# QData/LaMP

Hardware: AMD Instinct MI355X
Metric: forward samples/sec, reuters d512 2+2L 4h (higher is better)
Workload: dtype f32

## Files before the change

### include/lamp_hip.h

```cpp
#ifndef LAMP_HIP_H
#define LAMP_HIP_H

#include <stddef.h>
#include <stdint.h>

#ifdef __cplusplus
extern "C" {
#endif
#if defined(__GNUC__)
#pragma GCC visibility push(default)
#endif

#define LAMP_HIP_ABI_VERSION 5

typedef void* lamp_stream_t;

enum lamp_status {
    LAMP_OK = 0,
    LAMP_E_DIMS = -1,
    LAMP_E_ALIGN = -2,
    LAMP_E_WORKSPACE = -3,
    LAMP_E_UNSUPPORTED = -4,
    LAMP_E_NULL = -5
};
// ... 36 lines not shown
    const float* ln_g;
    const float* ln_b;
    int32_t n_head;
    int32_t present;
} lamp_mha_weights;

typedef struct lamp_ffn_weights {
    const float* w1;
    const float* b1;
    const float* w2;
    const float* b2;
    const float* ln_g;
    const float* ln_b;
} lamp_ffn_weights;

typedef struct lamp_enc_layer {
    lamp_mha_weights slf_attn;
    lamp_ffn_weights pos_ffn;
} lamp_enc_layer;

typedef struct lamp_dec_layer {
    lamp_mha_weights enc_attn;
    lamp_ffn_weights pos_ffn1;
    lamp_mha_weights slf_attn;
    lamp_ffn_weights pos_ffn2;
} lamp_dec_layer;

typedef struct lamp_chain_pack {
    const float* fc;
    const float* w1;
    const float* w2;
    const float* fc4;
    const float* w14;
    const float* w24;
} lamp_chain_pack;

typedef struct lamp_model {
    int32_t n_src_vocab, n_position, n_labels;
    int32_t d_model, d_inner, d_k, d_v;
    int32_t n_layers_enc, n_layers_dec;
    int32_t label_mask_flags;
    const float* src_word_emb;
    const float* position_enc;
    const float* tgt_word_emb;
    const float* w_out;
    const uint8_t* label_mask;
    const uint32_t* label_mask_bits;
    const int32_t* label_tiles;
    const lamp_enc_layer* enc_layers;
    const lamp_dec_layer* dec_layers;
    const float* dec0_query;
    const lamp_chain_pack* chain_packs;
    const float* enc0_emb_w1;
    const float* enc0_pos_w1;
    int64_t label_mask_allowed;
} lamp_model;

typedef struct lamp_aux {
    float* const* enc_self_attn;
    float* const* dec_self_attn;
    float* const* dec_enc_attn;
    float* const* int_preds;
    int32_t n_int_preds;
    int32_t reserved;
} lamp_aux;

int lamp_version(void);
const char* lamp_strerror(int status);


int lamp_linear_fwd(const float* A, int64_t M, int32_t K, int64_t lda,
                    const float* W, int32_t N, int64_t ldw, const float* bias,
                    const float* residual, int64_t ldr, int32_t relu,
                    float* C, int64_t ldc, lamp_stream_t stream);

#define LAMP_PREC_FP32 0
#define LAMP_PREC_BF16X3 1
#define LAMP_PREC_BF16X6 2
int lamp_linear_prec_fwd(const float* A, int64_t M, int32_t K, int64_t lda,
                         const float* W, int32_t N, int64_t ldw, const float* bias,
                         const float* residual, int64_t ldr, int32_t relu,
                         float* C, int64_t ldc, int32_t precision, lamp_stream_t stream);

int lamp_layernorm_fwd(const float* x, int64_t M, int32_t d, const float* gamma, const float* beta,
                       float eps, float* y, lamp_stream_t stream);

int lamp_sdpa_fwd(const float* q, const float* k, const float* v, float* out, float* attn,
                  int32_t B, int32_t H, int32_t lq, int32_t lk, int32_t d_k, int32_t d_v,
                  float inv_temperature, const lamp_mask* mask, const lamp_attn_layout* layout,
                  lamp_stream_t stream);

int lamp_sdpa_fwd_fast_maps(const float* q, const float* k, const float* v, float* out, float* attn, float* lse,
                            int32_t B, int32_t H, int32_t lq, int32_t lk, int32_t d_k, int32_t d_v,
                            float inv_temperature, const lamp_mask* mask, const lamp_attn_layout* layout,
                            lamp_stream_t stream);

#define LAMP_ATTN_SOFTMAX 0
#define LAMP_ATTN_SIGMOID 1

int lamp_sdpa_act_fwd(const float* q, const float* k, const float* v, float* out, float* attn,
                      int32_t B, int32_t H, int32_t lq, int32_t lk, int32_t d_k, int32_t d_v,
                      float inv_temperature, int32_t act, const lamp_mask* mask, const lamp_attn_layout* layout,
                      lamp_stream_t stream);

int lamp_mha_act_fwd(const float* xq, const float* xkv, int32_t B, int32_t lq, int32_t lk,
                     int32_t d_model, int32_t d_k, int32_t d_v, const lamp_mha_weights* w, int32_t act,
                     const lamp_mask* mask, float* out, float* attn,
                     void* workspace, size_t workspace_bytes, lamp_stream_t stream);

size_t lamp_mha_workspace_bytes(int32_t B, int32_t lq, int32_t lk, int32_t d_model, int32_t n_head,
                                int32_t d_k, int32_t d_v);
int lamp_mha_fwd(const float* xq, const float* xkv, int32_t B, int32_t lq, int32_t lk,
                 int32_t d_model, int32_t d_k, int32_t d_v, const lamp_mha_weights* w,
                 const lamp_mask* mask, float* out, float* attn,
                 void* workspace, size_t workspace_bytes, lamp_stream_t stream);

size_t lamp_ffn_workspace_bytes(int64_t M, int32_t d_model, int32_t d_inner);
int lamp_ffn_fwd(const float* x, int64_t M, int32_t d_model, int32_t d_inner,
                 const lamp_ffn_weights* w, float* out,
                 void* workspace, size_t workspace_bytes, lamp_stream_t stream);

int lamp_embed_fwd(const int64_t* src_seq, const int64_t* src_pos, int64_t n_tokens,
                   const float* emb, int32_t n_vocab, const float* pos_table, int32_t n_position,
                   int32_t d_model, float* out, lamp_stream_t stream);

int lamp_diag_logits_fwd(const float* y, const float* w_out, int32_t B, int32_t L, int32_t d_model,
                         float* logits, lamp_stream_t stream);

int lamp_sigmoid_bce_fwd(const float* logits, const float* targets, int64_t n_rows, int32_t L,
                         float* probs, float* row_loss, lamp_stream_t stream);

int lamp_prior_graph_build(const int64_t* label_ids, const int64_t* offsets, int64_t n_samples, int32_t L,
                           float* adj, uint8_t* blocked, lamp_stream_t stream);

int lamp_pack_weight(const float* W, int32_t N, int32_t K, int64_t ldw, int32_t format, float* packed, lamp_stream_t stream);


typedef struct lamp_gemm_desc {
    const float* A;
    const float* B;
    float* C;
    int32_t M, N, K;
    int32_t batch0, batch1;
    int32_t accumulate;
    int64_t a_row_stride, a_col_stride, a_batch0, a_batch1;
    int64_t b_row_stride, b_col_stride, b_batch0, b_batch1;
    int64_t ldc, c_batch0, c_batch1;
    const float* relu_mask;
    int64_t ld_mask;
    float alpha;
    int32_t reserved;
} lamp_gemm_desc;
size_t lamp_gemm_workspace_bytes(int32_t M, int32_t N, int32_t K, int32_t batch);
int lamp_gemm(const lamp_gemm_desc* d, void* workspace, size_t workspace_bytes, lamp_stream_t stream);

int lamp_gemm_grouped(const lamp_gemm_desc* descs, int32_t n, lamp_stream_t stream);


typedef struct lamp_reduce_job {
    const float* partial;
    int64_t n_total, n_seg;
    float* out[3];
    int32_t n_partials;
    int32_t reserved;
} lamp_reduce_job;
int lamp_reduce_partials_grouped(const lamp_reduce_job* jobs, int32_t n, lamp_stream_t stream);
// ... 13 lines not shown
    float p_attn, p_out;
    uint32_t seed_attn, seed_out;
} lamp_mha_train_desc;
int lamp_mha_train_fwd(const lamp_mha_train_desc* c, const lamp_mha_weights* w, const float* xq, const float* xk,
                       const float* xv, const lamp_mask* mask, float* q, float* k, float* v, float* a, float* P, float* Pd,
                       float* lse, float* o, float* y, lamp_stream_t stream);
size_t lamp_mha_bwd_workspace_bytes(const lamp_mha_train_desc* c);
size_t lamp_mha_bwd_partials_bytes(const lamp_mha_train_desc* c);
int lamp_mha_bwd(const lamp_mha_train_desc* c, const lamp_mha_weights* w, const float* xq, const float* xk, const float* xv,
                 const float* q, const float* k, const float* v, const float* a, const float* P, const float* Pd,
                 const float* o, const float* dy, float* dxq, float* d_o, float* da, float* dP, float* dq, float* dk, float* dv,
                 float* dxk, float* dxv, float* dgamma, float* dbeta, float* dwq, float* dwk, float* dwv, float* dfc,
                 void* workspace, size_t workspace_bytes, void* partials, size_t partials_bytes, lamp_reduce_job* job,
                 lamp_stream_t stream);

int lamp_mha_train_act_fwd(const lamp_mha_train_desc* c, const lamp_mha_weights* w, int32_t act, const float* xq,
                           const float* xk, const float* xv, const lamp_mask* mask, float* q, float* k, float* v, float* a,
                           float* P, float* Pd, float* lse, float* o, float* y, lamp_stream_t stream);
int lamp_mha_act_bwd(const lamp_mha_train_desc* c, const lamp_mha_weights* w, int32_t act, const float* xq, const float* xk,
                     const float* xv, const float* q, const float* k, const float* v, const float* a, const float* P,
                     const float* Pd, const float* o, const float* dy, float* dxq, float* d_o, float* da, float* dP, float* dq,
                     float* dk, float* dv, float* dxk, float* dxv, float* dgamma, float* dbeta, float* dwq, float* dwk,
                     float* dwv, float* dfc, void* workspace, size_t workspace_bytes, void* partials, size_t partials_bytes,
                     lamp_reduce_job* job, lamp_stream_t stream);

int lamp_layernorm_residual_fwd(const float* x, const float* residual, int64_t residual_rows, int64_t M, int32_t d,
                                const float* gamma, const float* beta, float eps, float dropout_p, uint32_t seed,
                                float* y, lamp_stream_t stream);

size_t lamp_layernorm_bwd_workspace_bytes(int64_t M, int32_t d);
int lamp_layernorm_bwd(const float* x, const float* residual, int64_t residual_rows, int64_t M, int32_t d,
                       const float* gamma, float eps, float dropout_p, uint32_t seed, const float* dy, float* dz,
                       float* dx, float* dgamma, float* dbeta, float* dbias, void* workspace, size_t workspace_bytes,
                       lamp_stream_t stream);

size_t lamp_colsum_workspace_bytes(int64_t M, int64_t N);
int lamp_colsum(const float* x, int64_t M, int64_t N, int64_t ldx, float* out, void* workspace,
                size_t workspace_bytes, lamp_stream_t stream);

int lamp_dropout(const float* x, int64_t n, float p, uint32_t seed, float* y, lamp_stream_t stream);

int lamp_softmax_bwd(const float* P, const float* dP, int64_t rows, int32_t lk, float scale, float* dS,
                     lamp_stream_t stream);

int lamp_sigmoid_attn_bwd(const float* P, const float* dP, int64_t rows, int32_t lk, float scale, float dropout_p,
                          uint32_t seed, float* dS, lamp_stream_t stream);

int lamp_diag_logits_bwd(const float* y, const float* w_out, const float* dlogits, int32_t B, int32_t L,
                         int32_t d_model, float* dy, float* dw, lamp_stream_t stream);

int lamp_embed_bwd(const int64_t* src_seq, int64_t n_tokens, const float* dout, int32_t d_model, int32_t n_vocab,
                   int64_t pad_idx, float* d_emb, lamp_stream_t stream);


size_t lamp_forward_workspace_bytes(const lamp_model* m, int32_t micro_batch, int32_t T,
                                    int32_t want_attn);

int lamp_forward(const lamp_model* m, const int64_t* src_seq, const int64_t* src_pos,
                 int32_t B, int32_t T, float* logits, float* enc_output, const lamp_aux* aux,
                 void* workspace, size_t workspace_bytes, lamp_stream_t stream);

#define LAMP_FWD_PACKED_ENCODER 1

#define LAMP_FWD_DEC_SIGMOID 2

#define LAMP_FWD_MATMUL_BF16X3 4
#define LAMP_FWD_MATMUL_BF16X6 8

#define LAMP_FWD_LABEL_BIAS 16

typedef struct lamp_fwd_options {
    int32_t enc_self_attn;
    int32_t flags;
    const lamp_mask* enc_mask;
    const lamp_chain_pack* enc_chain_packs;
} lamp_fwd_options;

size_t lamp_forward_opts_workspace_bytes(const lamp_model* m, const lamp_fwd_options* opts, int32_t micro_batch, int32_t T,
                                         int32_t want_attn);
int lamp_forward_opts(const lamp_model* m, const lamp_fwd_options* opts, const int64_t* src_seq, const int64_t* src_pos,
                      int32_t B, int32_t T, float* logits, float* enc_output, const lamp_aux* aux, void* workspace,
                      size_t workspace_bytes, lamp_stream_t stream);

typedef struct lamp_onehot_frontend {
    const float* t1;
    const float* conv1_b;
    const float* conv2_w;
    const float* conv2_b;
    const float* conv2_pack;
    int32_t n_vocab;
    int32_t taps;
} lamp_onehot_frontend;

size_t lamp_onehot_forward_workspace_bytes(const lamp_model* m, const lamp_onehot_frontend* fe, int32_t micro_batch, int32_t T,
                                           int32_t want_attn);
int lamp_onehot_forward(const lamp_model* m, const lamp_onehot_frontend* fe, const int64_t* src_seq, const int64_t* src_pos,
                        int32_t B, int32_t T, float* logits, float* enc_output, const lamp_aux* aux, void* workspace,
                        size_t workspace_bytes, lamp_stream_t stream);

size_t lamp_onehot_forward_opts_workspace_bytes(const lamp_model* m, const lamp_onehot_frontend* fe, const lamp_fwd_options* opts,
                                                int32_t micro_batch, int32_t T, int32_t want_attn);
int lamp_onehot_forward_opts(const lamp_model* m, const lamp_onehot_frontend* fe, const lamp_fwd_options* opts,
                             const int64_t* src_seq, const int64_t* src_pos, int32_t B, int32_t T, float* logits,
                             float* enc_output, const lamp_aux* aux, void* workspace, size_t workspace_bytes,
                             lamp_stream_t stream);

int lamp_conv_pack(const float* w, int32_t c_out, int32_t c_in, int32_t taps, int32_t flip, float* packed, lamp_stream_t stream);
int lamp_onehot_front_fwd(const int64_t* src_seq, int32_t B, int32_t T, const lamp_onehot_frontend* fe, int32_t d_model,
                          float dropout_p, uint32_t seed, float* xpad, lamp_stream_t stream);
int lamp_conv_window_fwd(const float* xpad, int32_t B, int32_t rows_out, int32_t rows_in, int32_t c_in, const float* w_pack,
                         int32_t c_out, const float* bias, int32_t relu, const float* pos_table, int32_t n_position,
                         const int64_t* src_pos, int64_t pos_ld, float* out, float* relu_out, lamp_stream_t stream);
int lamp_conv_relu_bwd_pad(const float* dy, const float* relu_out, int32_t B, int32_t rows, int32_t d, float* dz,
                           lamp_stream_t stream);
size_t lamp_onehot_front_bwd_partials_bytes(int32_t B, int32_t T, int32_t n_vocab, int32_t d_model);
int lamp_onehot_front_bwd(const int64_t* src_seq, int32_t B, int32_t T, const lamp_onehot_frontend* fe, int32_t d_model,
                          float dropout_p, uint32_t seed, const float* dP, float* dz, float* partials, size_t partials_bytes,
                          lamp_stream_t stream);

size_t lamp_ranking_metrics_workspace_bytes(int64_t n_rows, int32_t L);
int lamp_ranking_metrics(const float* probs, int64_t ld_probs, const float* targets, int64_t ld_targets, int64_t n_rows,
                         int32_t L, double fdr_cutoff, double* auc, double* aupr, double* fdr_recall, int64_t* n_pos,
                         int64_t* n_neg, void* workspace, size_t workspace_bytes, lamp_stream_t stream);

int lamp_threshold_counts(const float* probs, int64_t ld_probs, const float* targets, int64_t ld_targets, int64_t n_rows,
                          int32_t L, float threshold, int32_t* label_tp, int32_t* label_fp, int32_t* label_fn,
                          int32_t* sample_tp, int32_t* sample_pred, int32_t* sample_gold, int32_t* sample_mismatch,
                          lamp_stream_t stream);


int lamp_bce_logits_train(const float* const* logits, const float* weights, float* const* dlogits, int32_t n_mats,
                          const float* targets, int64_t n_rows, int32_t L, float* probs, int64_t ld_probs, float* row_loss,
                          int64_t ld_row_loss, lamp_stream_t stream);

int lamp_embed_bwd_ordered(const int64_t* src_seq, int64_t n_tokens, const float* dout, int32_t d_model, int32_t n_vocab,
                           int64_t pad_idx, float* d_emb, lamp_stream_t stream);

enum lamp_optim_kind { LAMP_OPTIM_ADAM = 0, LAMP_OPTIM_SGD = 1 };
typedef struct lamp_optim_entry {
    float* param;
    const float* grad;
    float* exp_avg;
    float* exp_avg_sq;
    int64_t numel;
} lamp_optim_entry;
int lamp_optim_step(const lamp_optim_entry* entries, int32_t n, int32_t kind, int64_t step, double lr, double beta1,
                    double beta2, double eps, lamp_stream_t stream);

enum lamp_kernel_class {
    LAMP_K_EMBED = 0, LAMP_K_GEMM = 1, LAMP_K_ATTN = 2, LAMP_K_LAYERNORM = 3, LAMP_K_DIAG = 4,
    LAMP_K_COUNT = 5
};
int lamp_prof_enable(int32_t on);
int lamp_prof_reset(void);
int lamp_prof_read(int32_t kernel_class, int64_t* launches, double* total_ms, double* flops,
                   double* bytes);

#if defined(__GNUC__)
#pragma GCC visibility pop
#endif
#ifdef __cplusplus
}
#endif
#endif
```

### lamp_amd/Models.py

```python
import ctypes as C

import collections

import torch
import torch.nn as nn

from . import _native as N
from .Decoders import GraphDecoder, MLPDecoder, RNNDecoder
from .Encoders import GraphEncoder, MLPEncoder, RNNEncoder
from .SubLayers import XavierLinear


def _chain_pack(fc, w1, w2, keep):
    ptrs = []
    for fmt in (0, 1):
        trio = [N.weight_pack(w, fmt) for w in (fc, w1, w2)]
        if any(t is None for t in trio):
            trio = [None] * 3
        keep.append(trio)
        ptrs += [N.ptr(t) for t in trio]
    return N.ChainPack(*ptrs)


class _MatmulPrecision:
# ... 88 lines not shown

    def get_trainable_parameters(self):
        frozen = set()
        if hasattr(self.encoder, 'position_enc'):
            frozen |= {id(p) for p in self.encoder.position_enc.parameters()}
        if self.onehot:
            frozen |= {id(p) for p in self.encoder.src_word_emb.parameters()}
        return (p for p in self.parameters() if id(p) not in frozen)

    def invalidate_native_cache(self):
        self._native_cache = None
        self._param_list = None

    def load_state_dict(self, state_dict, *args, **kwargs):
        if state_dict and all(k.startswith('module.') for k in state_dict):
            stripped = collections.OrderedDict((k[len('module.'):], v) for k, v in state_dict.items())
            meta = getattr(state_dict, '_metadata', None)
            if meta is not None:
                stripped._metadata = collections.OrderedDict(
                    (k[len('module.'):] if k.startswith('module.') else ('' if k == 'module' else k), v) for k, v in meta.items())
            state_dict = stripped
        self.invalidate_native_cache()
        return super().load_state_dict(state_dict, *args, **kwargs)

    def train(self, mode=True):
        self.invalidate_native_cache()
        return super().train(mode)

    def _apply(self, fn, *args, **kwargs):
        self.invalidate_native_cache()
        return super()._apply(fn, *args, **kwargs)

    def _weight_tensors(self):
        if not self._fused:
            raise NotImplementedError('the lamp_model descriptor exists for the graph encoder + graph decoder only')
        enc, dec = self.encoder, self.decoder
        out = [enc.src_word_emb.weight, dec.tgt_word_emb.weight, self.tgt_word_proj.linear.weight]
        if hasattr(enc, 'position_enc'):
            out.append(enc.position_enc.weight)

        def mha(m):
            out.extend((m.w_qs.weight, m.w_ks.weight, m.w_vs.weight, m.layer_norm.weight, m.layer_norm.bias))
            if getattr(m, 'fc', None) is not None:
                out.append(m.fc.weight)

        def ffn(m):
            out.extend((m.w_1.weight, m.w_1.bias, m.w_2.weight, m.w_2.bias, m.layer_norm.weight, m.layer_norm.bias))
        for l in enc.layer_stack:
            mha(l.slf_attn)
            ffn(l.pos_ffn)
        for l in dec.layer_stack:
            mha(l.enc_attn)
            ffn(l.pos_ffn1)
            if hasattr(l, 'slf_attn'):
                mha(l.slf_attn)
            ffn(l.pos_ffn2)
        return out

    def _fold_weights(self):
        enc = self.encoder
        ff = enc.layer_stack[0].pos_ffn
        return (enc.src_word_emb.weight, enc.position_enc.weight if hasattr(enc, 'position_enc') else None,
                ff.w_1.weight, ff.w_1.bias)

    def _onehot_weights(self):
        enc = self.encoder
        return (enc.src_word_emb.weight, enc.conv1.weight, enc.conv1.bias, enc.conv2.weight, enc.conv2.bias)

    def _chain_weights(self):
        out = []
        for l in self.decoder.layer_stack:
            for att, ff in ((l.enc_attn, l.pos_ffn1), (getattr(l, 'slf_attn', None), l.pos_ffn2)):
                if att is not None and getattr(att, 'fc', None) is not None:
                    out += [att.fc.weight, ff.w_1.weight, ff.w_2.weight]
        return out

    def _enc_chain_weights(self):
        out = []
        for l in self.encoder.layer_stack:
            if getattr(l.slf_attn, 'fc', None) is not None:
                out += [l.slf_attn.fc.weight, l.pos_ffn.w_1.weight, l.pos_ffn.w_2.weight]
        return out

    def _native_model(self):
        replica = getattr(self, '_is_replica', False)
        params = None if replica else self._param_list
        if params is None:
            params = self._weight_tensors()
            if not replica:
                self._param_list = params
        mask = self.decoder.label_mask_u8
        tiles = self.decoder.label_tiles
        bits = self.decoder.label_mask_bits
        bias = getattr(self.decoder, 'label_bias_f32', None)
        if bias is not None:
            mask, tiles, bits = bias, None, None
        hoist = self.cache_layer0_query and not replica
        packs = self.use_chain_packs and not replica
        onehot = bool(getattr(self.encoder, 'onehot', False))
        live = self.enc_self_attn
        fold = self.fold_embedding and not replica and len(self.encoder.layer_stack) > 0 and not onehot and not live
        sparse = bool(self.use_sparse_label_attention and self.use_mask_bits and self.decoder.label_rows_sparse and bias is None)
        key = tuple(p.data_ptr() for p in params) + (N.ptr(mask), N.ptr(bits), N.ptr(tiles), self.use_label_tiles,
                                                      hoist, self.use_mask_bits, packs, fold, sparse, live, bias is not None)
        if hoist:
            l0 = self.decoder.layer_stack[0].enc_attn
            key += (self.decoder.tgt_word_emb.weight._version, l0.w_qs.weight._version)
        if packs:
            key += tuple(w._version for w in self._chain_weights())
            if live:
                key += tuple(w._version for w in self._enc_chain_weights())
        if fold:
            key += tuple(w._version for w in self._fold_weights() if w is not None)
        if onehot:
            key += tuple((w.data_ptr(), w._version) for w in self._onehot_weights())
        cache = None if replica else self._native_cache
        if cache is not None and cache[0] == key:
            return cache[1]
        for p in params:
            if p.dtype != torch.float32 or not p.is_contiguous():
                raise RuntimeError('lamp_amd expects contiguous fp32 parameters')
        N.require_device(*params)
        enc, dec = self.encoder, self.decoder
        enc_arr = (N.EncLayer * max(1, len(enc.layer_stack)))()
        for i, l in enumerate(enc.layer_stack):
            enc_arr[i] = N.EncLayer(N.mha_weights(l.slf_attn), N.ffn_weights(l.pos_ffn))
        dec_arr = (N.DecLayer * max(1, len(dec.layer_stack)))()
        for i, l in enumerate(dec.layer_stack):
            slf = N.mha_weights(l.slf_attn) if hasattr(l, 'slf_attn') else N.MhaWeights()
            dec_arr[i] = N.DecLayer(N.mha_weights(l.enc_attn), N.ffn_weights(l.pos_ffn1), slf,
                                    N.ffn_weights(l.pos_ffn2))
        pos = enc.position_enc.weight if hasattr(enc, 'position_enc') else None
        w_out = self.tgt_word_proj.linear.weight
        if w_out.size(0) != self.n_labels:
            raise NotImplementedError('proj_share_weight=False read-out is not on the graph path')
        m = N.Model(enc.src_word_emb.weight.size(0), pos.size(0) if pos is not None else 0, self.n_labels,
                    self.d_model, self.d_inner, self.d_k, self.d_v, len(enc.layer_stack), len(dec.layer_stack),
                    N.LAMP_MASK_SPARSE_ROWS if sparse else 0, N.ptr(enc.src_word_emb.weight), N.ptr(pos), N.ptr(dec.tgt_word_emb.weight),
                    N.ptr(w_out), N.ptr(mask), N.ptr(bits) if self.use_mask_bits else 0,
                    N.ptr(tiles) if self.use_label_tiles else 0, enc_arr, dec_arr, 0)
        m.label_mask_allowed = self.decoder.label_allowed_pairs if sparse else 0
        q0 = None
        if hoist and len(dec.layer_stack) > 0:
            q0 = N.linear(dec.tgt_word_emb.weight.detach(), dec.layer_stack[0].enc_attn.w_qs.weight.detach())
            m.dec0_query = q0.data_ptr()
            torch.cuda.current_stream().synchronize()
        pack_arr = pack_keep = None
        if packs and len(dec.layer_stack) > 0:
            pack_arr = (N.ChainPack * (2 * len(dec.layer_stack)))()
            pack_keep = []
            for i, l in enumerate(dec.layer_stack):
                for j, (att, ff) in enumerate(((l.enc_attn, l.pos_ffn1), (getattr(l, 'slf_attn', None), l.pos_ffn2))):
                    if att is None or getattr(att, 'fc', None) is None:
                        continue
                    pack_arr[2 * i + j] = _chain_pack(att.fc.weight, ff.w_1.weight, ff.w_2.weight, pack_keep)
            m.chain_packs = pack_arr
            torch.cuda.current_stream().synchronize()
        enc_pack_arr = None
        if packs and live and len(enc.layer_stack) > 0:
            enc_pack_arr = (N.ChainPack * len(enc.layer_stack))()
            pack_keep = pack_keep if pack_keep is not None else []
            for i, l in enumerate(enc.layer_stack):
                if getattr(l.slf_attn, 'fc', None) is None:
                    continue
                enc_pack_arr[i] = _chain_pack(l.slf_attn.fc.weight, l.pos_ffn.w_1.weight, l.pos_ffn.w_2.weight, pack_keep)
            torch.cuda.current_stream().synchronize()
        fold_keep = None
        if fold:
            emb_w, pos_w, w1, b1 = self._fold_weights()
            w1 = w1.detach().reshape(w1.size(0), -1)
            e1 = N.linear(emb_w.detach(), w1, None if pos_w is not None else b1.detach())
            p1 = N.linear(pos_w.detach(), w1, b1.detach()) if pos_w is not None else None
            m.enc0_emb_w1, m.enc0_pos_w1 = e1.data_ptr(), N.ptr(p1)
            fold_keep = (e1, p1)
            torch.cuda.current_stream().synchronize()
        onehot_keep = None
        if onehot:
            e_w, w1, b1, w2, b2 = (w.detach() for w in self._onehot_weights())
            t1 = N.onehot_tap_table(e_w, w1)
            w2c, b1c, b2c = N.f32c(w2), N.f32c(b1), N.f32c(b2)
            w2p = N.conv_pack(w2c)
            fe = N.onehot_frontend(t1, b1c, w2c, b2c, w2p)
            onehot_keep = (fe, t1, w2c, b1c, b2c, w2p)
            torch.cuda.current_stream().synchronize()
        built = (m, enc_arr, dec_arr, q0, pack_arr, pack_keep, fold_keep, onehot_keep, enc_pack_arr)
        if not replica:
            self._native_cache = (key, built)
        return built

    def _forward_composite(self, src, adj, tgt_seq, return_attns, int_preds):
        src_seq, src_pos = src
        batch_size = src_seq.size(0)
        if self.decoder_type in ('sa_m', 'rnn_m'):
            tgt_seq = tgt_seq[:, :-1]
        enc_output, *enc_self_attns = self.encoder(src_seq, adj, src_pos, return_attns=return_attns)
        dec_output, *dec_output2 = self.decoder(tgt_seq, src_seq, enc_output, return_attns=return_attns,
                                                int_preds=int_preds)
        if self.decoder_type in ('rnn_m', 'mlp'):
            seq_logit = dec_output
        else:
            w = self.tgt_word_proj.linear.weight
            if self.decoder_type == 'graph' and w.size(0) == dec_output.size(1) and self.tgt_word_proj.linear.bias is None:
                if self.training:
                    from . import training
                    seq_logit = training._ReadoutFn.apply(dec_output, w)
                else:
                    seq_logit = N.diag_logits(dec_output, w)
            else:
                seq_logit = self.tgt_word_proj(dec_output)
                if self.decoder_type == 'graph':
                    seq_logit = torch.diagonal(seq_logit, 0, 1, 2)
        if int_preds:
            w = self.tgt_word_proj.linear.weight.detach()
            if self.training:
                from . import training
                preds = [training._ReadoutFn.apply(o, w) for o in dec_output2[0][:-1]]
            else:
                preds = [N.diag_logits(o, w) for o in dec_output2[0][:-1]]
            return seq_logit.reshape(-1, seq_logit.size(-1)), enc_output, preds
        if return_attns:
            return seq_logit.reshape(-1, seq_logit.size(-1)), enc_output, enc_self_attns, dec_output2
        return seq_logit.reshape(-1, seq_logit.size(-1)), enc_output, None

    def forward(self, src, adj, tgt_seq, binary_tgt, return_attns=False, int_preds=False):
        if self.onehot and adj:
            raise NotImplementedError('per-sample input graphs (adj) are not served with the one-hot encoder')
        if not self._fused:
            return self._forward_composite(src, adj, tgt_seq, return_attns, int_preds)
        if adj and return_attns and not int_preds and not self.training and not self.enc_self_attn:
            return self._forward_composite(src, adj, tgt_seq, return_attns, int_preds)
        src_seq, src_pos = src
        if src_seq.is_cuda and src_seq.device.index != torch.cuda.current_device():
            with torch.cuda.device(src_seq.device):
                return self.forward(src, adj, tgt_seq, binary_tgt, return_attns=return_attns, int_preds=int_preds)
        N.require_device(src_seq, src_pos)
        if self.training:
            from . import training
            return training.forward_train(self, src_seq, src_pos, return_attns=bool(return_attns and not int_preds),
                                          int_preds=bool(int_preds), adj=adj if self.enc_self_attn else None)
        dev = src_seq.device
        seq = src_seq.long().contiguous()
        pos = src_pos.long().contiguous()
        B, T = seq.shape
        L, d = self.n_labels, self.d_model
        built = self._native_model()
        model, enc_arr, dec_arr = built[:3]
        fe = built[7][0] if self.onehot else None
        T_in = T
        if fe is not None:
            T = T_in // 2
        Ne, Nd = model.n_layers_enc, model.n_layers_dec

        logits = torch.empty((B, L), dtype=torch.float32, device=dev)
        enc_output = torch.empty((B, T, d), dtype=torch.float32, device=dev)

        aux, keep = None, []
        want_attn = bool(return_attns and not int_preds)
        enc_attns = slf_attns = encdec_attns = ipreds = None
        if int_preds:
            n_int = sum(2 if hasattr(l, 'slf_attn') else 1 for l in self.decoder.layer_stack) - 1
            ipreds = [torch.empty((B, L), dtype=torch.float32, device=dev) for _ in range(n_int)]
            arr = (C.c_void_p * max(1, n_int))(*[t.data_ptr() for t in ipreds])
            keep.append(arr)
            aux = N.Aux(None, None, None, arr, n_int, 0)
        elif want_attn:
            def alloc(h, lq, lk):
                return torch.empty((h * B, lq, lk), dtype=torch.float32, device=dev)
            enc_attns = [alloc(l.slf_attn.n_head, T, T) for l in self.encoder.layer_stack]
            slf_attns = [alloc(l.slf_attn.n_head, L, L) if hasattr(l, 'slf_attn') else None
                         for l in self.decoder.layer_stack]
            encdec_attns = [alloc(l.enc_attn.n_head, L, T) for l in self.decoder.layer_stack]
            a0 = (C.c_void_p * max(1, Ne))(*[t.data_ptr() for t in enc_attns])
            a1 = (C.c_void_p * max(1, Nd))(*[N.ptr(t) for t in slf_attns])
            a2 = (C.c_void_p * max(1, Nd))(*[t.data_ptr() for t in encdec_attns])
            keep += [a0, a1, a2]
            aux = N.Aux(a0, a1, a2, None, 0, 0)

        lib = N.lib()
        opts = None
        if self.enc_self_attn:
            opts = N.FwdOptions(1, N.LAMP_FWD_PACKED_ENCODER if self.use_packed_live_encoder else 0, None, built[8])
            if adj:
                from .Encoders import adj_attn_mask
                m8 = adj_attn_mask(seq, adj)
                mstruct = N.Mask(N.LAMP_MASK_U8, 0, m8.data_ptr(), T * T, T, None, 0, 0)
                keep += [m8, mstruct]
                opts.enc_mask = C.pointer(mstruct)
        if self.dec_attn_type == 'sigmoid':
            if opts is None:
                opts = N.FwdOptions(0, 0, None, None)
            opts.flags |= N.LAMP_FWD_DEC_SIGMOID
        if getattr(self.decoder, 'label_bias_f32', None) is not None:
            if opts is None:
                opts = N.FwdOptions(0, 0, None, None)
            opts.flags |= N.LAMP_FWD_LABEL_BIAS
        prec_flag = N.matmul_precision(self.matmul_precision)[1]
        if prec_flag and not getattr(self, '_is_replica', False):
            if opts is None:
                opts = N.FwdOptions(0, 0, None, None)
            opts.flags |= prec_flag
        if opts is not None and fe is not None:
            def ws_bytes(mb):
                return lib.lamp_onehot_forward_opts_workspace_bytes(C.byref(model), C.byref(fe), C.byref(opts), mb, T_in,
                                                                    int(want_attn))
        elif opts is not None:
            def ws_bytes(mb):
                return lib.lamp_forward_opts_workspace_bytes(C.byref(model), C.byref(opts), mb, T, int(want_attn))
        elif fe is not None:
            def ws_bytes(mb):
                return lib.lamp_onehot_forward_workspace_bytes(C.byref(model), C.byref(fe), mb, T_in, int(want_attn))
        else:
            def ws_bytes(mb):
                return lib.lamp_forward_workspace_bytes(C.byref(model), mb, T, int(want_attn))
        per_sample = ws_bytes(1)
        fixed = 2 * per_sample - ws_bytes(2)
        whole = fixed + (per_sample - fixed) * B + 4096
        budget = max(per_sample + 4096, min(whole, self.workspace_limit_bytes))
        ws = N.workspace(budget, dev)
        if opts is not None and fe is not None:
            N.check(lib.lamp_onehot_forward_opts(C.byref(model), C.byref(fe), C.byref(opts), seq.data_ptr(), pos.data_ptr(), B,
                                                 T_in, logits.data_ptr(), enc_output.data_ptr(),
                                                 C.byref(aux) if aux is not None else None, ws.data_ptr(), ws.numel(),
                                                 N.stream()), 'lamp_onehot_forward_opts')
        elif opts is not None:
            N.check(lib.lamp_forward_opts(C.byref(model), C.byref(opts), seq.data_ptr(), pos.data_ptr(), B, T,
                                          logits.data_ptr(), enc_output.data_ptr(), C.byref(aux) if aux is not None else None,
                                          ws.data_ptr(), ws.numel(), N.stream()), 'lamp_forward_opts')
        elif fe is not None:
            N.check(lib.lamp_onehot_forward(C.byref(model), C.byref(fe), seq.data_ptr(), pos.data_ptr(), B, T_in,
                                            logits.data_ptr(), enc_output.data_ptr(), C.byref(aux) if aux is not None else None,
                                            ws.data_ptr(), ws.numel(), N.stream()), 'lamp_onehot_forward')
        else:
            N.check(lib.lamp_forward(C.byref(model), seq.data_ptr(), pos.data_ptr(), B, T, logits.data_ptr(),
                                     enc_output.data_ptr(), C.byref(aux) if aux is not None else None,
                                     ws.data_ptr(), ws.numel(), N.stream()), 'lamp_forward')
        del keep
        if int_preds:
            return logits, enc_output, ipreds
        if want_attn:
            return logits, enc_output, [enc_attns], [slf_attns, encdec_attns]
        return logits, enc_output, None

    workspace_limit_bytes = 8 << 30
    cache_layer0_query = True
    use_chain_packs = True
    fold_embedding = True
    matmul_precision = _MatmulPrecision()
    use_packed_live_encoder = False
    use_label_tiles = True
    use_sparse_label_attention = True
    use_mask_bits = True
```

### lamp_amd/_native.py

```python
import ctypes as C
import os
import threading

import torch

_HERE = os.path.dirname(os.path.abspath(__file__))
LIB_PATH = os.environ.get('LAMP_HIP_LIBRARY') or os.path.join(_HERE, 'liblamp_hip.so')
TUNING_LIB_PATH = os.path.join(_HERE, 'liblamp_hip_tuning.so')

ABI_VERSION = 5
LAMP_MASK_NONE, LAMP_MASK_U8, LAMP_MASK_KEY_TOKENS_I64, LAMP_MASK_BITS_U32 = 0, 1, 2, 3
LAMP_MASK_BIAS_F32 = 4
LAMP_MASK_SPARSE_ROWS, LAMP_MASK_SELF_RAGGED = 1, 2
LAMP_FWD_PACKED_ENCODER, LAMP_FWD_DEC_SIGMOID = 1, 2
LAMP_FWD_MATMUL_BF16X3, LAMP_FWD_MATMUL_BF16X6 = 4, 8
LAMP_FWD_LABEL_BIAS = 16
LAMP_PREC_FP32, LAMP_PREC_BF16X3, LAMP_PREC_BF16X6 = 0, 1, 2
MATMUL_PRECISIONS = {'highest': (LAMP_PREC_FP32, 0), 'high': (LAMP_PREC_BF16X3, LAMP_FWD_MATMUL_BF16X3),
                     'bf16x6': (LAMP_PREC_BF16X6, LAMP_FWD_MATMUL_BF16X6)}
LAMP_ATTN_SOFTMAX, LAMP_ATTN_SIGMOID = 0, 1
ATTN_TYPES = {'softmax': LAMP_ATTN_SOFTMAX, 'sigmoid': LAMP_ATTN_SIGMOID}
K_EMBED, K_GEMM, K_ATTN, K_LAYERNORM, K_DIAG, K_COUNT = 0, 1, 2, 3, 4, 5
KERNEL_CLASS_NAMES = ('embed', 'gemm', 'attention', 'layernorm', 'diag_readout')


class LampError(RuntimeError):
    def __init__(self, status, where):
        self.status = status
        msg = lib().lamp_strerror(status).decode() if _lib is not None else '?'
        super().__init__('%s failed with status %d: %s' % (where, status, msg))


_f32p = C.POINTER(C.c_float)
_vp = C.c_void_p


class Mask(C.Structure):
    _fields_ = [('kind', C.c_int32), ('flags', C.c_int32), ('ptr', _vp),
                ('stride_b', C.c_int64), ('stride_q', C.c_int64),
                ('tile_list', _vp), ('tile_list_stride', C.c_int64), ('allowed_pairs', C.c_int64)]


class AttnLayout(C.Structure):
    _fields_ = [(n, C.c_int64) for n in ('q_b', 'q_h', 'q_r', 'k_b', 'k_h', 'k_r',
                                         'v_b', 'v_h', 'v_r', 'o_b', 'o_h', 'o_r')]


class MhaWeights(C.Structure):
    _fields_ = [('w_qs', _vp), ('w_ks', _vp), ('w_vs', _vp), ('fc', _vp), ('ln_g', _vp), ('ln_b', _vp),
                ('n_head', C.c_int32), ('present', C.c_int32)]


class FfnWeights(C.Structure):
    _fields_ = [('w1', _vp), ('b1', _vp), ('w2', _vp), ('b2', _vp), ('ln_g', _vp), ('ln_b', _vp)]


class EncLayer(C.Structure):
    _fields_ = [('slf_attn', MhaWeights), ('pos_ffn', FfnWeights)]


class DecLayer(C.Structure):
    _fields_ = [('enc_attn', MhaWeights), ('pos_ffn1', FfnWeights), ('slf_attn', MhaWeights),
                ('pos_ffn2', FfnWeights)]


class ChainPack(C.Structure):
    _fields_ = [('fc', _vp), ('w1', _vp), ('w2', _vp), ('fc4', _vp), ('w14', _vp), ('w24', _vp)]


class Model(C.Structure):
    _fields_ = [('n_src_vocab', C.c_int32), ('n_position', C.c_int32), ('n_labels', C.c_int32),
                ('d_model', C.c_int32), ('d_inner', C.c_int32), ('d_k', C.c_int32), ('d_v', C.c_int32),
                ('n_layers_enc', C.c_int32), ('n_layers_dec', C.c_int32), ('label_mask_flags', C.c_int32),
                ('src_word_emb', _vp), ('position_enc', _vp), ('tgt_word_emb', _vp), ('w_out', _vp),
                ('label_mask', _vp), ('label_mask_bits', _vp), ('label_tiles', _vp), ('enc_layers', C.POINTER(EncLayer)), ('dec_layers', C.POINTER(DecLayer)),
                ('dec0_query', _vp), ('chain_packs', C.POINTER(ChainPack)),
                ('enc0_emb_w1', _vp), ('enc0_pos_w1', _vp), ('label_mask_allowed', C.c_int64)]


class GemmDesc(C.Structure):
    _fields_ = [('A', _vp), ('B', _vp), ('C', _vp), ('M', C.c_int32), ('N', C.c_int32), ('K', C.c_int32),
                ('batch0', C.c_int32), ('batch1', C.c_int32), ('accumulate', C.c_int32),
                ('a_row_stride', C.c_int64), ('a_col_stride', C.c_int64), ('a_batch0', C.c_int64), ('a_batch1', C.c_int64),
                ('b_row_stride', C.c_int64), ('b_col_stride', C.c_int64), ('b_batch0', C.c_int64), ('b_batch1', C.c_int64),
                ('ldc', C.c_int64), ('c_batch0', C.c_int64), ('c_batch1', C.c_int64),
                ('relu_mask', _vp), ('ld_mask', C.c_int64), ('alpha', C.c_float), ('reserved', C.c_int32)]


class ReduceJob(C.Structure):
    _fields_ = [('partial', _vp), ('n_total', C.c_int64), ('n_seg', C.c_int64), ('out', _vp * 3),
                ('n_partials', C.c_int32), ('reserved', C.c_int32)]


class MhaTrainDesc(C.Structure):
    _fields_ = [('B', C.c_int32), ('lq', C.c_int32), ('lk', C.c_int32), ('d_model', C.c_int32), ('n_head', C.c_int32),
                ('d_k', C.c_int32), ('d_v', C.c_int32), ('inv_temperature', C.c_float), ('p_attn', C.c_float),
                ('p_out', C.c_float), ('seed_attn', C.c_uint32), ('seed_out', C.c_uint32)]


class Aux(C.Structure):
    _fields_ = [('enc_self_attn', C.POINTER(_vp)), ('dec_self_attn', C.POINTER(_vp)),
                ('dec_enc_attn', C.POINTER(_vp)), ('int_preds', C.POINTER(_vp)),
                ('n_int_preds', C.c_int32), ('reserved', C.c_int32)]


class FwdOptions(C.Structure):
    _fields_ = [('enc_self_attn', C.c_int32), ('flags', C.c_int32), ('enc_mask', C.POINTER(Mask)),
                ('enc_chain_packs', C.POINTER(ChainPack))]


class OnehotFrontend(C.Structure):
    _fields_ = [('t1', _vp), ('conv1_b', _vp), ('conv2_w', _vp), ('conv2_b', _vp), ('conv2_pack', _vp),
                ('n_vocab', C.c_int32), ('taps', C.c_int32)]


class OptimEntry(C.Structure):
    _fields_ = [('param', _vp), ('grad', _vp), ('exp_avg', _vp), ('exp_avg_sq', _vp), ('numel', C.c_int64)]


LAMP_OPTIM_ADAM, LAMP_OPTIM_SGD = 0, 1
BCE_TRAIN_MAX_MATS = 8


_i32, _i64, _sz, _f = C.c_int32, C.c_int64, C.c_size_t, C.c_float
PROTOTYPES = {
    'lamp_version': (C.c_int, []),
    'lamp_strerror': (C.c_char_p, [C.c_int]),
    'lamp_linear_fwd': (C.c_int, [_vp, _i64, _i32, _i64, _vp, _i32, _i64, _vp, _vp, _i64, _i32, _vp, _i64, _vp]),
    'lamp_linear_prec_fwd': (C.c_int, [_vp, _i64, _i32, _i64, _vp, _i32, _i64, _vp, _vp, _i64, _i32, _vp, _i64, _i32, _vp]),
    'lamp_layernorm_fwd': (C.c_int, [_vp, _i64, _i32, _vp, _vp, _f, _vp, _vp]),
    'lamp_sdpa_fwd': (C.c_int, [_vp, _vp, _vp, _vp, _vp, _i32, _i32, _i32, _i32, _i32, _i32, _f,
                                C.POINTER(Mask), C.POINTER(AttnLayout), _vp]),
    'lamp_sdpa_fwd_fast_maps': (C.c_int, [_vp, _vp, _vp, _vp, _vp, _vp, _i32, _i32, _i32, _i32, _i32, _i32, _f,
                                          C.POINTER(Mask), C.POINTER(AttnLayout), _vp]),
    'lamp_mha_workspace_bytes': (_sz, [_i32, _i32, _i32, _i32, _i32, _i32, _i32]),
    'lamp_mha_fwd': (C.c_int, [_vp, _vp, _i32, _i32, _i32, _i32, _i32, _i32, C.POINTER(MhaWeights),
                               C.POINTER(Mask), _vp, _vp, _vp, _sz, _vp]),
    'lamp_ffn_workspace_bytes': (_sz, [_i64, _i32, _i32]),
    'lamp_ffn_fwd': (C.c_int, [_vp, _i64, _i32, _i32, C.POINTER(FfnWeights), _vp, _vp, _sz, _vp]),
    'lamp_embed_fwd': (C.c_int, [_vp, _vp, _i64, _vp, _i32, _vp, _i32, _i32, _vp, _vp]),
    'lamp_diag_logits_fwd': (C.c_int, [_vp, _vp, _i32, _i32, _i32, _vp, _vp]),
    'lamp_pack_weight': (C.c_int, [_vp, _i32, _i32, _i64, _i32, _vp, _vp]),
    'lamp_gemm_workspace_bytes': (_sz, [_i32, _i32, _i32, _i32]),
    'lamp_gemm': (C.c_int, [C.POINTER(GemmDesc), _vp, _sz, _vp]),
    'lamp_gemm_grouped': (C.c_int, [C.POINTER(GemmDesc), _i32, _vp]),
    'lamp_ffn_train_fwd': (C.c_int, [_vp, _i64, _i32, _i32, C.POINTER(FfnWeights), _f, C.c_uint32, _vp, _vp, _vp, _vp]),
    'lamp_reduce_partials_grouped': (C.c_int, [C.POINTER(ReduceJob), _i32, _vp]),
    'lamp_ffn_bwd_workspace_bytes': (_sz, [_i64, _i32, _i32]),
    'lamp_ffn_bwd_partials_bytes': (_sz, [_i64, _i32, _i32]),
    'lamp_ffn_bwd': (C.c_int, [_vp, _vp, _vp, _vp, _i64, _i32, _i32, C.POINTER(FfnWeights), _f, C.c_uint32] + [_vp] * 9 +
                     [_vp, _sz, _vp, _sz, C.POINTER(ReduceJob), _vp]),
    'lamp_mha_train_fwd': (C.c_int, [C.POINTER(MhaTrainDesc), C.POINTER(MhaWeights), _vp, _vp, _vp, C.POINTER(Mask)] +
                           [_vp] * 9 + [_vp]),
    'lamp_mha_bwd_workspace_bytes': (_sz, [C.POINTER(MhaTrainDesc)]),
    'lamp_mha_bwd_partials_bytes': (_sz, [C.POINTER(MhaTrainDesc)]),
    'lamp_mha_bwd': (C.c_int, [C.POINTER(MhaTrainDesc), C.POINTER(MhaWeights)] + [_vp] * 11 + [_vp] * 15 +
                     [_vp, _sz, _vp, _sz, C.POINTER(ReduceJob), _vp]),
    'lamp_layernorm_residual_fwd': (C.c_int, [_vp, _vp, _i64, _i64, _i32, _vp, _vp, _f, _f, C.c_uint32, _vp, _vp]),
    'lamp_layernorm_bwd_workspace_bytes': (_sz, [_i64, _i32]),
    'lamp_layernorm_bwd': (C.c_int, [_vp, _vp, _i64, _i64, _i32, _vp, _f, _f, C.c_uint32, _vp, _vp, _vp, _vp, _vp, _vp,
                                     _vp, _sz, _vp]),
    'lamp_colsum_workspace_bytes': (_sz, [_i64, _i64]),
    'lamp_colsum': (C.c_int, [_vp, _i64, _i64, _i64, _vp, _vp, _sz, _vp]),
    'lamp_dropout': (C.c_int, [_vp, _i64, _f, C.c_uint32, _vp, _vp]),
    'lamp_softmax_bwd': (C.c_int, [_vp, _vp, _i64, _i32, _f, _vp, _vp]),
    'lamp_diag_logits_bwd': (C.c_int, [_vp, _vp, _vp, _i32, _i32, _i32, _vp, _vp, _vp]),
    'lamp_embed_bwd': (C.c_int, [_vp, _i64, _vp, _i32, _i32, _i64, _vp, _vp]),
    'lamp_prior_graph_build': (C.c_int, [_vp, _vp, _i64, _i32, _vp, _vp, _vp]),
    'lamp_sigmoid_bce_fwd': (C.c_int, [_vp, _vp, _i64, _i32, _vp, _vp, _vp]),
    'lamp_forward_workspace_bytes': (_sz, [C.POINTER(Model), _i32, _i32, _i32]),
    'lamp_forward': (C.c_int, [C.POINTER(Model), _vp, _vp, _i32, _i32, _vp, _vp, C.POINTER(Aux), _vp, _sz, _vp]),
    'lamp_forward_opts_workspace_bytes': (_sz, [C.POINTER(Model), C.POINTER(FwdOptions), _i32, _i32, _i32]),
    'lamp_forward_opts': (C.c_int, [C.POINTER(Model), C.POINTER(FwdOptions), _vp, _vp, _i32, _i32, _vp, _vp, C.POINTER(Aux),
                                    _vp, _sz, _vp]),
    'lamp_onehot_forward_opts_workspace_bytes': (_sz, [C.POINTER(Model), C.POINTER(OnehotFrontend), C.POINTER(FwdOptions),
                                                       _i32, _i32, _i32]),
    'lamp_onehot_forward_opts': (C.c_int, [C.POINTER(Model), C.POINTER(OnehotFrontend), C.POINTER(FwdOptions), _vp, _vp, _i32,
                                           _i32, _vp, _vp, C.POINTER(Aux), _vp, _sz, _vp]),
    'lamp_onehot_forward_workspace_bytes': (_sz, [C.POINTER(Model), C.POINTER(OnehotFrontend), _i32, _i32, _i32]),
    'lamp_onehot_forward': (C.c_int, [C.POINTER(Model), C.POINTER(OnehotFrontend), _vp, _vp, _i32, _i32, _vp, _vp,
                                      C.POINTER(Aux), _vp, _sz, _vp]),
    'lamp_conv_pack': (C.c_int, [_vp, _i32, _i32, _i32, _i32, _vp, _vp]),
    'lamp_onehot_front_fwd': (C.c_int, [_vp, _i32, _i32, C.POINTER(OnehotFrontend), _i32, _f, C.c_uint32, _vp, _vp]),
    'lamp_conv_window_fwd': (C.c_int, [_vp, _i32, _i32, _i32, _i32, _vp, _i32, _vp, _i32, _vp, _i32, _vp, _i64, _vp, _vp,
                                       _vp]),
    'lamp_conv_relu_bwd_pad': (C.c_int, [_vp, _vp, _i32, _i32, _i32, _vp, _vp]),
    'lamp_onehot_front_bwd_partials_bytes': (_sz, [_i32, _i32, _i32, _i32]),
    'lamp_onehot_front_bwd': (C.c_int, [_vp, _i32, _i32, C.POINTER(OnehotFrontend), _i32, _f, C.c_uint32, _vp, _vp, _vp,
                                        _sz, _vp]),
    'lamp_ranking_metrics_workspace_bytes': (_sz, [_i64, _i32]),
    'lamp_ranking_metrics': (C.c_int, [_vp, _i64, _vp, _i64, _i64, _i32, C.c_double, _vp, _vp, _vp, _vp, _vp, _vp, _sz, _vp]),
    'lamp_threshold_counts': (C.c_int, [_vp, _i64, _vp, _i64, _i64, _i32, _f] + [_vp] * 7 + [_vp]),
    'lamp_embed_bwd_ordered': (C.c_int, [_vp, _i64, _vp, _i32, _i32, _i64, _vp, _vp]),
    'lamp_bce_logits_train': (C.c_int, [C.POINTER(_vp), _f32p, C.POINTER(_vp), _i32, _vp, _i64, _i32, _vp, _i64, _vp, _i64, _vp]),
    'lamp_optim_step': (C.c_int, [C.POINTER(OptimEntry), _i32, _i32, _i64] + [C.c_double] * 4 + [_vp]),
    'lamp_sdpa_act_fwd': (C.c_int, [_vp, _vp, _vp, _vp, _vp, _i32, _i32, _i32, _i32, _i32, _i32, _f, _i32,
                                    C.POINTER(Mask), C.POINTER(AttnLayout), _vp]),
    'lamp_mha_act_fwd': (C.c_int, [_vp, _vp, _i32, _i32, _i32, _i32, _i32, _i32, C.POINTER(MhaWeights), _i32,
                                   C.POINTER(Mask), _vp, _vp, _vp, _sz, _vp]),
    'lamp_mha_train_act_fwd': (C.c_int, [C.POINTER(MhaTrainDesc), C.POINTER(MhaWeights), _i32, _vp, _vp, _vp, C.POINTER(Mask)] +
                               [_vp] * 9 + [_vp]),
    'lamp_mha_act_bwd': (C.c_int, [C.POINTER(MhaTrainDesc), C.POINTER(MhaWeights), _i32] + [_vp] * 11 + [_vp] * 15 +
                         [_vp, _sz, _vp, _sz, C.POINTER(ReduceJob), _vp]),
    'lamp_sigmoid_attn_bwd': (C.c_int, [_vp, _vp, _i64, _i32, _f, _f, C.c_uint32, _vp, _vp]),
    'lamp_prof_enable': (C.c_int, [_i32]),
    'lamp_prof_reset': (C.c_int, []),
    'lamp_prof_read': (C.c_int, [_i32, C.POINTER(_i64), C.POINTER(C.c_double), C.POINTER(C.c_double),
                                 C.POINTER(C.c_double)]),
}

_lib = None
_lock = threading.Lock()


def load_library(path):
    if not os.path.exists(path):
        raise RuntimeError(
            'lamp_amd: %s is missing -- build it with `python -m lamp_amd.build` '
            '(hipcc, gfx950).  There is no CPU or PyTorch fallback.' % path)
    handle = C.CDLL(path)
    handle.lamp_version.restype = C.c_int
    version = handle.lamp_version()
    old_ok = version in (2, 3) and os.environ.get('LAMP_ALLOW_OLD_ABI') == '1'
    if version != ABI_VERSION and not old_ok:
        raise RuntimeError('lamp_amd: ABI version mismatch in ' + path)
    for name, (res, args) in PROTOTYPES.items():
        if old_ok and not hasattr(handle, name):
            continue
        fn = getattr(handle, name)
        fn.restype = res
        fn.argtypes = args
    return handle


def lib():
    global _lib
    if _lib is None:
        with _lock:
            if _lib is None:
                _lib = load_library(LIB_PATH)
    return _lib


def check(status, where):
    if status != 0:
        raise LampError(status, where)


def require_device(*tensors):
    cur = None
    for t in tensors:
        if t is None:
            continue
        if not t.is_cuda:
            raise RuntimeError('lamp_amd runs on an MI355X HIP device only; got a %s tensor (%s). '
                               'There is no CPU path.' % (t.device, tuple(t.shape)))
        if cur is None:
            cur = torch.cuda.current_device()
        if t.device.index != cur:
            raise RuntimeError('lamp_amd: tensor on %s but the current device is cuda:%d -- wrap the call in '
                               '`with torch.cuda.device(tensor.device):` (LAMP.forward does so itself)' % (t.device, cur))


def f32c(t):
    if t.dtype != torch.float32:
        t = t.float()
    return t if t.is_contiguous() else t.contiguous()


def ptr(t):
    return 0 if t is None else t.data_ptr()


_raw_stream = getattr(torch._C, '_cuda_getCurrentRawStream', None)


def stream():
    if _raw_stream is not None:
        return _raw_stream(torch.cuda.current_device())
    return torch.cuda.current_stream().cuda_stream


_ws = {}


def workspace(nbytes, device):
    key = (device.type, device.index if device.index is not None else torch.cuda.current_device(), stream())
    buf = _ws.get(key)
    if buf is None or buf.numel() < nbytes:
        buf = torch.empty(int(nbytes) + 256, dtype=torch.uint8, device=device)
        _ws[key] = buf
    return buf


def make_mask(mask, B, lq, lk):
    if mask is None:
        return None, None
    require_device(mask)
    m = mask
    if m.dtype == torch.bool:
        m = m.view(torch.uint8) if m.is_contiguous() or m.stride(-1) == 1 else m.contiguous().view(torch.uint8)
    elif m.dtype != torch.uint8:
        m = (m != 0).view(torch.uint8)
    if m.dim() == 2:
        m = m.unsqueeze(0)
    if m.dim() != 3 or m.size(-1) != lk or m.size(1) not in (1, lq) or m.size(0) not in (1, B):
        raise ValueError('attention mask of shape %s does not broadcast to (%d, %d, %d)' %
                         (tuple(mask.shape), B, lq, lk))
    if m.stride(-1) != 1 and lk > 1:
        m = m.contiguous()
# ... 130 lines not shown
    lay = AttnLayout(lq * H * dk, dk, H * dk, lk * H * dk, dk, H * dk, lk * H * dv, dv, H * dv, lq * H * dv, dv, H * dv)
    m = C.byref(mask_struct) if mask_struct is not None else None
    if act != LAMP_ATTN_SOFTMAX:
        check(L.lamp_sdpa_act_fwd(ptr(q), ptr(k), ptr(v), ptr(out), ptr(attn), B, H, lq, lk, dk, dv,
                                  float(inv_temperature), int(act), m, C.byref(lay), stream()), 'lamp_sdpa_act_fwd')
        return out, (attn if need_attn else None)
    if fast_maps and need_attn:
        lse = torch.empty((H * B * lq,), dtype=torch.float32, device=q.device)
        check(L.lamp_sdpa_fwd_fast_maps(ptr(q), ptr(k), ptr(v), ptr(out), ptr(attn), ptr(lse), B, H, lq, lk, dk, dv,
                                        float(inv_temperature), m, C.byref(lay), stream()), 'lamp_sdpa_fwd_fast_maps')
        return (out, attn, lse.view(H * B, lq)) if return_lse else (out, attn)
    check(L.lamp_sdpa_fwd(ptr(q), ptr(k), ptr(v), ptr(out), ptr(attn), B, H, lq, lk, dk, dv,
                          float(inv_temperature), m, C.byref(lay), stream()), 'lamp_sdpa_fwd')
    return out, (attn if need_attn else None)


def mha_weights(mod):
    fc = getattr(mod, 'fc', None)
    return MhaWeights(ptr(mod.w_qs.weight), ptr(mod.w_ks.weight), ptr(mod.w_vs.weight),
                      ptr(fc.weight) if fc is not None else 0, ptr(mod.layer_norm.weight),
                      ptr(mod.layer_norm.bias), mod.n_head, 1)


def ffn_weights(mod):
    return FfnWeights(ptr(mod.w_1.weight), ptr(mod.w_1.bias), ptr(mod.w_2.weight), ptr(mod.w_2.bias),
                      ptr(mod.layer_norm.weight), ptr(mod.layer_norm.bias))


def mha(xq, xkv, weights, d_k, d_v, mask_struct, need_attn, act=LAMP_ATTN_SOFTMAX):
    require_device(xq, xkv)
    xq, xkv = f32c(xq), f32c(xkv)
    B, lq, d = xq.shape
    lk = xkv.size(1)
    h = weights.n_head
    out = torch.empty_like(xq)
    attn = torch.empty((h * B, lq, lk), dtype=torch.float32, device=xq.device) if need_attn else None
    nbytes = lib().lamp_mha_workspace_bytes(B, lq, lk, d, h, d_k, d_v)
    ws = workspace(nbytes, xq.device)
    m = C.byref(mask_struct) if mask_struct is not None else None
    if act != LAMP_ATTN_SOFTMAX:
        check(lib().lamp_mha_act_fwd(ptr(xq), ptr(xkv), B, lq, lk, d, d_k, d_v, C.byref(weights), int(act), m, ptr(out),
                                     ptr(attn), ptr(ws), ws.numel(), stream()), 'lamp_mha_act_fwd')
        return out, attn
    check(lib().lamp_mha_fwd(ptr(xq), ptr(xkv), B, lq, lk, d, d_k, d_v, C.byref(weights), m, ptr(out), ptr(attn),
                             ptr(ws), ws.numel(), stream()), 'lamp_mha_fwd')
    return out, attn


def ffn(x, weights, d_inner):
    require_device(x)
    x2 = f32c(x).reshape(-1, x.size(-1))
    M, d = x2.shape
    out = torch.empty_like(x2)
    nbytes = lib().lamp_ffn_workspace_bytes(M, d, d_inner)
    ws = workspace(nbytes, x.device)
    check(lib().lamp_ffn_fwd(ptr(x2), M, d, d_inner, C.byref(weights), ptr(out), ptr(ws), ws.numel(),
                             stream()), 'lamp_ffn_fwd')
    return out.view(x.shape)


def embed(src_seq, src_pos, emb, pos_table):
    require_device(src_seq, src_pos, emb, pos_table)
    seq = src_seq.long().contiguous()
    pos = src_pos.long().contiguous() if pos_table is not None else None
    d = emb.size(1)
    out = torch.empty(tuple(seq.shape) + (d,), dtype=torch.float32, device=emb.device)
    check(lib().lamp_embed_fwd(ptr(seq), ptr(pos), seq.numel(), ptr(f32c(emb)), emb.size(0),
                               ptr(f32c(pos_table)) if pos_table is not None else 0,
                               pos_table.size(0) if pos_table is not None else 0, d, ptr(out), stream()),
          'lamp_embed_fwd')
    return out


def weight_pack(w, fmt=0):
    require_device(w)
    w = f32c(w.detach())
    n, k = w.size(0), w.size(1)
    fn = getattr(lib(), 'lamp_pack_weight', None)
    if fn is None or (n % 16 or k % 32 if fmt == 0 else n % 64 or k % 16):
        return None
    out = torch.empty(n * k, dtype=torch.float32, device=w.device)
    check(fn(ptr(w), n, k, k, fmt, ptr(out), stream()), 'lamp_pack_weight')
    return out


def diag_logits(y, w_out):
    require_device(y, w_out)
    y = f32c(y)
    B, L, d = y.shape
    out = torch.empty((B, L), dtype=torch.float32, device=y.device)
    check(lib().lamp_diag_logits_fwd(ptr(y), ptr(f32c(w_out)), B, L, d, ptr(out), stream()),
          'lamp_diag_logits_fwd')
    return out


def _dims4(t):
    sh, st = tuple(t.shape), t.stride()
    n = len(sh)
    if n == 2:
        return (1, 1) + sh, (0, 0) + st
    if n == 3:
        return (1,) + sh, (0,) + st
    if n == 4:
        return sh, st
    raise ValueError('gemm operands must be 2-, 3- or 4-dimensional')


def _operand(t):
    sh, st = _dims4(t)
    rs, cs = st[2], st[3]
    if sh[3] == 1 and rs != 1:
        cs = 1
    elif sh[2] == 1 and cs != 1:
        rs = 1
    if rs != 1 and cs != 1:
        t = t.contiguous()
        sh, st = _dims4(t)
        rs, cs = st[2], st[3]
    return t, sh, rs, cs, (0 if sh[0] == 1 else st[0], 0 if sh[1] == 1 else st[1])


def matmul_nt(a, b, out=None, alpha=1.0, accumulate=False, relu_mask=None):
    if not (a.is_cuda and b.is_cuda):
        require_device(a, b)
    if a.dtype != torch.float32 or b.dtype != torch.float32:
        raise TypeError('matmul_nt needs float32 operands')
    A, ash, ars, acs, abs_ = _operand(a)
    Bm, bsh, brs, bcs, bbs = _operand(b)
    M, K, Nn = ash[2], ash[3], bsh[2]
    if bsh[3] != K:
        raise ValueError('contraction sizes differ: %s vs %s' % (tuple(a.shape), tuple(b.shape)))
    b0, b1 = max(ash[0], bsh[0]), max(ash[1], bsh[1])
    if ash[0] not in (1, b0) or ash[1] not in (1, b1) or bsh[0] not in (1, b0) or bsh[1] not in (1, b1):
        raise ValueError('batch dims do not broadcast: %s vs %s' % (tuple(a.shape), tuple(b.shape)))
    if out is None:
        if accumulate:
            raise ValueError('accumulate needs an out tensor')
        lead = a.shape[:-2] if a.dim() >= b.dim() else b.shape[:-2]
        out = torch.empty(tuple(lead) + (M, Nn), dtype=torch.float32, device=a.device)
    csh, cst = _dims4(out)
    if cst[3] != 1 and csh[3] != 1:
        raise ValueError('out must have unit stride on its last dim')
    if csh != (b0, b1, M, Nn):
        raise ValueError('out has shape %s, expected %s' % (tuple(out.shape), (b0, b1, M, Nn)))
    d = GemmDesc(A.data_ptr(), Bm.data_ptr(), out.data_ptr(), M, Nn, K, b0, b1, 1 if accumulate else 0,
                 ars, acs, abs_[0], abs_[1], brs, bcs, bbs[0], bbs[1],
                 cst[2], 0 if csh[0] == 1 else cst[0], 0 if csh[1] == 1 else cst[1], None, 0, float(alpha), 0)
    keep = None
    if relu_mask is not None:
        keep = f32c(relu_mask)
        if tuple(keep.shape[-2:]) != (M, Nn) or keep.numel() != M * Nn:
            raise ValueError('relu_mask must be (M, N)')
        d.relu_mask, d.ld_mask = keep.data_ptr(), Nn
    L = lib()
    nb = L.lamp_gemm_workspace_bytes(M, Nn, K, b0 * b1)
    ws = workspace(nb, a.device) if nb else None
    check(L.lamp_gemm(C.byref(d), ptr(ws), nb, stream()), 'lamp_gemm')
    return out


def matmul_nt_grouped(problems):
    groups = {}
    for a, b, out, accumulate in problems:
        if not (a.is_cuda and b.is_cuda and out.is_cuda):
            require_device(a, b, out)
        if a.dtype != torch.float32 or b.dtype != torch.float32 or out.dtype != torch.float32:
# ... 443 lines not shown
```

### lamp_amd/csrc/api.hip

```cpp
#include <algorithm>
#include <mutex>
#include <vector>

#include "lamp_kernels.h"

namespace lamp {

namespace {
struct ProfRec {
    int cls;
    double flops, bytes;
    hipEvent_t e0, e1;
};
std::mutex g_prof_mu;
bool g_prof_on = false;
std::vector<ProfRec> g_prof;
std::vector<hipEvent_t> g_event_pool;
constexpr size_t PROF_MAX = 1 << 16;

hipEvent_t take_event() {
    if (!g_event_pool.empty()) {
        hipEvent_t e = g_event_pool.back();
        g_event_pool.pop_back();
        return e;
    }
    hipEvent_t e = nullptr;
    if (hipEventCreate(&e) != hipSuccess) return nullptr;
    return e;
}
}

ProfScope::ProfScope(int kernel_class, double flops, double bytes, hipStream_t stream) : idx(-1), s(stream) {
    if (!g_prof_on) return;
    std::lock_guard<std::mutex> lk(g_prof_mu);
    if (!g_prof_on || g_prof.size() >= PROF_MAX) return;
    ProfRec r{kernel_class, flops, bytes, take_event(), take_event()};
    if (!r.e0 || !r.e1) return;
    (void)hipEventRecord(r.e0, s);
    idx = int(g_prof.size());
    g_prof.push_back(r);
}

ProfScope::~ProfScope() {
    if (idx < 0) return;
    std::lock_guard<std::mutex> lk(g_prof_mu);
    if (idx < int(g_prof.size())) (void)hipEventRecord(g_prof[idx].e1, s);
}

#define LAMP_CK(expr)            \
    do {                         \
        int _e = (expr);         \
        if (_e != 0) return _e;  \
    } while (0)

static inline size_t align_up(size_t v, size_t a) { return (v + a - 1) / a * a; }

struct Carver {
    char* base;
    size_t mb;
    size_t off = 0;
    size_t per = 0, fixed = 0;
    template <class P>
    void take(P** p, size_t per_sample_floats, size_t fixed_floats = 0) {
        if (p) *p = base ? reinterpret_cast<P*>(base + off) : nullptr;
        off += align_up((per_sample_floats * mb + fixed_floats) * sizeof(float), 256);
        per += per_sample_floats * sizeof(float);
        fixed += fixed_floats * sizeof(float) + 256;
    }
    size_t bound(size_t n) const { return per * n + fixed; }
};

struct ResGather {
    const int* tok;
    const int* pos;
    const float* emb;
    const float* pos_table;
};

static inline int fwd_matmul_prec(const lamp_fwd_options* o) {
    const int f = o ? o->flags & (LAMP_FWD_MATMUL_BF16X3 | LAMP_FWD_MATMUL_BF16X6) : 0;
    return f == 0 ? LAMP_PREC_FP32 : f == LAMP_FWD_MATMUL_BF16X3 ? LAMP_PREC_BF16X3 : f == LAMP_FWD_MATMUL_BF16X6 ? LAMP_PREC_BF16X6 : -1;
}

static int linear(const float* A, int64_t M, int K, int64_t lda, const float* const* W, int nseg, int N,
                  int64_t ldw, const float* const* bias, const float* R, int64_t ldr, int relu,
                  float* const* C, int64_t ldc, int prec, hipStream_t s, const int* m_dev = nullptr,
                  const float* A_dense = nullptr, const ResGather* rg = nullptr) {
    GemmParams p{};
    p.A = A; p.lda = lda; p.M = M; p.K = K; p.N = N; p.nseg = nseg; p.ldw = ldw; p.ldc = ldc;
    p.R = R; p.ldr = ldr; p.relu = relu; p.m_dev = m_dev; p.A_dense = A_dense;
    if (rg) {
        p.R = nullptr;
        p.rg_tok = rg->tok; p.rg_pos = rg->pos; p.rg_emb = rg->emb; p.rg_pos_table = rg->pos_table;
    }
    for (int i = 0; i < nseg; ++i) {
        p.W[i] = W[i];
        p.bias[i] = bias ? bias[i] : nullptr;
        p.C[i] = C[i];
    }
    if (prec == LAMP_PREC_BF16X3) return launch_gemm_split(p, 3, s);
    if (prec == LAMP_PREC_BF16X6) return launch_gemm_split(p, 6, s);
    return launch_gemm(p, s);
}

static int check_mask(const lamp_mask* m, int act = LAMP_ATTN_SOFTMAX) {
    if (!m) return 0;
    if (m->kind != LAMP_MASK_NONE && m->kind != LAMP_MASK_U8 && m->kind != LAMP_MASK_KEY_TOKENS_I64 &&
        m->kind != LAMP_MASK_BITS_U32 && m->kind != LAMP_MASK_BIAS_F32)
        return LAMP_E_UNSUPPORTED;
    if (m->kind != LAMP_MASK_NONE && !m->ptr) return LAMP_E_NULL;
    if (m->kind == LAMP_MASK_BIAS_F32) {
        if (act == LAMP_ATTN_SIGMOID || m->tile_list || (m->flags & (LAMP_MASK_SPARSE_ROWS | LAMP_MASK_SELF_RAGGED)))
            return LAMP_E_UNSUPPORTED;
        if (!aligned16(m->ptr) || (m->stride_q & 3) || (m->stride_b & 3)) return LAMP_E_ALIGN;
    }
    return 0;
}

static void attn_mask(AttnParams& a, const lamp_mask* mask) {
    a.mask_kind = mask ? mask->kind : LAMP_MASK_NONE;
    a.mask = mask ? mask->ptr : nullptr;
    a.m_sb = mask ? mask->stride_b : 0;
    a.m_sq = mask ? mask->stride_q : 0;
    a.tiles = (mask && !a.P) ? mask->tile_list : nullptr;
    a.tiles_stride = mask ? mask->tile_list_stride : 0;
    a.sparse_rows = mask && (mask->flags & LAMP_MASK_SPARSE_ROWS) != 0;
    a.self_ragged = mask && (mask->flags & LAMP_MASK_SELF_RAGGED) != 0;
    a.allowed_pairs = mask ? mask->allowed_pairs : 0;
}

static int project_qkv(const lamp_mha_weights& w, int d, int dk, int dv, const float* xq, int64_t Mq, float* Q,
                       const float* xk, const float* xv, int64_t Mk, float* K, float* V, int prec, hipStream_t s,
                       const int* m_dev, const float* A_dense) {
    const int hdk = w.n_head * dk, hdv = w.n_head * dv;
    const bool one_kv = K && V && xk == xv && hdk == hdv;
    const bool one_qkv = one_kv && Q && xq == xk && Mq == Mk && !m_dev;
    const float* W[3] = {w.w_qs, w.w_ks, w.w_vs};
    float* C[3] = {Q, K, V};
    if (Q) LAMP_CK(linear(xq, Mq, d, d, W, one_qkv ? 3 : 1, hdk, d, nullptr, nullptr, 0, 0, C, hdk, prec, s));
    if (one_qkv) return 0;
    if (one_kv) return linear(xk, Mk, d, d, W + 1, 2, hdk, d, nullptr, nullptr, 0, 0, C + 1, hdk, prec, s, m_dev, A_dense);
    if (K) LAMP_CK(linear(xk, Mk, d, d, W + 1, 1, hdk, d, nullptr, nullptr, 0, 0, C + 1, hdk, prec, s, m_dev, A_dense));
    if (V) LAMP_CK(linear(xv, Mk, d, d, W + 2, 1, hdv, d, nullptr, nullptr, 0, 0, C + 2, hdv, prec, s, m_dev, A_dense));
    return 0;
}

struct FfnParams {
    const float* x;
    int64_t M;
    int d, dff;
    const lamp_ffn_weights* w;
    float *out, *hidden;
    const float* w_out = nullptr;
    int n_labels = 0;
    float* logits = nullptr;
    const int* rows_dev = nullptr;
    const SeqPlan* scatter = nullptr;
    int nb = 0, T = 0;
    float* y_flat = nullptr;
    bool hidden_ready = false;
    const ResGather* rg = nullptr;
    int prec = LAMP_PREC_FP32;
};

static int ffn_core(const FfnParams& f, hipStream_t s) {
    const lamp_ffn_weights& w = *f.w;
    const int d = f.d, dff = f.dff;
    if (!w.w1 || !w.b1 || !w.w2 || !w.b2 || !w.ln_g || !w.ln_b) return LAMP_E_NULL;
    if (f.rg && !f.hidden_ready) return LAMP_E_UNSUPPORTED;
    if (!f.hidden_ready) {
        const float* W[1] = {w.w1};
        const float* b[1] = {w.b1};
        float* C[1] = {f.hidden};
        LAMP_CK(linear(f.x, f.M, d, d, W, 1, dff, d, b, nullptr, 0, 1, C, dff, f.prec, s, f.rows_dev));
    }
    {
        const float* W[1] = {w.w2};
        const float* b[1] = {w.b2};
        float* C[1] = {f.out};
        LAMP_CK(linear(f.hidden, f.M, dff, dff, W, 1, d, dff, b, f.x, d, 0, C, d, f.prec, s, f.rows_dev, nullptr, f.rg));
    }
    LayerNormParams ln{f.out, f.M, d, w.ln_g, w.ln_b, f.out};
    if (f.scatter) {
        ln.M = int64_t(f.nb) * f.T; ln.scatter = f.scatter; ln.T = f.T; ln.y_flat = f.y_flat;
    } else if (f.rows_dev) {
        ln.m_dev = f.rows_dev;
    } else if (f.w_out) {
        ln.y = nullptr; ln.w_out = f.w_out; ln.n_labels = f.n_labels; ln.logits = f.logits;
    }
    return launch_layernorm(ln, s);
}

struct MhaScratch {
    float *Q, *K, *V, *A;
    float* S = nullptr;
    float* lse = nullptr;
    int* plan_ints = nullptr;
};
static inline SeqPlan plan_from(int* ints, int64_t B, int T) {
    return SeqPlan{ints, ints + B, ints + 2 * B, ints + 3 * B + 1, reinterpret_cast<unsigned*>(ints + 3 * B + 3), (T + 31) / 32, nullptr};
}
static inline bool wide_heads(int dk, int dv) { return dk > 128 || dv > 128; }
static inline void take_plan(Carver& c, int** ints, int T) { c.take(ints, 3 + size_t((T + 31) / 32), 3); }

static void mha_layout(Carver& c, MhaScratch& sc, int lq, int lk, int h, int dk, int dv, bool plan) {
    c.take(&sc.Q, size_t(lq) * h * dk);
    c.take(&sc.K, size_t(lk) * h * dk);
    c.take(&sc.V, size_t(lk) * h * dv);
    c.take(&sc.A, size_t(lq) * h * dv);
    if (wide_heads(dk, dv)) c.take(&sc.S, size_t(h) * lq * lk);
    c.take(&sc.lse, size_t(h) * lq);
    if (plan) take_plan(c, &sc.plan_ints, lk);
}

struct MhaCall {
    const float* xq;
    const float* xkv;
    int B, lq, lk, d, dk, dv;
    const lamp_mha_weights* w;
    const lamp_mask* mask;
    float* out;
    float* attn;
    int P_batch = 0, P_b0 = 0;
    bool xq_shared = false;
    const float* q_ready = nullptr;
    bool kv_ready = false;
    const SeqPlan* keys = nullptr;
    bool keys_packed = false;
    const float* xkv_dense = nullptr;
    int act = LAMP_ATTN_SOFTMAX;
    int prec = LAMP_PREC_FP32;
};


static int mha_attend(const MhaCall& c, const MhaScratch& sc, hipStream_t s) {
    const lamp_mha_weights& w = *c.w;
    const int h = w.n_head, d = c.d, dk = c.dk, dv = c.dv, B = c.B, lq = c.lq, lk = c.lk;
    if (h < 1 || dk < 1 || dv < 1) return LAMP_E_DIMS;
    if (!w.w_qs || !w.w_ks || !w.w_vs || (c.out && (!w.ln_g || !w.ln_b))) return LAMP_E_NULL;
    if (h == 1 && c.out && dv != d) return LAMP_E_DIMS;
    if (h > 1 && c.out && !w.fc) return LAMP_E_NULL;
    const int hdk = h * dk, hdv = h * dv;
    const bool need_v = c.out != nullptr;
    const bool kv = !c.kv_ready;
    LAMP_CK(project_qkv(w, d, dk, dv, c.xq, c.xq_shared ? lq : int64_t(B) * lq, c.q_ready ? nullptr : sc.Q, c.xkv, c.xkv,
                        int64_t(B) * lk, kv ? sc.K : nullptr, kv && need_v ? sc.V : nullptr, c.prec, s,
                        c.keys_packed ? c.keys->rows : nullptr, c.keys_packed ? c.xkv_dense : nullptr));

    const lamp_mask* mask = c.mask;
    const SeqPlan* keys = c.keys;
    SeqPlan local_plan{};
    if (!keys && mask && mask->kind == LAMP_MASK_KEY_TOKENS_I64 && sc.plan_ints && !wide_heads(dk, dv)) {
        local_plan = plan_from(sc.plan_ints, B, lk);
        LAMP_CK(launch_seq_plan(static_cast<const int64_t*>(mask->ptr), nullptr, B, lk, mask->stride_b, false, local_plan, s));
        keys = &local_plan;
    }

    AttnParams a{};
    a.Q = c.q_ready ? c.q_ready : sc.Q; a.K = sc.K; a.V = need_v ? sc.V : nullptr; a.O = need_v ? sc.A : nullptr; a.P = c.attn;
    a.scratch = sc.S;
    if (c.attn && need_v && sc.lse && c.act == LAMP_ATTN_SOFTMAX) a.lse = sc.lse;
    a.act = c.act;
    a.B = B; a.H = h; a.lq = lq; a.lk = lk; a.dk = dk; a.dv = dv;
    a.P_batch = c.P_batch > 0 ? c.P_batch : B; a.P_b0 = c.P_b0;
    a.lay.q_b = c.xq_shared ? 0 : int64_t(lq) * hdk; a.lay.q_h = dk; a.lay.q_r = hdk;
    a.lay.k_b = int64_t(lk) * hdk; a.lay.k_h = dk; a.lay.k_r = hdk;
    a.lay.v_b = int64_t(lk) * hdv; a.lay.v_h = dv; a.lay.v_r = hdv;
    a.lay.o_b = int64_t(lq) * hdv; a.lay.o_h = dv; a.lay.o_r = hdv;
    a.scale_log2e = float(1.4426950408889634 / sqrt(double(dk)));
    attn_mask(a, mask);
    if (keys && mask && mask->kind == LAMP_MASK_KEY_TOKENS_I64) {
        a.kv_len = keys->klen;
        a.kv_off = keys->off;
        if (!wide_heads(dk, dv)) {
            a.mask_kind = LAMP_MASK_BITS_U32;
            a.mask = keys->padbits;
            a.m_sb = keys->words;
            a.m_sq = 0;
        }
    }
    return launch_attn(a, s);
}

static int mha_tail(const MhaCall& c, const MhaScratch& sc, const FfnParams* f, const lamp_chain_pack* pk, bool* ffn_ran,
                    hipStream_t s) {
    const lamp_mha_weights& w = *c.w;
    const int h = w.n_head, d = c.d, B = c.B, lq = c.lq, hdv = h * c.dv;
    const float* xq = c.xq;
    float* out = c.out;
    const int64_t M = int64_t(B) * lq;
    const int64_t r_mod = c.xq_shared ? lq : 0;
    if (f) *ffn_ran = false;
    if (h > 1 && f && chain_applies(M, d, hdv, f->dff, true, pk, c.xq_shared, f->w_out != nullptr)) {
        *ffn_ran = true;
        return launch_chain(sc.A, hdv, hdv, xq, r_mod, M, d, w.fc, w.ln_g, w.ln_b, f->w, f->dff, f->w_out ? nullptr : out,
                            f->w_out, f->n_labels, f->logits, s, pk);
    }
    if (h > 1 && f && pk && M > 6144 && (!f->w_out || f->n_labels == lq)) {
        const int per = (B + 1) / 2, last = B - per;
        if (int64_t(per) * lq <= 6144 && int64_t(last) * lq > 4608 &&
            chain_applies(int64_t(per) * lq, d, hdv, f->dff, true, pk, c.xq_shared, f->w_out != nullptr) &&
            chain_applies(int64_t(last) * lq, d, hdv, f->dff, true, pk, c.xq_shared, f->w_out != nullptr)) {
            for (int g = 0; g < 2; ++g) {
                const int64_t r0 = int64_t(g) * per * lq, rows = int64_t(g == 0 ? per : last) * lq;
                LAMP_CK(launch_chain(sc.A + r0 * hdv, hdv, hdv, c.xq_shared ? xq : xq + r0 * d, r_mod, rows, d, w.fc, w.ln_g,
                                     w.ln_b, f->w, f->dff, f->w_out ? nullptr : out + r0 * d, f->w_out, f->n_labels,
                                     f->logits ? f->logits + r0 : nullptr, s, pk));
            }
            *ffn_ran = true;
            return 0;
        }
    }
    LayerNormParams ln{h == 1 ? sc.A : out, M, d, w.ln_g, w.ln_b, out};
    if (h == 1 || c.xq_shared) { ln.residual = xq; ln.r_mod = r_mod; }
    if (h > 1) {
        const float* W[1] = {w.fc};
        float* C[1] = {out};
        LAMP_CK(linear(sc.A, M, hdv, hdv, W, 1, d, hdv, nullptr, ln.residual ? nullptr : xq, ln.residual ? 0 : d, 0, C, d, c.prec, s));
    }
    return launch_layernorm(ln, s);
}

}

using namespace lamp;

namespace {
int sdpa_impl(const float* q, const float* k, const float* v, float* out, float* attn, float* lse, int32_t B, int32_t H,
              int32_t lq, int32_t lk, int32_t d_k, int32_t d_v, float inv_temperature, const lamp_mask* mask,
                  const lamp_attn_layout* layout, lamp_stream_t stream, int act = LAMP_ATTN_SOFTMAX) {
    if (!layout) return LAMP_E_NULL;
    LAMP_CK(check_mask(mask, act));
    AttnParams a{};
    a.Q = q; a.K = k; a.V = v; a.O = out; a.P = attn; a.lse = act == LAMP_ATTN_SOFTMAX ? lse : nullptr;
    a.act = act;
    a.B = B; a.H = H; a.lq = lq; a.lk = lk; a.dk = d_k; a.dv = d_v;
    a.P_batch = B; a.P_b0 = 0;
    a.lay = *layout;
    a.scale_log2e = float(double(inv_temperature) * 1.4426950408889634);
    attn_mask(a, mask);
    return launch_attn(a, hipStream_t(stream));
}
}

extern "C" {

int lamp_version(void) { return LAMP_HIP_ABI_VERSION; }

const char* lamp_strerror(int status) {
    switch (status) {
        case LAMP_OK: return "ok";
        case LAMP_E_DIMS: return "lamp: non-positive or inconsistent dimensions";
        case LAMP_E_ALIGN: return "lamp: pointer or leading dimension not 16-byte aligned";
        case LAMP_E_WORKSPACE: return "lamp: workspace too small";
        case LAMP_E_UNSUPPORTED: return "lamp: configuration not supported by this build";
        case LAMP_E_NULL: return "lamp: required pointer is NULL";
        default: break;
    }
    if (status > 0) return hipGetErrorString(hipError_t(status));
    return "lamp: unknown status";
}

int lamp_linear_fwd(const float* A, int64_t M, int32_t K, int64_t lda, const float* W, int32_t N, int64_t ldw,
                    const float* bias, const float* residual, int64_t ldr, int32_t relu, float* C, int64_t ldc,
                    lamp_stream_t stream) {
    return lamp_linear_prec_fwd(A, M, K, lda, W, N, ldw, bias, residual, ldr, relu, C, ldc, LAMP_PREC_FP32, stream);
}

int lamp_linear_prec_fwd(const float* A, int64_t M, int32_t K, int64_t lda, const float* W, int32_t N, int64_t ldw,
                         const float* bias, const float* residual, int64_t ldr, int32_t relu, float* C, int64_t ldc,
                         int32_t precision, lamp_stream_t stream) {
    if (precision != LAMP_PREC_FP32 && precision != LAMP_PREC_BF16X3 && precision != LAMP_PREC_BF16X6) return LAMP_E_UNSUPPORTED;
    const float* Ws[1] = {W};
    const float* bs[1] = {bias};
    float* Cs[1] = {C};
    if (lda < K || ldw < K || ldc < N || (residual && ldr < N)) return LAMP_E_DIMS;
    return linear(A, M, K, lda, Ws, 1, N, ldw, bs, residual, ldr, relu, Cs, ldc, precision, hipStream_t(stream));
}

int lamp_layernorm_fwd(const float* x, int64_t M, int32_t d, const float* gamma, const float* beta, float eps,
                       float* y, lamp_stream_t stream) {
    LayerNormParams p{x, M, d, gamma, beta, y, eps};
    return launch_layernorm(p, hipStream_t(stream));
}

int lamp_sdpa_fwd(const float* q, const float* k, const float* v, float* out, float* attn, int32_t B, int32_t H,
                  int32_t lq, int32_t lk, int32_t d_k, int32_t d_v, float inv_temperature, const lamp_mask* mask,
                  const lamp_attn_layout* layout, lamp_stream_t stream) {
    return sdpa_impl(q, k, v, out, attn, nullptr, B, H, lq, lk, d_k, d_v, inv_temperature, mask, layout, stream);
}

int lamp_sdpa_act_fwd(const float* q, const float* k, const float* v, float* out, float* attn, int32_t B, int32_t H,
                      int32_t lq, int32_t lk, int32_t d_k, int32_t d_v, float inv_temperature, int32_t act,
                      const lamp_mask* mask, const lamp_attn_layout* layout, lamp_stream_t stream) {
    return sdpa_impl(q, k, v, out, attn, nullptr, B, H, lq, lk, d_k, d_v, inv_temperature, mask, layout, stream, act);
}

int lamp_sdpa_fwd_fast_maps(const float* q, const float* k, const float* v, float* out, float* attn, float* lse,
                            int32_t B, int32_t H, int32_t lq, int32_t lk, int32_t d_k, int32_t d_v,
                            float inv_temperature, const lamp_mask* mask, const lamp_attn_layout* layout,
                            lamp_stream_t stream) {
    if (!attn || !lse || !out || !v) return LAMP_E_NULL;
    return sdpa_impl(q, k, v, out, attn, lse, B, H, lq, lk, d_k, d_v, inv_temperature, mask, layout, stream);
}

size_t lamp_mha_workspace_bytes(int32_t B, int32_t lq, int32_t lk, int32_t d_model, int32_t n_head, int32_t d_k,
                                int32_t d_v) {
    (void)d_model;
    if (B <= 0 || lq <= 0 || lk <= 0 || n_head <= 0 || d_k <= 0 || d_v <= 0) return 0;
    Carver c{nullptr, size_t(B)};
    MhaScratch sc;
    mha_layout(c, sc, lq, lk, n_head, d_k, d_v, true);
    return c.off;
}

int lamp_mha_fwd(const float* xq, const float* xkv, int32_t B, int32_t lq, int32_t lk, int32_t d_model,
                 int32_t d_k, int32_t d_v, const lamp_mha_weights* w, const lamp_mask* mask, float* out,
                 float* attn, void* workspace, size_t workspace_bytes, lamp_stream_t stream) {
    return lamp_mha_act_fwd(xq, xkv, B, lq, lk, d_model, d_k, d_v, w, LAMP_ATTN_SOFTMAX, mask, out, attn, workspace,
                            workspace_bytes, stream);
}

int lamp_mha_act_fwd(const float* xq, const float* xkv, int32_t B, int32_t lq, int32_t lk, int32_t d_model,
                     int32_t d_k, int32_t d_v, const lamp_mha_weights* w, int32_t act, const lamp_mask* mask, float* out,
                     float* attn, void* workspace, size_t workspace_bytes, lamp_stream_t stream) {
    if (act != LAMP_ATTN_SOFTMAX && act != LAMP_ATTN_SIGMOID) return LAMP_E_UNSUPPORTED;
    if (!xq || !xkv || !w || !out || !workspace) return LAMP_E_NULL;
    if (B <= 0 || lq <= 0 || lk <= 0 || d_model <= 0 || d_k <= 0 || d_v <= 0 || w->n_head <= 0) return LAMP_E_DIMS;
    if (d_model & 3) return LAMP_E_UNSUPPORTED;
    LAMP_CK(check_mask(mask, act));
    Carver c{static_cast<char*>(workspace), size_t(B)};
    MhaScratch sc;
    mha_layout(c, sc, lq, lk, w->n_head, d_k, d_v, true);
    if (c.off > workspace_bytes) return LAMP_E_WORKSPACE;
    MhaCall a{xq, xkv, B, lq, lk, d_model, d_k, d_v, w, mask, out, attn};
    a.act = act;
    LAMP_CK(mha_attend(a, sc, hipStream_t(stream)));
    return mha_tail(a, sc, nullptr, nullptr, nullptr, hipStream_t(stream));
}

size_t lamp_ffn_workspace_bytes(int64_t M, int32_t d_model, int32_t d_inner) {
    (void)d_model;
    if (M <= 0 || d_inner <= 0) return 0;
    return align_up(size_t(M) * d_inner * sizeof(float), 256);
}

int lamp_ffn_fwd(const float* x, int64_t M, int32_t d_model, int32_t d_inner, const lamp_ffn_weights* w,
                 float* out, void* workspace, size_t workspace_bytes, lamp_stream_t stream) {
    if (!x || !w || !out || !workspace) return LAMP_E_NULL;
    if (M <= 0 || d_model <= 0 || d_inner <= 0) return LAMP_E_DIMS;
    if ((d_model & 3) || (d_inner & 3)) return LAMP_E_UNSUPPORTED;
    if (workspace_bytes < size_t(M) * d_inner * sizeof(float)) return LAMP_E_WORKSPACE;
    return ffn_core(FfnParams{x, M, d_model, d_inner, w, out, static_cast<float*>(workspace)}, hipStream_t(stream));
}

int lamp_embed_fwd(const int64_t* src_seq, const int64_t* src_pos, int64_t n_tokens, const float* emb,
                   int32_t n_vocab, const float* pos_table, int32_t n_position, int32_t d_model, float* out,
                   lamp_stream_t stream) {
    return launch_embed(src_seq, src_pos, n_tokens, emb, n_vocab, pos_table, n_position, d_model, out,
                        hipStream_t(stream));
// ... 370 lines not shown
    if (!m) return LAMP_E_NULL;
    const int T = fe ? T_in / 2 : T_in;
    if (m->d_model <= 0 || m->d_inner <= 0 || m->d_k <= 0 || m->d_v <= 0 || m->n_labels <= 0 || T <= 0 ||
        m->n_layers_enc < 0 || m->n_layers_dec < 0)
        return LAMP_E_DIMS;
    if ((m->n_layers_enc && !m->enc_layers) || (m->n_layers_dec && !m->dec_layers)) return LAMP_E_NULL;
    int h = 1;
    for (int i = 0; i < m->n_layers_enc; ++i) h = std::max(h, m->enc_layers[i].slf_attn.n_head);
    for (int i = 0; i < m->n_layers_dec; ++i) {
        const lamp_dec_layer& l = m->dec_layers[i];
        h = std::max(h, l.enc_attn.n_head);
        if (l.slf_attn.present) h = std::max(h, l.slf_attn.n_head);
    }
    const int L = m->n_labels, R = std::max(T + (live ? 1 : 0), L);
    *g = FwdDims{T, L, R, want_attn || live ? R : L, m->d_model, m->d_inner, h, m->d_k, m->d_v, fe ? 0 : m->n_layers_dec,
                 fe ? T + 16 : 0, fe && !fe->conv2_pack, live};
    return 0;
}

struct FwdScratch {
    float* H;
    MhaScratch mha;
    float* Y;
    float* Xp;
    int* plan_ints;
    unsigned long long* granules;
    int *row_tok, *row_pos;
    float *K_ahead[GEMM_MAX_SEG / 2], *V_ahead[GEMM_MAX_SEG / 2];
    int* live_rows;
    float* fe_x;
    float* w2;
};

static void fwd_layout(const FwdDims& g, Carver& c, FwdScratch& w) {
    const size_t T = g.T, d = g.d;
    c.take(&w.H, size_t(g.R) * g.dff, g.dff);
    mha_layout(c, w.mha, g.Rq, g.R, g.h, g.dk, g.dv, false);
    c.take(&w.Y, size_t(g.L) * d);
    c.take(&w.Xp, (T + (g.live ? 1 : 0)) * d, d);
    if (g.live) c.take(&w.live_rows, 0, 4);
    take_plan(c, &w.plan_ints, g.T);
    c.take(&w.granules, 4, 4);
    c.take(&w.row_tok, 2 * T, 2);
    for (int i = 0; i < g.n_ahead; ++i) {
        const bool kept = i < GEMM_MAX_SEG / 2;
        c.take(kept ? &w.K_ahead[i] : nullptr, T * g.h * g.dk);
        c.take(kept ? &w.V_ahead[i] : nullptr, T * g.h * g.dv);
    }
    if (g.fe_rows) c.take(&w.fe_x, size_t(g.fe_rows) * d, 16 * d);
    if (g.w2_repack) c.take(&w.w2, 0, 16 * d * d);
    w.row_pos = w.row_tok ? w.row_tok + (c.mb * T + 1) : nullptr;
}

static Carver fwd_size(const FwdDims& g) {
    Carver c{nullptr, 1};
    FwdScratch unused;
    fwd_layout(g, c, unused);
    return c;
}

struct Pass {
    const lamp_model* m;
    const lamp_onehot_frontend* fe;
    const FwdDims& g;
    const FwdScratch& w;
    const lamp_aux* aux;
    float* logits;
    hipStream_t s;
    int B, nb;
    int64_t b0;
    const int64_t *seq, *pos;
    int64_t ld_seq;
    float* x;
    bool packed;
    SeqPlan sp;
    lamp_mask pad_mask;
    lamp_mask label_mask;
    const float* xk = nullptr;
    int n_int = 0;
    const lamp_mask* enc_mask = nullptr;
    const lamp_chain_pack* enc_packs = nullptr;
    int dec_act = LAMP_ATTN_SOFTMAX;
    int prec = LAMP_PREC_FP32;
};

static int encode_packed(Pass& p) {
    const lamp_model* m = p.m;
    const FwdScratch& w = p.w;
    const int d = p.g.d, dff = p.g.dff, T = p.g.T;
    const bool folded = m->enc0_emb_w1 != nullptr;
    const bool gather_res =
        folded && gemm_gathered_residual_ok(d, dff, d, m->enc_layers[0].pos_ffn.b2, w.Xp, m->src_word_emb, m->position_enc);
    const EmbedFold fold{m->enc0_emb_w1, m->enc0_pos_w1, dff, folded ? w.H : nullptr, gather_res ? w.row_tok : nullptr,
                         gather_res ? w.row_pos : nullptr};
    const ResGather rg{w.row_tok, w.row_pos, m->src_word_emb, m->position_enc};
    LAMP_CK(launch_embed_plan(p.seq, p.pos, m->position_enc != nullptr, p.nb, T, m->src_word_emb, m->n_src_vocab,
                              m->position_enc, m->n_position, d, p.sp, w.granules, w.Xp, p.s, &fold));
    for (int i = 0; i < m->n_layers_enc; ++i) {
        FfnParams f{w.Xp, int64_t(p.nb) * T + 1, d, dff, &m->enc_layers[i].pos_ffn, w.Xp, w.H};
        f.prec = p.prec;
        f.rows_dev = p.sp.rows + 1; f.hidden_ready = folded && i == 0; f.rg = gather_res && i == 0 ? &rg : nullptr;
        if (i + 1 == m->n_layers_enc) { f.scatter = &p.sp; f.nb = p.nb; f.T = T; f.y_flat = p.x; }
        LAMP_CK(ffn_core(f, p.s));
    }
    p.xk = w.Xp;
    return 0;
}

static int encode_packed_live(Pass& p) {
    const lamp_model* m = p.m;
    const FwdScratch& w = p.w;
    const int d = p.g.d, dff = p.g.dff, T = p.g.T, dk = p.g.dk, dv = p.g.dv;
    const int64_t Mub = int64_t(p.nb) * (T + 1);
    const EmbedFold fold{nullptr, nullptr, dff, nullptr, nullptr, nullptr};
    LAMP_CK(launch_embed_plan(p.seq, p.pos, m->position_enc != nullptr, p.nb, T, m->src_word_emb, m->n_src_vocab,
                              m->position_enc, m->n_position, d, p.sp, w.granules, w.Xp, p.s, &fold));
    LAMP_CK(launch_pad_rows(m->src_word_emb, m->position_enc, d, p.nb, p.sp, w.Xp, w.live_rows, p.s));
    for (int i = 0; i < m->n_layers_enc; ++i) {
        const lamp_mha_weights& a = m->enc_layers[i].slf_attn;
        const int hdk = a.n_head * dk, hdv = a.n_head * dv;
        const float* W[3] = {a.w_qs, a.w_ks, a.w_vs};
        float* C[3] = {w.mha.Q, w.mha.K, w.mha.V};
        LAMP_CK(linear(w.Xp, Mub, d, d, W, 3, hdk, d, nullptr, nullptr, 0, 0, C, hdk, p.prec, p.s, w.live_rows));
        LAMP_CK(launch_attn_ragged_self(w.mha.Q, w.mha.K, w.mha.V, w.mha.A, p.nb, a.n_head, T, dk, dv, p.sp, p.s));
        const float* Wfc[1] = {a.fc};
        float* Cx[1] = {w.Xp};
        LAMP_CK(linear(w.mha.A, Mub, hdv, hdv, Wfc, 1, d, hdv, nullptr, w.Xp, d, 0, Cx, d, p.prec, p.s, w.live_rows));
        LayerNormParams ln{w.Xp, Mub, d, a.ln_g, a.ln_b, w.Xp};
        ln.m_dev = w.live_rows;
        LAMP_CK(launch_layernorm(ln, p.s));
        FfnParams f{w.Xp, Mub, d, dff, &m->enc_layers[i].pos_ffn, w.Xp, w.H};
        f.rows_dev = w.live_rows; f.prec = p.prec;
        LAMP_CK(ffn_core(f, p.s));
    }
    LAMP_CK(launch_scatter_rows(w.Xp, d, p.nb, T, p.sp, p.x, p.s));
    p.xk = w.Xp;
    return 0;
}

static int encode_onehot_front(const Pass& p) {
    const lamp_onehot_frontend* fe = p.fe;
    const int d = p.g.d, T = p.g.T;
    LAMP_CK(launch_front_fwd(p.seq, p.nb, int(p.ld_seq), fe->t1, fe->n_vocab, fe->conv1_b, d, 0.f, 0u, 0, p.w.fe_x, p.s));
    ConvWindowParams cp{p.w.fe_x, p.w.w2, fe->conv2_b, p.x, nullptr, p.m->position_enc, p.pos, int64_t(p.nb) * T, d, p.ld_seq,
                        d, 16 * d, d, T, T + 16, 1, p.m->n_position};
    return launch_conv_window(cp, p.s);
}

static int encode_padded(Pass& p) {
    const lamp_model* m = p.m;
    const FwdScratch& w = p.w;
    const int d = p.g.d, dff = p.g.dff, T = p.g.T;
    const int64_t Me = int64_t(p.nb) * T;
    LAMP_CK(launch_seq_plan(p.seq, m->position_enc ? p.pos : nullptr, p.nb, T, p.ld_seq, false, p.sp, p.s));
    const bool folded = m->enc0_emb_w1 && m->n_layers_enc > 0;
    if (p.fe) {
        LAMP_CK(encode_onehot_front(p));
    } else {
        const EmbedFold fold{m->enc0_emb_w1, m->enc0_pos_w1, dff, folded ? w.H : nullptr, nullptr, nullptr};
        LAMP_CK(launch_embed(p.seq, p.pos, Me, m->src_word_emb, m->n_src_vocab, m->position_enc, m->n_position, d, p.x, p.s,
                             &fold));
    }
    for (int i = 0; i < m->n_layers_enc; ++i) {
        const lamp_enc_layer& l = m->enc_layers[i];
        float* map = p.aux && p.aux->enc_self_attn ? p.aux->enc_self_attn[i] : nullptr;
        FfnParams f{p.x, Me, d, dff, &l.pos_ffn, p.x, w.H};
        f.prec = p.prec;
        if (p.g.live) {
            MhaCall a{p.x, p.x, p.nb, T, T, d, p.g.dk, p.g.dv, &l.slf_attn, p.enc_mask, p.x, map, p.B, int(p.b0)};
            a.keys = &p.sp; a.prec = p.prec;
            bool ffn_ran = false;
            LAMP_CK(mha_attend(a, w.mha, p.s));
            LAMP_CK(mha_tail(a, w.mha, &f, p.enc_packs ? p.enc_packs + i : nullptr, &ffn_ran, p.s));
            if (!ffn_ran) LAMP_CK(ffn_core(f, p.s));
            continue;
        }
        if (map) {
            MhaCall a{p.x, p.x, p.nb, T, T, d, p.g.dk, p.g.dv, &l.slf_attn, p.enc_mask, nullptr, map, p.B, int(p.b0)};
            a.keys = &p.sp; a.prec = p.prec;
            LAMP_CK(mha_attend(a, w.mha, p.s));
        }
        f.hidden_ready = folded && i == 0;
        LAMP_CK(ffn_core(f, p.s));
    }
    p.xk = p.x;
    return 0;
}

static int project_kv_layers(const float* x, int64_t Me, int d, int dk, int dv, const lamp_dec_layer* layers, int n,
                             float* const* K, float* const* V, int prec, hipStream_t s, const int* m_dev, const float* A_dense) {
    const int h = layers[0].enc_attn.n_head;
    bool uniform = 2 * n <= GEMM_MAX_SEG && h * dk == h * dv;
    for (int i = 1; i < n && uniform; ++i) uniform = layers[i].enc_attn.n_head == h;
    if (uniform) {
        const float* W[GEMM_MAX_SEG];
        float* C[GEMM_MAX_SEG];
        for (int i = 0; i < n; ++i) {
            if (!layers[i].enc_attn.w_ks || !layers[i].enc_attn.w_vs) return LAMP_E_NULL;
            W[2 * i] = layers[i].enc_attn.w_ks;
            W[2 * i + 1] = layers[i].enc_attn.w_vs;
            C[2 * i] = K[i];
            C[2 * i + 1] = V[i];
        }
        return linear(x, Me, d, d, W, 2 * n, h * dk, d, nullptr, nullptr, 0, 0, C, h * dk, prec, s, m_dev, A_dense);
    }
    for (int i = 0; i < n; ++i)
        LAMP_CK(project_qkv(layers[i].enc_attn, d, dk, dv, nullptr, 0, nullptr, x, x, Me, K[i], V[i], prec, s, m_dev, A_dense));
    return 0;
}

static int int_pred(Pass& p) {
    const lamp_aux* a = p.aux;
    const int n = p.n_int++;
    if (!a || !a->int_preds || n >= a->n_int_preds || !a->int_preds[n]) return 0;
    return launch_diag(p.w.Y, p.m->w_out, p.nb, p.g.L, p.g.d, a->int_preds[n] + p.b0 * p.g.L, p.s);
}

static int decoder_layer(Pass& p, int i) {
    const lamp_model* m = p.m;
    const FwdDims& g = p.g;
    const FwdScratch& w = p.w;
    const lamp_dec_layer& l = m->dec_layers[i];
    const int d = g.d, dff = g.dff, L = g.L;
    const bool last = i + 1 == m->n_layers_dec;
    const int64_t Md = int64_t(p.nb) * L;
    float* Y = w.Y;
    const lamp_chain_pack* pk = m->chain_packs ? m->chain_packs + 2 * i : nullptr;
    bool ffn_ran = false;
    FfnParams f1{Y, Md, d, dff, &l.pos_ffn1, Y, w.H}, f2{Y, Md, d, dff, &l.pos_ffn2, Y, w.H};
    f2.n_labels = L;
    f1.prec = f2.prec = p.prec;
    const bool fused_readout = last && !g.live;
    if (fused_readout) { f2.w_out = m->w_out; f2.logits = p.logits + p.b0 * L; }

    MhaScratch sc = w.mha;
    if (g.n_ahead) { sc.K = w.K_ahead[i]; sc.V = w.V_ahead[i]; }
    MhaCall enc{i == 0 ? m->tgt_word_emb : Y, p.xk, p.nb, L, g.T, d, g.dk, g.dv, &l.enc_attn, &p.pad_mask, Y,
                p.aux && p.aux->dec_enc_attn ? p.aux->dec_enc_attn[i] : nullptr, p.B, int(p.b0)};
    enc.xq_shared = i == 0; enc.q_ready = i == 0 ? m->dec0_query : nullptr; enc.kv_ready = g.n_ahead > 0;
    enc.keys = &p.sp; enc.keys_packed = p.packed; enc.xkv_dense = p.x;
    enc.act = p.dec_act; enc.prec = p.prec;
    LAMP_CK(mha_attend(enc, sc, p.s));
    LAMP_CK(mha_tail(enc, sc, &f1, pk, &ffn_ran, p.s));
    if (!ffn_ran) LAMP_CK(ffn_core(f1, p.s));

    ffn_ran = false;
    if (l.slf_attn.present) {
        LAMP_CK(int_pred(p));
        MhaCall slf{Y, Y, p.nb, L, L, d, g.dk, g.dv, &l.slf_attn, &p.label_mask, Y,
                    p.aux && p.aux->dec_self_attn ? p.aux->dec_self_attn[i] : nullptr, p.B, int(p.b0)};
        slf.act = p.dec_act; slf.prec = p.prec;
        LAMP_CK(mha_attend(slf, w.mha, p.s));
        LAMP_CK(mha_tail(slf, w.mha, &f2, pk ? pk + 1 : nullptr, &ffn_ran, p.s));
    }
    if (!ffn_ran) LAMP_CK(ffn_core(f2, p.s));
    if (last && !fused_readout) LAMP_CK(launch_diag(Y, m->w_out, p.nb, L, d, p.logits + p.b0 * L, p.s));
    if (!last) LAMP_CK(int_pred(p));
    return 0;
}

static int onehot_check(const lamp_model* m, const lamp_onehot_frontend* fe, int32_t T) {
    if (!m || !fe) return LAMP_E_NULL;
    if (!fe->t1 || !fe->conv1_b || !fe->conv2_b || (!fe->conv2_w && !fe->conv2_pack)) return LAMP_E_NULL;
    if (fe->n_vocab <= 0 || fe->n_vocab > 16 || fe->taps != 16 || T < 2 || m->d_model <= 0) return LAMP_E_DIMS;
    if (!m->position_enc) return LAMP_E_NULL;
    if (m->enc0_emb_w1 || (m->d_model & 3)) return LAMP_E_UNSUPPORTED;
    return 0;
}

static int check_forward(const lamp_model* m, const lamp_onehot_frontend* fe, const int64_t* src_seq, const int64_t* src_pos,
                         int32_t B, int32_t T_in, const float* logits, const float* enc_output, const lamp_aux* aux,
                         const void* workspace, FwdDims* g, const lamp_fwd_options* o = nullptr) {
    if (fwd_matmul_prec(o) < 0) return LAMP_E_UNSUPPORTED;
    if (fe) LAMP_CK(onehot_check(m, fe, T_in));
    if (!m || !src_seq || (fe && !src_pos) || !logits || !enc_output || !workspace) return LAMP_E_NULL;
    if (B <= 0 || T_in <= 0) return LAMP_E_DIMS;
    if ((!fe && !m->src_word_emb) || !m->tgt_word_emb || !m->w_out) return LAMP_E_NULL;
    if (m->position_enc && !src_pos) return LAMP_E_NULL;
    if (m->enc0_emb_w1 && m->position_enc && !m->enc0_pos_w1) return LAMP_E_NULL;
    if (m->n_layers_dec <= 0) return LAMP_E_DIMS;
    LAMP_CK(fwd_dims(m, fe, T_in, aux && aux->enc_self_attn, g, o && o->enc_self_attn));
    if (g->live) {
        if (m->enc0_emb_w1) return LAMP_E_UNSUPPORTED;
        for (int i = 0; i < m->n_layers_enc; ++i) {
            const lamp_mha_weights& a = m->enc_layers[i].slf_attn;
            if (!a.w_qs || !a.w_ks || !a.w_vs || !a.ln_g || !a.ln_b || (a.n_head > 1 && !a.fc)) return LAMP_E_NULL;
            if (a.n_head < 1 || (a.n_head == 1 && m->d_v != m->d_model)) return LAMP_E_DIMS;
        }
    }
    if (o && o->enc_mask) {
        LAMP_CK(check_mask(o->enc_mask));
        if (o->enc_mask->kind != LAMP_MASK_U8 || o->enc_mask->stride_b == 0 || o->enc_mask->tile_list) return LAMP_E_UNSUPPORTED;
        if (!g->live && !(aux && aux->enc_self_attn)) return LAMP_E_UNSUPPORTED;
    }
    if (o && (o->flags & LAMP_FWD_LABEL_BIAS)) {
        if ((o->flags & LAMP_FWD_DEC_SIGMOID) || m->label_mask_bits || m->label_tiles || m->label_mask_flags ||
            m->label_mask_allowed)
            return LAMP_E_UNSUPPORTED;
        if (m->label_mask && !aligned16(m->label_mask)) return LAMP_E_ALIGN;
    }
    if ((m->d_model & 3) || (m->d_inner & 3) || (m->d_k & 3) || (m->d_v & 3)) return LAMP_E_UNSUPPORTED;
    if (fe && ((fe->conv2_pack && !aligned16(fe->conv2_pack)) || (!fe->conv2_pack && !aligned16(fe->conv2_w)) ||
               !aligned16(fe->t1) || !aligned16(fe->conv1_b) || !aligned16(workspace)))
        return LAMP_E_ALIGN;
    return 0;
}

static int forward(const lamp_model* m, const lamp_onehot_frontend* fe, const FwdDims& g, const int64_t* src_seq,
                   const int64_t* src_pos, int32_t B, int32_t T_in, float* logits, float* enc_output, const lamp_aux* aux,
                   void* workspace, size_t workspace_bytes, hipStream_t s, const lamp_fwd_options* o = nullptr) {
    const Carver size = fwd_size(g);
    if (workspace_bytes < size.bound(1)) return LAMP_E_WORKSPACE;
    const int64_t mb = std::min<int64_t>(B, (workspace_bytes - size.fixed) / size.per);
    Carver c{static_cast<char*>(workspace), size_t(mb)};
    FwdScratch w{};
    fwd_layout(g, c, w);
    if (fe) {
        if (g.w2_repack) LAMP_CK(launch_conv_pack(fe->conv2_w, g.d, g.d, 16, 0, w.w2, s));
        else w.w2 = const_cast<float*>(fe->conv2_pack);
    }

    bool packed_live = g.live && o && (o->flags & LAMP_FWD_PACKED_ENCODER) && !o->enc_mask && g.dk == g.dv &&
                       attn_ragged_applies(g.T, g.dk, g.dv);
    for (int i = 0; i < m->n_layers_enc && packed_live; ++i) packed_live = m->enc_layers[i].slf_attn.n_head > 1;
    const bool packed = !(aux && aux->enc_self_attn) && !wide_heads(g.dk, g.dv) && m->n_layers_enc > 0 && !fe &&
                        (!g.live || packed_live);
    const int L = g.L;
    lamp_mask label_mask{LAMP_MASK_NONE, 0, nullptr, 0, 0, nullptr, 0};
    if (o && (o->flags & LAMP_FWD_LABEL_BIAS)) {
        if (m->label_mask)
            label_mask = lamp_mask{LAMP_MASK_BIAS_F32, 0, m->label_mask, 0, (L + 3) & ~3, nullptr, 0};
    } else if (m->label_mask_bits)
        label_mask = lamp_mask{LAMP_MASK_BITS_U32, m->label_mask_flags, m->label_mask_bits, 0, (L + 31) / 32, m->label_tiles,
                               (L + 31) / 32 + 1, m->label_mask_allowed};
    else if (m->label_mask)
        label_mask = lamp_mask{LAMP_MASK_U8, 0, m->label_mask, 0, L, m->label_tiles, (L + 31) / 32 + 1};
    for (int64_t b0 = 0; b0 < B; b0 += mb) {
        const int nb = int(std::min<int64_t>(B - b0, mb));
        const int64_t* seq = src_seq + b0 * T_in;
        Pass p{m, fe, g, w, aux, logits, s, B, nb, b0, seq, src_pos ? src_pos + b0 * T_in : nullptr, T_in,
               enc_output + b0 * int64_t(g.T) * g.d, packed, plan_from(w.plan_ints, nb, g.T),
               lamp_mask{LAMP_MASK_KEY_TOKENS_I64, 0, seq, T_in, 0, nullptr, 0}, label_mask};
        p.sp.granules = packed ? w.granules : nullptr;
        lamp_mask enc_mask = p.pad_mask;
        if (o && o->enc_mask) {
            enc_mask = *o->enc_mask;
            enc_mask.ptr = static_cast<const uint8_t*>(enc_mask.ptr) + b0 * enc_mask.stride_b;
        }
        if (g.live) enc_mask.flags |= LAMP_MASK_SELF_RAGGED;
        p.enc_mask = &enc_mask;
        p.enc_packs = o ? o->enc_chain_packs : nullptr;
        p.dec_act = (o && (o->flags & LAMP_FWD_DEC_SIGMOID)) ? LAMP_ATTN_SIGMOID : LAMP_ATTN_SOFTMAX;
        p.prec = fwd_matmul_prec(o);
        LAMP_CK(!packed ? encode_padded(p) : g.live ? encode_packed_live(p) : encode_packed(p));
        if (g.n_ahead)
            LAMP_CK(project_kv_layers(p.xk, int64_t(nb) * g.T, g.d, g.dk, g.dv, m->dec_layers, g.n_ahead, w.K_ahead,
                                      w.V_ahead, p.prec, s, packed ? p.sp.rows : nullptr, packed ? p.x : nullptr));
        for (int i = 0; i < m->n_layers_dec; ++i) LAMP_CK(decoder_layer(p, i));
    }
    return 0;
}

size_t lamp_forward_workspace_bytes(const lamp_model* m, int32_t micro_batch, int32_t T, int32_t want_attn) {
    FwdDims g;
    if (micro_batch <= 0 || fwd_dims(m, nullptr, T, want_attn != 0, &g) != 0) return 0;
    return fwd_size(g).bound(micro_batch);
}

static int forward_tokens(const lamp_model* m, const lamp_fwd_options* o, const int64_t* src_seq, const int64_t* src_pos,
                          int32_t B, int32_t T, float* logits, float* enc_output, const lamp_aux* aux, void* workspace,
                          size_t workspace_bytes, lamp_stream_t stream) {
    FwdDims g;
    LAMP_CK(check_forward(m, nullptr, src_seq, src_pos, B, T, logits, enc_output, aux, workspace, &g, o));
    if (workspace_bytes < fwd_size(g).bound(1)) return LAMP_E_WORKSPACE;
    const bool kv_ahead =
        2 * m->n_layers_dec <= GEMM_MAX_SEG && m->n_layers_dec > 1 && workspace_bytes >= fwd_size(g).bound(size_t(B));
    if (!kv_ahead) g.n_ahead = 0;
    return forward(m, nullptr, g, src_seq, src_pos, B, T, logits, enc_output, aux, workspace, workspace_bytes,
                   hipStream_t(stream), o);
}

int lamp_forward(const lamp_model* m, const int64_t* src_seq, const int64_t* src_pos, int32_t B, int32_t T,
                 float* logits, float* enc_output, const lamp_aux* aux, void* workspace, size_t workspace_bytes,
                 lamp_stream_t stream) {
    return forward_tokens(m, nullptr, src_seq, src_pos, B, T, logits, enc_output, aux, workspace, workspace_bytes, stream);
}

size_t lamp_forward_opts_workspace_bytes(const lamp_model* m, const lamp_fwd_options* opts, int32_t micro_batch, int32_t T,
                                         int32_t want_attn) {
    FwdDims g;
    if (micro_batch <= 0 || fwd_dims(m, nullptr, T, want_attn != 0, &g, opts && opts->enc_self_attn) != 0) return 0;
    return fwd_size(g).bound(micro_batch);
}

int lamp_forward_opts(const lamp_model* m, const lamp_fwd_options* opts, const int64_t* src_seq, const int64_t* src_pos,
                      int32_t B, int32_t T, float* logits, float* enc_output, const lamp_aux* aux, void* workspace,
                      size_t workspace_bytes, lamp_stream_t stream) {
    return forward_tokens(m, opts, src_seq, src_pos, B, T, logits, enc_output, aux, workspace, workspace_bytes, stream);
}

size_t lamp_onehot_forward_workspace_bytes(const lamp_model* m, const lamp_onehot_frontend* fe, int32_t micro_batch, int32_t T,
                                           int32_t want_attn) {
    FwdDims g;
    if (micro_batch <= 0 || onehot_check(m, fe, T) != 0 || fwd_dims(m, fe, T, want_attn != 0, &g) != 0) return 0;
    return fwd_size(g).bound(micro_batch);
}

int lamp_onehot_forward(const lamp_model* m, const lamp_onehot_frontend* fe, const int64_t* src_seq, const int64_t* src_pos,
                        int32_t B, int32_t T, float* logits, float* enc_output, const lamp_aux* aux, void* workspace,
                        size_t workspace_bytes, lamp_stream_t stream) {
    return lamp_onehot_forward_opts(m, fe, nullptr, src_seq, src_pos, B, T, logits, enc_output, aux, workspace, workspace_bytes,
                                    stream);
}

size_t lamp_onehot_forward_opts_workspace_bytes(const lamp_model* m, const lamp_onehot_frontend* fe, const lamp_fwd_options* opts,
                                                int32_t micro_batch, int32_t T, int32_t want_attn) {
    FwdDims g;
    if (micro_batch <= 0 || onehot_check(m, fe, T) != 0 ||
        fwd_dims(m, fe, T, want_attn != 0, &g, opts && opts->enc_self_attn) != 0)
        return 0;
    return fwd_size(g).bound(micro_batch);
}

int lamp_onehot_forward_opts(const lamp_model* m, const lamp_onehot_frontend* fe, const lamp_fwd_options* opts,
                             const int64_t* src_seq, const int64_t* src_pos, int32_t B, int32_t T, float* logits,
                             float* enc_output, const lamp_aux* aux, void* workspace, size_t workspace_bytes,
                             lamp_stream_t stream) {
    FwdDims g;
    LAMP_CK(check_forward(m, fe, src_seq, src_pos, B, T, logits, enc_output, aux, workspace, &g, opts));
    return forward(m, fe, g, src_seq, src_pos, B, T, logits, enc_output, aux, workspace, workspace_bytes, hipStream_t(stream),
                   opts);
}

int lamp_conv_pack(const float* w, int32_t c_out, int32_t c_in, int32_t taps, int32_t flip, float* packed,
                   lamp_stream_t stream) {
    return launch_conv_pack(w, c_out, c_in, taps, flip, packed, hipStream_t(stream));
}

int lamp_onehot_front_fwd(const int64_t* src_seq, int32_t B, int32_t T, const lamp_onehot_frontend* fe, int32_t d_model,
                          float dropout_p, uint32_t seed, float* xpad, lamp_stream_t stream) {
    if (!fe) return LAMP_E_NULL;
    return launch_front_fwd(src_seq, B, T, fe->t1, fe->n_vocab, fe->conv1_b, d_model, dropout_p, seed, 0, xpad,
                            hipStream_t(stream));
}

int lamp_conv_window_fwd(const float* xpad, int32_t B, int32_t rows_out, int32_t rows_in, int32_t c_in, const float* w_pack,
                         int32_t c_out, const float* bias, int32_t relu, const float* pos_table, int32_t n_position,
                         const int64_t* src_pos, int64_t pos_ld, float* out, float* relu_out, lamp_stream_t stream) {
    if (B <= 0) return LAMP_E_DIMS;
    ConvWindowParams p{xpad, w_pack, bias, out, relu_out, pos_table, src_pos, int64_t(B) * rows_out, c_out, pos_ld,
                       c_out, 16 * c_in, c_in, rows_out, rows_in, relu != 0, n_position};
    return launch_conv_window(p, hipStream_t(stream));
}

int lamp_conv_relu_bwd_pad(const float* dy, const float* relu_out, int32_t B, int32_t rows, int32_t d, float* dz,
                           lamp_stream_t stream) {
    return launch_relu_bwd_pad(dy, relu_out, B, rows, d, dz, hipStream_t(stream));
}

size_t lamp_onehot_front_bwd_partials_bytes(int32_t B, int32_t T, int32_t n_vocab, int32_t d_model) {
    if (B <= 0 || T <= 0 || n_vocab <= 0 || d_model <= 0) return 0;
    return size_t(front_dt1_chunks(B, T)) * n_vocab * 16 * d_model * sizeof(float);
}

int lamp_onehot_front_bwd(const int64_t* src_seq, int32_t B, int32_t T, const lamp_onehot_frontend* fe, int32_t d_model,
                          float dropout_p, uint32_t seed, const float* dP, float* dz, float* partials, size_t partials_bytes,
                          lamp_stream_t stream) {
    if (!fe) return LAMP_E_NULL;
    if (partials_bytes < lamp_onehot_front_bwd_partials_bytes(B, T, fe->n_vocab, d_model)) return LAMP_E_WORKSPACE;
    return launch_front_bwd(src_seq, B, T, fe->t1, fe->n_vocab, fe->conv1_b, d_model, dropout_p, seed, dP, dz, partials,
                            hipStream_t(stream));
}

int lamp_prof_enable(int32_t on) {
    std::lock_guard<std::mutex> lk(g_prof_mu);
    g_prof_on = on != 0;
    return 0;
}

int lamp_prof_reset(void) {
    std::lock_guard<std::mutex> lk(g_prof_mu);
// ... 34 lines not shown
```

### lamp_amd/csrc/gemm.hip

```cpp
#include <type_traits>

#include "lamp_kernels.h"

namespace lamp {

struct FastDiv {
    unsigned mul, shift;
};
static inline FastDiv make_fastdiv(unsigned d) {
    if (d <= 1) return FastDiv{0u, 0u};
    unsigned l = 0;
    while ((1ull << l) < d) ++l;
    return FastDiv{unsigned(((1ull << (31 + l)) + d - 1) / d), l - 1};
}
__device__ __forceinline__ int fdiv(int n, FastDiv f) { return f.mul ? int(__umulhi(unsigned(n), f.mul) >> f.shift) : n; }
__device__ __forceinline__ int div_1_to_8(int n, int d) {
    if ((d & (d - 1)) == 0) return n >> (31 - __builtin_clz(unsigned(d)));
    const unsigned mul = d == 5 ? 0xCCCCCCCDu : (d == 7 ? 0x92492493u : 0xAAAAAAABu);
    return int(__umulhi(unsigned(n), mul) >> (d == 3 ? 1 : 2));
}

constexpr int gemm_min_waves(int bm, int bn, int bk, int mf) { return (mf == 16 && bm == 64 && bn == 64 && bk == 16) ? 5 : 1; }

template <int BM, int BN, int BK, int WAVES_M, int WAVES_N, int MF = 32>
struct GemmTile {
    static constexpr int NT = WAVES_M * WAVES_N * 64;
    static constexpr int WTM = BM / WAVES_M;
    static constexpr int WTN = BN / WAVES_N;
    static constexpr int MI = WTM / MF;
    static constexpr int NI = WTN / MF;
#ifndef LAMP_LDS_PAD16
#define LAMP_LDS_PAD16 8
#endif
    static constexpr int LDS_STRIDE = BK + (MF == 16 ? LAMP_LDS_PAD16 : 4);
    static constexpr int A_LD = BM * BK / 4 / NT;
    static constexpr int B_LD = BN * BK / 4 / NT;
    static constexpr size_t LDS_BYTES = size_t(2) * (BM + BN) * LDS_STRIDE * sizeof(float);
    static constexpr int MIN_WAVES = gemm_min_waves(BM, BN, BK, MF);
    static_assert(MF == 32 || MF == 16, "MFMA block edge");
    static_assert(WTM % MF == 0 && WTN % MF == 0, "wave tile must be a multiple of the MFMA block");
    static_assert(BK % (MF == 32 ? 8 : 16) == 0, "BK must cover whole fragment reads");
    static_assert((BM * BK / 4) % NT == 0 && (BN * BK / 4) % NT == 0, "staging must divide evenly");
    static_assert(BK % 8 == 0, "BK must be a multiple of 8");
};


__device__ __forceinline__ const float* uniform_ptr(const float* q) {
    const uint64_t b = reinterpret_cast<uint64_t>(q);
    const unsigned lo = __builtin_amdgcn_readfirstlane(unsigned(b)), hi = __builtin_amdgcn_readfirstlane(unsigned(b >> 32));
    return reinterpret_cast<const float*>((uint64_t(hi) << 32) | lo);
}
template <int BM, int BN, int BK, int WAVES_M, int WAVES_N, bool KTAIL, int MF, bool RPRE, bool VEC, bool RGATHER>
__device__ __forceinline__ void gemm_body(const GemmParams& p, int tiles_n_seg, int tiles_n, int tiles_m, int panel_split,
                                          FastDiv fd_group, FastDiv fd_seg) {
    using T = GemmTile<BM, BN, BK, WAVES_M, WAVES_N, MF>;
    constexpr int KQ = 64 / MF;
    constexpr int KCH = 4 * KQ;
    constexpr int NACC = MF == 32 ? 16 : 4;
    using acc_t = typename std::conditional<MF == 32, f32x16, f32x4>::type;
    constexpr int S = T::LDS_STRIDE;
    constexpr int C4 = BK / 4;
    extern __shared__ __attribute__((aligned(16))) float smem[];
    float* As = smem;
    float* Bs = smem + 2 * BM * S;

    const int tid = threadIdx.x;
    const int lane = tid & 63;
    const int wave = tid >> 6;
    const int wm = wave / WAVES_N, wn = wave % WAVES_N;
    const int l31 = lane & (MF - 1), hi = lane / MF;

#ifdef LAMP_TUNING
    const unsigned long long t_entry = p.trace ? wall_clock64() : 0ull;
#endif
    constexpr int GROUP_M = 8;
    int64_t M = p.M;
    if (p.m_dev) {
        M = *p.m_dev;
        if (M > p.M) M = p.M;
        tiles_m = int((M + BM - 1) / BM);
        const int nwg = tiles_m * tiles_n, pan_xcd = (tiles_m + 7) >> 3;
        panel_split = tiles_m >= 16 && (pan_xcd * tiles_n + 31) / 32 <= ((nwg + 7) / 8 + 31) / 32;
    }
    int item = 0, pan0 = 0, pan1 = tiles_m;
    int tn_all = 0, tm = 0;
    if (panel_split) {
        const int q = tiles_m >> 3, r = tiles_m & 7, xcd = blockIdx.x & 7;
        pan0 = xcd * q + (xcd < r ? xcd : r);
        pan1 = pan0 + q + (xcd < r ? 1 : 0);
        item = blockIdx.x >> 3;
        if (item >= (pan1 - pan0) * tiles_n) return;
    } else {
        const int nwg = p.m_dev ? tiles_m * tiles_n : int(gridDim.x);
        if (int(blockIdx.x) >= nwg) return;
        item = xcd_remap(blockIdx.x, nwg);
        pan0 = 0;
        pan1 = tiles_m;
    }
    if (p.walk_gn > 0) {
        const int rows = pan1 - pan0;
        const int group_sz = rows * p.walk_gn;
        const int grp = item / group_sz;
        const int in_grp = item - grp * group_sz;
        const int first_n = grp * p.walk_gn;
        const int gn = tiles_n - first_n < p.walk_gn ? tiles_n - first_n : p.walk_gn;
        const int tml = in_grp / gn;
        tm = pan0 + tml;
        tn_all = first_n + (in_grp - tml * gn);
    } else {
        const int group_sz = GROUP_M * tiles_n;
        const int grp = fdiv(item, fd_group);
        const int in_grp = item - grp * group_sz;
        const int first_m = pan0 + grp * GROUP_M;
        const int gm = pan1 - first_m < GROUP_M ? pan1 - first_m : GROUP_M;
        tn_all = div_1_to_8(in_grp, gm);
        tm = first_m + (in_grp - tn_all * gm);
    }
    const int seg = fdiv(tn_all, fd_seg);
    const int tn = tn_all - seg * tiles_n_seg;
    const int64_t m0 = int64_t(tm) * BM;
    const int n0 = tn * BN;
    const int rows_m = int(M - m0 < BM ? M - m0 : BM);
    const int rows_n = p.N - n0 < BN ? p.N - n0 : BN;

    const int lda = int(p.lda), ldw = int(p.ldw);
    const float* Abase = p.A;
    if (p.A_dense) {
        if (p.m_dev[0] == p.m_dev[1]) Abase = p.A_dense;
    }
    const __amdgpu_buffer_rsrc_t rsA =
        make_rsrc(uniform_ptr(Abase + m0 * p.lda), __builtin_amdgcn_readfirstlane(unsigned((uint64_t(rows_m - 1) * lda + p.K) * 4u)));
    const __amdgpu_buffer_rsrc_t rsW =
        make_rsrc(uniform_ptr(p.W[seg] + int64_t(n0) * p.ldw), __builtin_amdgcn_readfirstlane(unsigned((uint64_t(rows_n - 1) * ldw + p.K) * 4u)));

    acc_t acc[T::MI][T::NI];
#pragma unroll
    for (int i = 0; i < T::MI; ++i)
#pragma unroll
        for (int j = 0; j < T::NI; ++j)
#pragma unroll
            for (int r = 0; r < NACC; ++r) acc[i][j][r] = 0.f;

    float4 ra0[T::A_LD], rb0[T::B_LD], ra1[T::A_LD], rb1[T::B_LD];
    unsigned voa[T::A_LD], vob[T::B_LD];
#pragma unroll
    for (int i = 0; i < T::A_LD; ++i) {
        const int idx = tid + i * T::NT;
        const int row = idx / C4, c4 = idx - row * C4;
        voa[i] = unsigned(row * lda + c4 * 4) * 4u;
    }
#pragma unroll
    for (int i = 0; i < T::B_LD; ++i) {
        const int idx = tid + i * T::NT;
        const int row = idx / C4, c4 = idx - row * C4;
        vob[i] = unsigned(row * ldw + c4 * 4) * 4u;
    }

    auto gload = [&](int k0, float4 (&ra)[T::A_LD], float4 (&rb)[T::B_LD]) {
        if constexpr (KTAIL) {
#pragma unroll
            for (int i = 0; i < T::A_LD; ++i) {
                const int k = k0 + ((tid + i * T::NT) % C4) * 4;
                ra[i] = bload4(rsA, k < p.K ? voa[i] + unsigned(k0) * 4u : OOB, 0);
            }
#pragma unroll
            for (int i = 0; i < T::B_LD; ++i) {
                const int k = k0 + ((tid + i * T::NT) % C4) * 4;
                rb[i] = bload4(rsW, k < p.K ? vob[i] + unsigned(k0) * 4u : OOB, 0);
            }
        } else {
            const unsigned so = unsigned(k0) * 4u;
#pragma unroll
            for (int i = 0; i < T::A_LD; ++i) ra[i] = bload4(rsA, voa[i], so);
#pragma unroll
            for (int i = 0; i < T::B_LD; ++i) rb[i] = bload4(rsW, vob[i], so);
        }
    };
    auto lstore = [&](int buf, const float4 (&ra)[T::A_LD], const float4 (&rb)[T::B_LD]) {
        float* a = As + buf * BM * S;
        float* b = Bs + buf * BN * S;
#pragma unroll
        for (int i = 0; i < T::A_LD; ++i) {
            const int idx = tid + i * T::NT;
            const int row = idx / C4, c4 = idx - row * C4;
            *reinterpret_cast<float4*>(a + row * S + c4 * 4) = ra[i];
        }
#pragma unroll
        for (int i = 0; i < T::B_LD; ++i) {
            const int idx = tid + i * T::NT;
            const int row = idx / C4, c4 = idx - row * C4;
            *reinterpret_cast<float4*>(b + row * S + c4 * 4) = rb[i];
        }
    };
    auto mfma_chunk = [&](const float4 (&fa)[T::MI], const float4 (&fb)[T::NI]) {
#ifdef LAMP_SETPRIO
        __builtin_amdgcn_s_setprio(1);
#endif
#pragma unroll
        for (int i = 0; i < T::MI; ++i)
#pragma unroll
            for (int j = 0; j < T::NI; ++j) {
                if constexpr (MF == 32) {
                    acc[i][j] = __builtin_amdgcn_mfma_f32_32x32x2f32(fb[j].x, fa[i].x, acc[i][j], 0, 0, 0);
                    acc[i][j] = __builtin_amdgcn_mfma_f32_32x32x2f32(fb[j].y, fa[i].y, acc[i][j], 0, 0, 0);
                    acc[i][j] = __builtin_amdgcn_mfma_f32_32x32x2f32(fb[j].z, fa[i].z, acc[i][j], 0, 0, 0);
                    acc[i][j] = __builtin_amdgcn_mfma_f32_32x32x2f32(fb[j].w, fa[i].w, acc[i][j], 0, 0, 0);
                } else {
                    acc[i][j] = __builtin_amdgcn_mfma_f32_16x16x4f32(fb[j].x, fa[i].x, acc[i][j], 0, 0, 0);
                    acc[i][j] = __builtin_amdgcn_mfma_f32_16x16x4f32(fb[j].y, fa[i].y, acc[i][j], 0, 0, 0);
                    acc[i][j] = __builtin_amdgcn_mfma_f32_16x16x4f32(fb[j].z, fa[i].z, acc[i][j], 0, 0, 0);
                    acc[i][j] = __builtin_amdgcn_mfma_f32_16x16x4f32(fb[j].w, fa[i].w, acc[i][j], 0, 0, 0);
                }
            }
#ifdef LAMP_SETPRIO
        __builtin_amdgcn_s_setprio(0);
#endif
    };
    auto compute = [&](int buf) {
        const float* a = As + buf * BM * S + (wm * T::WTM + l31) * S + hi * 4;
        const float* b = Bs + buf * BN * S + (wn * T::WTN + l31) * S + hi * 4;
#pragma unroll
        for (int c = 0; c < BK / KCH; ++c) {
            float4 fa[T::MI], fb[T::NI];
#pragma unroll
            for (int i = 0; i < T::MI; ++i) fa[i] = *reinterpret_cast<const float4*>(a + i * MF * S + c * KCH);
#pragma unroll
            for (int j = 0; j < T::NI; ++j) fb[j] = *reinterpret_cast<const float4*>(b + j * MF * S + c * KCH);
            mfma_chunk(fa, fb);
        }
    };

    const int nk = (p.K + BK - 1) / BK;
    gload(0, ra0, rb0);

    const int ldc = int(p.ldc), ldr = int(p.ldr);
    const bool has_r = RGATHER || p.R != nullptr;
    const bool read_r = !RGATHER && p.R != nullptr;
    const __amdgpu_buffer_rsrc_t rsR =
        make_rsrc(read_r ? p.R + m0 * p.ldr + n0 : p.A, read_r ? (uint64_t(rows_m - 1) * ldr + rows_n) * 4u : 0);
    const float* bias = p.bias[seg];
    const __amdgpu_buffer_rsrc_t rsBias = make_rsrc(bias ? bias + n0 : p.A, bias ? uint64_t(rows_n) * 4u : 0);
    constexpr int NQ = NACC / 4;
    constexpr bool vec = VEC;
    const int lrow0 = wm * T::WTM + l31;
    const int lcol0 = wn * T::WTN + 4 * hi;
    auto load4 = [&](__amdgpu_buffer_rsrc_t rs, unsigned off, int lcol) -> float4 {
        if constexpr (vec) return bload4(rs, lcol < rows_n ? off * 4u : OOB, 0);
        float4 v;
        v.x = bload1(rs, lcol + 0 < rows_n ? (off + 0) * 4u : OOB);
        v.y = bload1(rs, lcol + 1 < rows_n ? (off + 1) * 4u : OOB);
        v.z = bload1(rs, lcol + 2 < rows_n ? (off + 2) * 4u : OOB);
        v.w = bload1(rs, lcol + 3 < rows_n ? (off + 3) * 4u : OOB);
        return v;
    };
    const float* ge[RGATHER ? T::MI : 1];
    const float* gp[RGATHER ? T::MI : 1];
    if constexpr (RGATHER) {
#pragma unroll
        for (int i = 0; i < T::MI; ++i) {
            const int lrow = lrow0 + i * MF;
            const bool in = lrow < rows_m;
            const int tk = in ? p.rg_tok[m0 + lrow] : 0, ps = (in && p.rg_pos_table) ? p.rg_pos[m0 + lrow] : 0;
            ge[i] = p.rg_emb + int64_t(tk) * p.N + n0;
            gp[i] = p.rg_pos_table ? p.rg_pos_table + int64_t(ps) * p.N + n0 : nullptr;
        }
    }
    auto gathered = [&](int i, int lcol) -> float4 {
        if constexpr (RGATHER) {
            if (lcol >= rows_n) return make_float4(0.f, 0.f, 0.f, 0.f);
            float4 v = *reinterpret_cast<const float4*>(ge[i] + lcol);
            if (gp[i]) {
                const float4 w = *reinterpret_cast<const float4*>(gp[i] + lcol);
                v.x += w.x; v.y += w.y; v.z += w.z; v.w += w.w;
            }
            return v;
        }
        return make_float4(0.f, 0.f, 0.f, 0.f);
    };
    constexpr int NPRE = RPRE ? T::MI * T::NI * NQ : 1;
    float4 pre_r[NPRE], pre_b[RPRE ? T::NI * NQ : 1];
    if constexpr (RPRE) {
#pragma unroll
        for (int j = 0; j < T::NI; ++j)
#pragma unroll
            for (int q = 0; q < NQ; ++q) {
                const int lcol = lcol0 + j * MF + 8 * q;
                pre_b[j * NQ + q] = load4(rsBias, unsigned(lcol), lcol);
#pragma unroll
                for (int i = 0; i < T::MI; ++i)
                    pre_r[(j * T::MI + i) * NQ + q] = RGATHER ? gathered(i, lcol) : load4(rsR, unsigned((lrow0 + i * MF) * ldr + lcol), lcol);
            }
    }

    lstore(0, ra0, rb0);
    if (nk > 1) gload(BK, ra0, rb0);
    if (nk > 2) gload(2 * BK, ra1, rb1);
    __syncthreads();
#ifdef LAMP_TUNING
    const unsigned long long t_loop = p.trace ? wall_clock64() : 0ull;
    const unsigned long long c_loop = p.trace ? __builtin_readcyclecounter() : 0ull;
#endif

    for (int kt = 0; kt < nk; kt += 2) {
        compute(0);
        if (kt + 1 < nk) lstore(1, ra0, rb0);
        if (kt + 3 < nk) gload((kt + 3) * BK, ra0, rb0);
        __syncthreads();
        if (kt + 1 >= nk) break;
        compute(1);
        if (kt + 2 < nk) lstore(0, ra1, rb1);
        if (kt + 4 < nk) gload((kt + 4) * BK, ra1, rb1);
        __syncthreads();
    }
#ifdef LAMP_TUNING
    const unsigned long long t_epi = p.trace ? wall_clock64() : 0ull;
    const unsigned long long c_epi = p.trace ? __builtin_readcyclecounter() : 0ull;
#endif

    const __amdgpu_buffer_rsrc_t rsC =
        make_rsrc(p.C[seg] + m0 * p.ldc + n0, (uint64_t(rows_m - 1) * ldc + rows_n) * 4u);
    auto relu1 = [](float x) {
        float y;
        asm("v_max_f32 %0, 0, %1" : "=v"(y) : "v"(x));
        return y;
    };
    auto emit = [&](auto with_r, auto with_relu) {
        constexpr bool WITH_R = decltype(with_r)::value, WITH_RELU = decltype(with_relu)::value;
    #pragma unroll
        for (int i = 0; i < T::MI; ++i) {
            const int lrow = lrow0 + i * MF;
    #pragma unroll
            for (int j = 0; j < T::NI; ++j)
    #pragma unroll
                for (int q = 0; q < NQ; ++q) {
                    const int lcol = lcol0 + j * MF + 8 * q;
                    float4 bv, res = make_float4(0.f, 0.f, 0.f, 0.f);
                    if constexpr (RPRE) {
                        bv = pre_b[j * NQ + q];
                        res = pre_r[(j * T::MI + i) * NQ + q];
                    } else {
                        bv = load4(rsBias, unsigned(lcol), lcol);
                        if constexpr (WITH_R) res = RGATHER ? gathered(i, lcol) : load4(rsR, unsigned(lrow * ldr + lcol), lcol);
                    }
                    float4 v = make_float4(acc[i][j][4 * q + 0] + bv.x, acc[i][j][4 * q + 1] + bv.y,
                                           acc[i][j][4 * q + 2] + bv.z, acc[i][j][4 * q + 3] + bv.w);
                    if constexpr (WITH_RELU) v = make_float4(relu1(v.x), relu1(v.y), relu1(v.z), relu1(v.w));
                    if constexpr (WITH_R) v = make_float4(v.x + res.x, v.y + res.y, v.z + res.z, v.w + res.w);
                    const unsigned off = unsigned(lrow * ldc + lcol);
                    if constexpr (vec) {
                        bstore4(rsC, lcol < rows_n ? off * 4u : OOB, v);
                    } else {
                        bstore1(rsC, lcol + 0 < rows_n ? (off + 0) * 4u : OOB, v.x);
                        bstore1(rsC, lcol + 1 < rows_n ? (off + 1) * 4u : OOB, v.y);
                        bstore1(rsC, lcol + 2 < rows_n ? (off + 2) * 4u : OOB, v.z);
                        bstore1(rsC, lcol + 3 < rows_n ? (off + 3) * 4u : OOB, v.w);
                    }
                }
        }
    };
    if (has_r) {
        if (p.relu) emit(std::true_type{}, std::true_type{});
        else emit(std::true_type{}, std::false_type{});
    } else {
        if (p.relu) emit(std::false_type{}, std::true_type{});
        else emit(std::false_type{}, std::false_type{});
    }
#ifdef LAMP_TUNING
    if (p.trace && tid == 0) {
        unsigned long long* t = p.trace + size_t(blockIdx.x) * 8;
        t[0] = t_entry; t[1] = t_loop; t[2] = t_epi; t[3] = wall_clock64();
        t[4] = __builtin_amdgcn_s_getreg((31 << 11) | 4);
        t[5] = __builtin_amdgcn_s_getreg((31 << 11) | 20);
        t[6] = unsigned(item);
        t[7] = c_epi - c_loop;
    }
#endif
}

template <int BM, int BN, int BK, int WAVES_M, int WAVES_N, bool KTAIL, int MF, bool RPRE, bool VEC, bool RGATHER = false>
__global__ __launch_bounds__(WAVES_M* WAVES_N * 64, (gemm_min_waves(BM, BN, BK, MF))) void gemm_nt_kernel(GemmParams p, int tiles_n_seg,
                                                                          int tiles_n, int tiles_m,
                                                                          int panel_split, FastDiv fd_group,
                                                                          FastDiv fd_seg) {
    gemm_body<BM, BN, BK, WAVES_M, WAVES_N, KTAIL, MF, RPRE, VEC, RGATHER>(p, tiles_n_seg, tiles_n, tiles_m, panel_split, fd_group, fd_seg);
}

#ifdef LAMP_TUNING
static int g_force_walk = -1;
extern "C" __attribute__((visibility("default"))) void lamp_debug_force_gemm_walk(int gn) { g_force_walk = gn; }
static long long g_trace_slab_words = 0;
static size_t g_extra_lds = 0;
extern "C" __attribute__((visibility("default"))) void lamp_debug_set_gemm_extra_lds(int bytes) { g_extra_lds = size_t(bytes); }
#endif

template <int BM, int BN, int BK, int WAVES_M, int WAVES_N, bool KTAIL, int MF, bool VEC, bool RGATHER = false>
static int launch_cfg2(const GemmParams& p, hipStream_t s) {
    using T = GemmTile<BM, BN, BK, WAVES_M, WAVES_N, MF>;
    constexpr bool RPRE = T::MI * T::NI * (MF == 32 ? 16 : 4) <= 16;
    auto kern = gemm_nt_kernel<BM, BN, BK, WAVES_M, WAVES_N, KTAIL, MF, RPRE, VEC, RGATHER>;
    size_t LDS = T::LDS_BYTES;
    static AttrOnce once;
#ifdef LAMP_TUNING
    LDS += g_extra_lds;
    if (int e = once.set(reinterpret_cast<const void*>(kern), 160 * 1024)) return e;
#else
    if (int e = once.set(reinterpret_cast<const void*>(kern), LDS)) return e;
#endif
    const int64_t ldmax = p.lda > p.ldw ? (p.lda > p.ldc ? p.lda : p.ldc) : (p.ldw > p.ldc ? p.ldw : p.ldc);
    if (ldmax * (BM > BN ? BM : BN) * 4 >= 0x7fffffffLL || (p.R && p.ldr * BM * 4 >= 0x7fffffffLL))
        return LAMP_E_UNSUPPORTED;
    const int64_t tiles_m = (p.M + BM - 1) / BM;
    const int tiles_n_seg = (p.N + BN - 1) / BN;
    const int tiles_n = tiles_n_seg * p.nseg;
    int64_t nwg = tiles_m * tiles_n;
    const int64_t pan_xcd = (tiles_m + 7) / 8;
    int panel_split = tiles_m >= 16 && (pan_xcd * tiles_n + 31) / 32 <= ((nwg + 7) / 8 + 31) / 32;
    if (panel_split) nwg = 8 * pan_xcd * tiles_n;
    if (p.m_dev) {
        const int64_t split_grid = 8 * pan_xcd * tiles_n;
        if (split_grid > nwg) nwg = split_grid;
        panel_split = 0;
    }
    if (nwg > 0x7fffffffLL) return LAMP_E_DIMS;
    GemmParams q = p;
    q.walk_gn = (int64_t(p.nseg) * p.N * p.K * 4 >= (8ll << 20) && tiles_n > 8) ? 8 : 0;
#ifdef LAMP_TUNING
    if (p.trace && nwg * 8 > g_trace_slab_words) return LAMP_E_WORKSPACE;
    if (g_force_walk >= 0) q.walk_gn = g_force_walk < tiles_n ? g_force_walk : tiles_n;
#endif
    hipLaunchKernelGGL(kern, dim3((unsigned)nwg), dim3(T::NT), LDS, s, q, tiles_n_seg, tiles_n, int(tiles_m),
                       panel_split, make_fastdiv(unsigned(8 * tiles_n)), make_fastdiv(unsigned(tiles_n_seg)));
    return int(hipGetLastError());
}

template <int BM, int BN, int BK, int WAVES_M, int WAVES_N, int MF = 32>
static int launch_cfg(const GemmParams& p, hipStream_t s) {
    if (p.rg_tok) {
        if (!p.vec_epilogue || (p.K % BK)) return LAMP_E_UNSUPPORTED;
        return launch_cfg2<BM, BN, BK, WAVES_M, WAVES_N, false, MF, true, true>(p, s);
    }
    if (p.vec_epilogue) {
        if (p.K % BK) return launch_cfg2<BM, BN, BK, WAVES_M, WAVES_N, true, MF, true>(p, s);
        return launch_cfg2<BM, BN, BK, WAVES_M, WAVES_N, false, MF, true>(p, s);
    }
    if (p.K % BK) return launch_cfg2<BM, BN, BK, WAVES_M, WAVES_N, true, MF, false>(p, s);
    return launch_cfg2<BM, BN, BK, WAVES_M, WAVES_N, false, MF, false>(p, s);
}

#ifdef LAMP_TUNING
static int g_force_tile = 0;
static unsigned long long* g_gemm_trace = nullptr;
static long long g_trace_slab = 0;
static int g_trace_slabs = 0, g_trace_count = 0;
extern "C" __attribute__((visibility("default"))) void lamp_debug_force_gemm_tile(int cfg) { g_force_tile = cfg; }
extern "C" __attribute__((visibility("default"))) void lamp_debug_set_gemm_trace(unsigned long long* buf, long long slab_words, int n_slabs) {
    g_gemm_trace = buf;
    g_trace_slab = slab_words;
    g_trace_slab_words = slab_words;
    g_trace_slabs = n_slabs;
    g_trace_count = 0;
}
#endif

bool gemm_gathered_residual_ok(int N, int K, int64_t ldc, const float* bias, const float* C, const float* emb, const float* pos_table) {
    return N > 0 && !(N & 3) && K > 0 && (K % 32) == 0 && !(ldc & 3) && aligned16(C) && (!bias || aligned16(bias)) && emb && aligned16(emb) &&
           (!pos_table || aligned16(pos_table));
}

int launch_gemm(const GemmParams& p_in, hipStream_t s) {
    GemmParams p = p_in;
    if (p.M <= 0 || p.N <= 0 || p.K <= 0 || p.nseg < 1 || p.nseg > GEMM_MAX_SEG) return LAMP_E_DIMS;
    if ((p.K & 3) || (p.lda & 3) || (p.ldw & 3)) return LAMP_E_ALIGN;
    if (!p.A || (p.A_dense && !p.m_dev)) return LAMP_E_NULL;
    if (p.rg_tok && (p.R || !p.rg_emb || p.nseg != 1 || (p.rg_pos_table && !p.rg_pos))) return LAMP_E_UNSUPPORTED;
    if (p.rg_tok && (!aligned16(p.rg_emb) || (p.rg_pos_table && !aligned16(p.rg_pos_table)))) return LAMP_E_ALIGN;
    if (!aligned16(p.A) || (p.A_dense && !aligned16(p.A_dense))) return LAMP_E_ALIGN;
    for (int i = 0; i < p.nseg; ++i) {
        if (!p.W[i] || !p.C[i]) return LAMP_E_NULL;
        if (!aligned16(p.W[i])) return LAMP_E_ALIGN;
    }
    const double flops = 2.0 * double(p.M) * p.N * p.nseg * p.K;
    const double bytes = 4.0 * (double(p.M) * p.K + double(p.N) * p.nseg * p.K +
                                double(p.M) * p.N * p.nseg * ((p.R || p.rg_tok) ? 2 : 1));
    ProfScope prof(LAMP_K_GEMM, flops, bytes, s);
    p.trace = nullptr;
    bool vec = !(p.N & 3) && !(p.ldc & 3) && (!p.R || (!(p.ldr & 3) && aligned16(p.R)));
    for (int i = 0; i < p.nseg; ++i) vec = vec && aligned16(p.C[i]) && (!p.bias[i] || aligned16(p.bias[i]));
    p.vec_epilogue = vec ? 1 : 0;
#ifdef LAMP_TUNING
    if (g_gemm_trace && g_trace_slabs > 0) {
        const long long wg_max = ((p.M + 31) / 32) * ((p.N + 63) / 64) * p.nseg;
        if (wg_max * 8 <= g_trace_slab) p.trace = g_gemm_trace + (g_trace_count % g_trace_slabs) * g_trace_slab;
        ++g_trace_count;
    }
    switch (g_force_tile) {
        case 1: return launch_cfg<128, 128, 32, 2, 2>(p, s);
        case 2: return launch_cfg<64, 64, 32, 2, 2>(p, s);
        case 3: return launch_cfg<128, 64, 32, 2, 2>(p, s);
        case 4: return launch_cfg<64, 128, 32, 2, 2>(p, s);
        case 5: return launch_cfg<128, 128, 16, 2, 2>(p, s);
        case 6: return launch_cfg<64, 64, 16, 2, 2>(p, s);
        case 7: return launch_cfg<128, 64, 16, 2, 2>(p, s);
        case 8: return launch_cfg<256, 128, 16, 4, 2>(p, s);
        case 9: return launch_cfg<32, 64, 32, 1, 4, 16>(p, s);
        case 10: return launch_cfg<64, 32, 32, 4, 1, 16>(p, s);
        case 11: return launch_cfg<64, 64, 16, 2, 2, 16>(p, s);
        case 12: return launch_cfg<64, 64, 32, 2, 2, 16>(p, s);
        case 13: return launch_cfg<32, 128, 32, 1, 4, 16>(p, s);
        case 14: return launch_cfg<128, 128, 32, 2, 2, 16>(p, s);
        case 15: return launch_cfg<128, 128, 16, 2, 2, 16>(p, s);
        case 16: return launch_cfg<128, 64, 32, 2, 2, 16>(p, s);
        case 17: return launch_cfg<64, 128, 32, 2, 2, 16>(p, s);
        case 18: return launch_cfg<128, 64, 16, 2, 2, 16>(p, s);
        default: break;
    }
#endif
    auto tiles = [&](int bm, int bn) { return ((p.M + bm - 1) / bm) * ((p.N + bn - 1) / bn) * p.nseg; };
    const int64_t t64 = tiles(64, 64);
    if (tiles(128, 64) >= 2048 && p.K >= 512) return launch_cfg<128, 64, 16, 2, 2, 16>(p, s);
    if (t64 >= 2048) return launch_cfg<64, 64, 32, 2, 2, 16>(p, s);
    if (t64 >= 1200) return launch_cfg<64, 64, 16, 2, 2, 16>(p, s);
    return launch_cfg<32, 64, 32, 1, 4, 16>(p, s);
}

}
```

### lamp_amd/csrc/lamp_kernels.h

```cpp
#pragma once
#include <hip/hip_runtime.h>
#include <stdint.h>

#include <mutex>
#include "../../include/lamp_hip.h"

typedef float f32x16 __attribute__((ext_vector_type(16)));
typedef float f32x4 __attribute__((ext_vector_type(4)));

namespace lamp {

constexpr int GEMM_MAX_SEG = 4;

struct GemmParams {
    const float* A;
    int64_t lda;
    int64_t M;
    int K;
    int N;
    int nseg;
    const float* W[GEMM_MAX_SEG];
    int64_t ldw;
    const float* bias[GEMM_MAX_SEG];
    float* C[GEMM_MAX_SEG];
    int64_t ldc;
    const float* R;
    int64_t ldr;
    int relu;
    const int* rg_tok;
    const int* rg_pos;
    const float* rg_emb;
    const float* rg_pos_table;
    const int* m_dev;
    const float* A_dense;
    int vec_epilogue;
    int walk_gn;
    unsigned long long* trace;
};

struct AttnParams {
    const float* Q;
    const float* K;
    const float* V;
    float* O;
    float* P;
    float* lse;
    float* scratch;
    int B, H, lq, lk, dk, dv;
    int P_batch, P_b0;
    lamp_attn_layout lay;
    float scale_log2e;
    int mask_kind;
    const void* mask;
    int64_t m_sb, m_sq;
    const int* tiles;
    int64_t tiles_stride;
    int self_ragged;
    int sparse_rows;
    int64_t allowed_pairs;
    const int* kv_len;
    const int* kv_off;
    unsigned long long* trace;
    int act;
};

int launch_gemm(const GemmParams& p, hipStream_t s);
int launch_gemm_split(const GemmParams& p, int nprod, hipStream_t s);
bool gemm_gathered_residual_ok(int N, int K, int64_t ldc, const float* bias, const float* C, const float* emb, const float* pos_table);
bool slab_applies(int64_t M, int N, int K, int nseg, const float* const* Wq);
int launch_slab_gemm(const GemmParams& p, const float* const* Wq, hipStream_t s);
int launch_attn(const AttnParams& p, hipStream_t s);
int launch_attn_general(const AttnParams& p, hipStream_t s);
bool attn_small_applies(const AttnParams& p, bool any_lq = false);
int launch_attn_small(const AttnParams& p, int force_ksplit, hipStream_t s);
bool attn_tile_applies(const AttnParams& p);
int launch_attn_tile(const AttnParams& p, hipStream_t s);
bool attn_sparse_applies(const AttnParams& p);
int launch_attn_sparse(const AttnParams& p, hipStream_t s);
int launch_attn_sigmoid(const AttnParams& p, hipStream_t s);
int launch_attn_bias(const AttnParams& p, hipStream_t s);
size_t gemm_gen_workspace_bytes(int M, int N, int K, int batch);
int launch_gemm_gen(const lamp_gemm_desc& d, void* ws, size_t ws_bytes, hipStream_t s);
int launch_gemm_group(const lamp_gemm_desc* descs, int n, hipStream_t s);
struct DropoutSpec {
    unsigned threshold;
    float scale;
    unsigned seed;
};
inline DropoutSpec make_dropout(float p, uint32_t seed) {
    const double t = double(p) * 4294967296.0;
    return DropoutSpec{t >= 4294967295.0 ? 4294967295u : unsigned(t), 1.0f / (1.0f - p), seed};
}
__device__ __forceinline__ unsigned mix32(unsigned lo, unsigned hi, unsigned seed) {
    unsigned h = lo ^ (hi * 0x9E3779B9u) ^ seed;
    h ^= h >> 16; h *= 0x7feb352du;
    h ^= h >> 15; h *= 0x846ca68bu;
    h ^= h >> 16;
    return h;
}
__device__ __forceinline__ float drop1(float v, int64_t e, const DropoutSpec& d) {
    return mix32(unsigned(e), unsigned(uint64_t(e) >> 32), d.seed) >= d.threshold ? v * d.scale : 0.f;
}
__device__ __forceinline__ float4 drop4(float4 v, int64_t e, const DropoutSpec& d) {
    return make_float4(drop1(v.x, e, d), drop1(v.y, e + 1, d), drop1(v.z, e + 2, d), drop1(v.w, e + 3, d));
// ... 219 lines not shown
```

Before: 45330.

## Add pre-packed weight GEMM path loading B fragments directly into registers

Adds a WPACK variant of the NT GEMM kernel that reads weights from a pre-packed MFMA fragment layout straight into registers, skipping the LDS staging of the weight tile. The model now builds packed copies of the encoder FFN and decoder query/self-attention projection weights and routes the forward pass through a new lamp_forward_packs entry point. The dispatcher also sends medium-sized GEMMs that would have used the 64x64 tile to the packed 32x64 kernel instead. The aim is lower LDS traffic and footprint for the small-M GEMMs, at the cost of extra weight memory, more registers, and a pack step whenever the weights change.

```diff
diff --git a/include/lamp_hip.h b/include/lamp_hip.h
--- a/include/lamp_hip.h
+++ b/include/lamp_hip.h
@@ -142,6 +142,10 @@
                          const float* residual, int64_t ldr, int32_t relu,
                          float* C, int64_t ldc, int32_t precision, lamp_stream_t stream);
 
+int lamp_linear_packed_fwd(const float* A, int64_t M, int32_t K, int64_t lda, const float* const* W, const float* const* W_pack,
+                           int32_t n_seg, int32_t N, int64_t ldw, const float* const* bias, const float* residual, int64_t ldr,
+                           int32_t relu, float* const* C, int64_t ldc, const int32_t* m_dev, lamp_stream_t stream);
+
 int lamp_layernorm_fwd(const float* x, int64_t M, int32_t d, const float* gamma, const float* beta,
                        float eps, float* y, lamp_stream_t stream);
 
@@ -321,6 +325,25 @@
                       int32_t B, int32_t T, float* logits, float* enc_output, const lamp_aux* aux, void* workspace,
                       size_t workspace_bytes, lamp_stream_t stream);
 
+typedef struct lamp_dec_gemm_pack {
+    const float* enc_q;
+    const float* slf_q;
+    const float* slf_k;
+    const float* slf_v;
+} lamp_dec_gemm_pack;
+typedef struct lamp_enc_gemm_pack {
+    const float* w1;
+    const float* w2;
+} lamp_enc_gemm_pack;
+typedef struct lamp_gemm_packs {
+    const lamp_enc_gemm_pack* enc;
+    const lamp_dec_gemm_pack* dec;
+} lamp_gemm_packs;
+
+int lamp_forward_packs(const lamp_model* m, const lamp_fwd_options* opts, const lamp_gemm_packs* packs, const int64_t* src_seq,
+                       const int64_t* src_pos, int32_t B, int32_t T, float* logits, float* enc_output, const lamp_aux* aux,
+                       void* workspace, size_t workspace_bytes, lamp_stream_t stream);
+
 typedef struct lamp_onehot_frontend {
     const float* t1;
     const float* conv1_b;
diff --git a/lamp_amd/Models.py b/lamp_amd/Models.py
--- a/lamp_amd/Models.py
+++ b/lamp_amd/Models.py
@@ -194,6 +194,15 @@
                 out += [l.slf_attn.fc.weight, l.pos_ffn.w_1.weight, l.pos_ffn.w_2.weight]
         return out
 
+    def _gemm_pack_weights(self):
+        enc = [(l.pos_ffn.w_1.weight, l.pos_ffn.w_2.weight) for l in self.encoder.layer_stack]
+        dec = []
+        for l in self.decoder.layer_stack:
+            slf = getattr(l, 'slf_attn', None)
+            dec.append((l.enc_attn.w_qs.weight,) + (tuple(getattr(slf, n).weight for n in ('w_qs', 'w_ks', 'w_vs')) if slf is not None
+                                                     else (None, None, None)))
+        return enc, dec
+
     def _native_model(self):
         replica = getattr(self, '_is_replica', False)
         params = None if replica else self._param_list
@@ -211,10 +220,11 @@
         packs = self.use_chain_packs and not replica
         onehot = bool(getattr(self.encoder, 'onehot', False))
         live = self.enc_self_attn
+        gpacks = bool(self.use_gemm_packs and not replica and not onehot and getattr(N.lib(), 'lamp_forward_packs', None))
         fold = self.fold_embedding and not replica and len(self.encoder.layer_stack) > 0 and not onehot and not live
         sparse = bool(self.use_sparse_label_attention and self.use_mask_bits and self.decoder.label_rows_sparse and bias is None)
         key = tuple(p.data_ptr() for p in params) + (N.ptr(mask), N.ptr(bits), N.ptr(tiles), self.use_label_tiles,
-                                                      hoist, self.use_mask_bits, packs, fold, sparse, live, bias is not None)
+                                                      hoist, self.use_mask_bits, packs, fold, sparse, live, bias is not None, gpacks)
         if hoist:
             l0 = self.decoder.layer_stack[0].enc_attn
             key += (self.decoder.tgt_word_emb.weight._version, l0.w_qs.weight._version)
@@ -222,6 +232,8 @@
             key += tuple(w._version for w in self._chain_weights())
             if live:
                 key += tuple(w._version for w in self._enc_chain_weights())
+        if gpacks:
+            key += tuple(w._version for group in self._gemm_pack_weights() for ws in group for w in ws if w is not None)
         if fold:
             key += tuple(w._version for w in self._fold_weights() if w is not None)
         if onehot:
@@ -277,6 +289,19 @@
                     continue
                 enc_pack_arr[i] = _chain_pack(l.slf_attn.fc.weight, l.pos_ffn.w_1.weight, l.pos_ffn.w_2.weight, pack_keep)
             torch.cuda.current_stream().synchronize()
+        gemm_keep = None
+        if gpacks:
+            enc_ws, dec_ws = self._gemm_pack_weights()
+            tensors = []
+
+            def pk(w):
+                t = N.weight_pack(w, 0) if w is not None else None
+                tensors.append(t)
+                return N.ptr(t)
+            enc_gp = (N.EncGemmPack * max(1, len(enc_ws)))(*[N.EncGemmPack(*[pk(w) for w in ws]) for ws in enc_ws])
+            dec_gp = (N.DecGemmPack * max(1, len(dec_ws)))(*[N.DecGemmPack(*[pk(w) for w in ws]) for ws in dec_ws])
+            gemm_keep = (N.GemmPacks(enc_gp, dec_gp), enc_gp, dec_gp, tensors)
+            torch.cuda.current_stream().synchronize()
         fold_keep = None
         if fold:
             emb_w, pos_w, w1, b1 = self._fold_weights()
@@ -295,7 +320,7 @@
             fe = N.onehot_frontend(t1, b1c, w2c, b2c, w2p)
             onehot_keep = (fe, t1, w2c, b1c, b2c, w2p)
             torch.cuda.current_stream().synchronize()
-        built = (m, enc_arr, dec_arr, q0, pack_arr, pack_keep, fold_keep, onehot_keep, enc_pack_arr)
+        built = (m, enc_arr, dec_arr, q0, pack_arr, pack_keep, fold_keep, onehot_keep, enc_pack_arr, gemm_keep)
         if not replica:
             self._native_cache = (key, built)
         return built
@@ -358,6 +383,7 @@
         built = self._native_model()
         model, enc_arr, dec_arr = built[:3]
         fe = built[7][0] if self.onehot else None
+        gp = built[9][0] if built[9] is not None else None
         T_in = T
         if fe is not None:
             T = T_in // 2
@@ -434,6 +460,11 @@
                                                  T_in, logits.data_ptr(), enc_output.data_ptr(),
                                                  C.byref(aux) if aux is not None else None, ws.data_ptr(), ws.numel(),
                                                  N.stream()), 'lamp_onehot_forward_opts')
+        elif gp is not None and fe is None:
+            N.check(lib.lamp_forward_packs(C.byref(model), C.byref(opts) if opts is not None else None, C.byref(gp), seq.data_ptr(),
+                                           pos.data_ptr(), B, T, logits.data_ptr(), enc_output.data_ptr(),
+                                           C.byref(aux) if aux is not None else None, ws.data_ptr(), ws.numel(), N.stream()),
+                    'lamp_forward_packs')
         elif opts is not None:
             N.check(lib.lamp_forward_opts(C.byref(model), C.byref(opts), seq.data_ptr(), pos.data_ptr(), B, T,
                                           logits.data_ptr(), enc_output.data_ptr(), C.byref(aux) if aux is not None else None,
@@ -456,6 +487,7 @@
     workspace_limit_bytes = 8 << 30
     cache_layer0_query = True
     use_chain_packs = True
+    use_gemm_packs = True
     fold_embedding = True
     matmul_precision = _MatmulPrecision()
     use_packed_live_encoder = False
diff --git a/lamp_amd/_native.py b/lamp_amd/_native.py
--- a/lamp_amd/_native.py
+++ b/lamp_amd/_native.py
@@ -78,6 +78,18 @@
                 ('enc0_emb_w1', _vp), ('enc0_pos_w1', _vp), ('label_mask_allowed', C.c_int64)]
 
 
+class DecGemmPack(C.Structure):
+    _fields_ = [('enc_q', _vp), ('slf_q', _vp), ('slf_k', _vp), ('slf_v', _vp)]
+
+
+class EncGemmPack(C.Structure):
+    _fields_ = [('w1', _vp), ('w2', _vp)]
+
+
+class GemmPacks(C.Structure):
+    _fields_ = [('enc', C.POINTER(EncGemmPack)), ('dec', C.POINTER(DecGemmPack))]
+
+
 class GemmDesc(C.Structure):
     _fields_ = [('A', _vp), ('B', _vp), ('C', _vp), ('M', C.c_int32), ('N', C.c_int32), ('K', C.c_int32),
                 ('batch0', C.c_int32), ('batch1', C.c_int32), ('accumulate', C.c_int32),
@@ -128,6 +140,8 @@
     'lamp_strerror': (C.c_char_p, [C.c_int]),
     'lamp_linear_fwd': (C.c_int, [_vp, _i64, _i32, _i64, _vp, _i32, _i64, _vp, _vp, _i64, _i32, _vp, _i64, _vp]),
     'lamp_linear_prec_fwd': (C.c_int, [_vp, _i64, _i32, _i64, _vp, _i32, _i64, _vp, _vp, _i64, _i32, _vp, _i64, _i32, _vp]),
+    'lamp_linear_packed_fwd': (C.c_int, [_vp, _i64, _i32, _i64, C.POINTER(_vp), C.POINTER(_vp), _i32, _i32, _i64, C.POINTER(_vp), _vp, _i64,
+                                         _i32, C.POINTER(_vp), _i64, _vp, _vp]),
     'lamp_layernorm_fwd': (C.c_int, [_vp, _i64, _i32, _vp, _vp, _f, _vp, _vp]),
     'lamp_sdpa_fwd': (C.c_int, [_vp, _vp, _vp, _vp, _vp, _i32, _i32, _i32, _i32, _i32, _i32, _f,
                                 C.POINTER(Mask), C.POINTER(AttnLayout), _vp]),
@@ -173,6 +187,8 @@
     'lamp_forward_opts_workspace_bytes': (_sz, [C.POINTER(Model), C.POINTER(FwdOptions), _i32, _i32, _i32]),
     'lamp_forward_opts': (C.c_int, [C.POINTER(Model), C.POINTER(FwdOptions), _vp, _vp, _i32, _i32, _vp, _vp, C.POINTER(Aux),
                                     _vp, _sz, _vp]),
+    'lamp_forward_packs': (C.c_int, [C.POINTER(Model), C.POINTER(FwdOptions), C.POINTER(GemmPacks), _vp, _vp, _i32, _i32, _vp, _vp,
+                                     C.POINTER(Aux), _vp, _sz, _vp]),
     'lamp_onehot_forward_opts_workspace_bytes': (_sz, [C.POINTER(Model), C.POINTER(OnehotFrontend), C.POINTER(FwdOptions),
                                                        _i32, _i32, _i32]),
     'lamp_onehot_forward_opts': (C.c_int, [C.POINTER(Model), C.POINTER(OnehotFrontend), C.POINTER(FwdOptions), _vp, _vp, _i32,
@@ -209,6 +225,8 @@
                                  C.POINTER(C.c_double)]),
 }
 
+LATE_ENTRY_POINTS = ('lamp_linear_packed_fwd', 'lamp_forward_packs')
+
 _lib = None
 _lock = threading.Lock()
 
@@ -225,7 +243,7 @@
     if version != ABI_VERSION and not old_ok:
         raise RuntimeError('lamp_amd: ABI version mismatch in ' + path)
     for name, (res, args) in PROTOTYPES.items():
-        if old_ok and not hasattr(handle, name):
+        if (old_ok or name in LATE_ENTRY_POINTS) and not hasattr(handle, name):
             continue
         fn = getattr(handle, name)
         fn.restype = res
@@ -522,6 +540,22 @@
     out = torch.empty(n * k, dtype=torch.float32, device=w.device)
     check(fn(ptr(w), n, k, k, fmt, ptr(out), stream()), 'lamp_pack_weight')
     return out
+
+
+def linear_packed(x, weights, packs=None, biases=None, residual=None, relu=False, m_dev=None, M=None):
+    require_device(x, *weights)
+    x2 = f32c(x).reshape(-1, x.size(-1))
+    M = x2.size(0) if M is None else M
+    K, n, N = x2.size(1), len(weights), weights[0].size(0)
+    ws = [f32c(w.detach()) for w in weights]
+    outs = [torch.zeros((M, N), dtype=torch.float32, device=x.device) for _ in ws]
+    arr = lambda ts: (_vp * n)(*[ptr(t) for t in ts])
+    bs = [f32c(b) if b is not None else None for b in biases] if biases is not None else None
+    res = f32c(residual) if residual is not None else None
+    check(lib().lamp_linear_packed_fwd(ptr(x2), M, K, K, arr(ws), arr(packs) if packs is not None else None, n, N, K,
+                                       arr(bs) if bs is not None else None, ptr(res), N, int(bool(relu)), arr(outs), N,
+                                       ptr(m_dev), stream()), 'lamp_linear_packed_fwd')
+    return outs
 
 
 def diag_logits(y, w_out):
diff --git a/lamp_amd/csrc/api.hip b/lamp_amd/csrc/api.hip
--- a/lamp_amd/csrc/api.hip
+++ b/lamp_amd/csrc/api.hip
@@ -85,7 +85,7 @@
 static int linear(const float* A, int64_t M, int K, int64_t lda, const float* const* W, int nseg, int N,
                   int64_t ldw, const float* const* bias, const float* R, int64_t ldr, int relu,
                   float* const* C, int64_t ldc, int prec, hipStream_t s, const int* m_dev = nullptr,
-                  const float* A_dense = nullptr, const ResGather* rg = nullptr) {
+                  const float* A_dense = nullptr, const ResGather* rg = nullptr, const float* const* Wp = nullptr) {
     GemmParams p{};
     p.A = A; p.lda = lda; p.M = M; p.K = K; p.N = N; p.nseg = nseg; p.ldw = ldw; p.ldc = ldc;
     p.R = R; p.ldr = ldr; p.relu = relu; p.m_dev = m_dev; p.A_dense = A_dense;
@@ -95,6 +95,7 @@
     }
     for (int i = 0; i < nseg; ++i) {
         p.W[i] = W[i];
+        p.Wp[i] = Wp ? Wp[i] : nullptr;
         p.bias[i] = bias ? bias[i] : nullptr;
         p.C[i] = C[i];
     }
@@ -131,17 +132,19 @@
 
 static int project_qkv(const lamp_mha_weights& w, int d, int dk, int dv, const float* xq, int64_t Mq, float* Q,
                        const float* xk, const float* xv, int64_t Mk, float* K, float* V, int prec, hipStream_t s,
-                       const int* m_dev, const float* A_dense) {
+                       const int* m_dev, const float* A_dense, const float* const* Wp = nullptr) {
     const int hdk = w.n_head * dk, hdv = w.n_head * dv;
     const bool one_kv = K && V && xk == xv && hdk == hdv;
     const bool one_qkv = one_kv && Q && xq == xk && Mq == Mk && !m_dev;
     const float* W[3] = {w.w_qs, w.w_ks, w.w_vs};
     float* C[3] = {Q, K, V};
-    if (Q) LAMP_CK(linear(xq, Mq, d, d, W, one_qkv ? 3 : 1, hdk, d, nullptr, nullptr, 0, 0, C, hdk, prec, s));
+    const float* const* P1 = Wp ? Wp + 1 : nullptr;
+    const float* const* P2 = Wp ? Wp + 2 : nullptr;
+    if (Q) LAMP_CK(linear(xq, Mq, d, d, W, one_qkv ? 3 : 1, hdk, d, nullptr, nullptr, 0, 0, C, hdk, prec, s, nullptr, nullptr, nullptr, Wp));
     if (one_qkv) return 0;
-    if (one_kv) return linear(xk, Mk, d, d, W + 1, 2, hdk, d, nullptr, nullptr, 0, 0, C + 1, hdk, prec, s, m_dev, A_dense);
-    if (K) LAMP_CK(linear(xk, Mk, d, d, W + 1, 1, hdk, d, nullptr, nullptr, 0, 0, C + 1, hdk, prec, s, m_dev, A_dense));
-    if (V) LAMP_CK(linear(xv, Mk, d, d, W + 2, 1, hdv, d, nullptr, nullptr, 0, 0, C + 2, hdv, prec, s, m_dev, A_dense));
+    if (one_kv) return linear(xk, Mk, d, d, W + 1, 2, hdk, d, nullptr, nullptr, 0, 0, C + 1, hdk, prec, s, m_dev, A_dense, nullptr, P1);
+    if (K) LAMP_CK(linear(xk, Mk, d, d, W + 1, 1, hdk, d, nullptr, nullptr, 0, 0, C + 1, hdk, prec, s, m_dev, A_dense, nullptr, P1));
+    if (V) LAMP_CK(linear(xv, Mk, d, d, W + 2, 1, hdv, d, nullptr, nullptr, 0, 0, C + 2, hdv, prec, s, m_dev, A_dense, nullptr, P2));
     return 0;
 }
 
@@ -161,6 +164,7 @@
     bool hidden_ready = false;
     const ResGather* rg = nullptr;
     int prec = LAMP_PREC_FP32;
+    const float *w1_pack = nullptr, *w2_pack = nullptr;
 };
 
 static int ffn_core(const FfnParams& f, hipStream_t s) {
@@ -172,13 +176,15 @@
         const float* W[1] = {w.w1};
         const float* b[1] = {w.b1};
         float* C[1] = {f.hidden};
-        LAMP_CK(linear(f.x, f.M, d, d, W, 1, dff, d, b, nullptr, 0, 1, C, dff, f.prec, s, f.rows_dev));
+        const float* P[1] = {f.w1_pack};
+        LAMP_CK(linear(f.x, f.M, d, d, W, 1, dff, d, b, nullptr, 0, 1, C, dff, f.prec, s, f.rows_dev, nullptr, nullptr, P));
     }
     {
         const float* W[1] = {w.w2};
         const float* b[1] = {w.b2};
         float* C[1] = {f.out};
-        LAMP_CK(linear(f.hidden, f.M, dff, dff, W, 1, d, dff, b, f.x, d, 0, C, d, f.prec, s, f.rows_dev, nullptr, f.rg));
+        const float* P[1] = {f.w2_pack};
+        LAMP_CK(linear(f.hidden, f.M, dff, dff, W, 1, d, dff, b, f.x, d, 0, C, d, f.prec, s, f.rows_dev, nullptr, f.rg, P));
     }
     LayerNormParams ln{f.out, f.M, d, w.ln_g, w.ln_b, f.out};
     if (f.scatter) {
@@ -230,6 +236,7 @@
     const float* xkv_dense = nullptr;
     int act = LAMP_ATTN_SOFTMAX;
     int prec = LAMP_PREC_FP32;
+    const float* const* w_packs = nullptr;
 };
 
 
@@ -245,7 +252,7 @@
     const bool kv = !c.kv_ready;
     LAMP_CK(project_qkv(w, d, dk, dv, c.xq, c.xq_shared ? lq : int64_t(B) * lq, c.q_ready ? nullptr : sc.Q, c.xkv, c.xkv,
                         int64_t(B) * lk, kv ? sc.K : nullptr, kv && need_v ? sc.V : nullptr, c.prec, s,
-                        c.keys_packed ? c.keys->rows : nullptr, c.keys_packed ? c.xkv_dense : nullptr));
+                        c.keys_packed ? c.keys->rows : nullptr, c.keys_packed ? c.xkv_dense : nullptr, c.w_packs));
 
     const lamp_mask* mask = c.mask;
     const SeqPlan* keys = c.keys;
@@ -376,6 +383,15 @@
     float* Cs[1] = {C};
     if (lda < K || ldw < K || ldc < N || (residual && ldr < N)) return LAMP_E_DIMS;
     return linear(A, M, K, lda, Ws, 1, N, ldw, bs, residual, ldr, relu, Cs, ldc, precision, hipStream_t(stream));
+}
+
+int lamp_linear_packed_fwd(const float* A, int64_t M, int32_t K, int64_t lda, const float* const* W, const float* const* W_pack,
+                           int32_t n_seg, int32_t N, int64_t ldw, const float* const* bias, const float* residual, int64_t ldr,
+                           int32_t relu, float* const* C, int64_t ldc, const int32_t* m_dev, lamp_stream_t stream) {
+    if (!W || !C) return LAMP_E_NULL;
+    if (n_seg < 1 || n_seg > GEMM_MAX_SEG || lda < K || ldw < K || ldc < N || (residual && ldr < N)) return LAMP_E_DIMS;
+    return linear(A, M, K, lda, W, n_seg, N, ldw, bias, residual, ldr, relu, C, ldc, LAMP_PREC_FP32, hipStream_t(stream), m_dev,
+                  nullptr, nullptr, W_pack);
 }
 
 int lamp_layernorm_fwd(const float* x, int64_t M, int32_t d, const float* gamma, const float* beta, float eps,
@@ -912,6 +928,10 @@
     const lamp_chain_pack* enc_packs = nullptr;
     int dec_act = LAMP_ATTN_SOFTMAX;
     int prec = LAMP_PREC_FP32;
+    const lamp_gemm_packs* gp = nullptr;
+    void ffn_packs(FfnParams& f, int layer) const {
+        if (gp && gp->enc) { f.w1_pack = gp->enc[layer].w1; f.w2_pack = gp->enc[layer].w2; }
+    }
 };
 
 static int encode_packed(Pass& p) {
@@ -931,6 +951,7 @@
         f.prec = p.prec;
         f.rows_dev = p.sp.rows + 1; f.hidden_ready = folded && i == 0; f.rg = gather_res && i == 0 ? &rg : nullptr;
         if (i + 1 == m->n_layers_enc) { f.scatter = &p.sp; f.nb = p.nb; f.T = T; f.y_flat = p.x; }
+        p.ffn_packs(f, i);
         LAMP_CK(ffn_core(f, p.s));
     }
     p.xk = w.Xp;
@@ -961,6 +982,7 @@
         LAMP_CK(launch_layernorm(ln, p.s));
         FfnParams f{w.Xp, Mub, d, dff, &m->enc_layers[i].pos_ffn, w.Xp, w.H};
         f.rows_dev = w.live_rows; f.prec = p.prec;
+        p.ffn_packs(f, i);
         LAMP_CK(ffn_core(f, p.s));
     }
     LAMP_CK(launch_scatter_rows(w.Xp, d, p.nb, T, p.sp, p.x, p.s));
@@ -996,6 +1018,7 @@
         float* map = p.aux && p.aux->enc_self_attn ? p.aux->enc_self_attn[i] : nullptr;
         FfnParams f{p.x, Me, d, dff, &l.pos_ffn, p.x, w.H};
         f.prec = p.prec;
+        p.ffn_packs(f, i);
         if (p.g.live) {
             MhaCall a{p.x, p.x, p.nb, T, T, d, p.g.dk, p.g.dv, &l.slf_attn, p.enc_mask, p.x, map, p.B, int(p.b0)};
             a.keys = &p.sp; a.prec = p.prec;
@@ -1070,6 +1093,10 @@
     enc.xq_shared = i == 0; enc.q_ready = i == 0 ? m->dec0_query : nullptr; enc.kv_ready = g.n_ahead > 0;
     enc.keys = &p.sp; enc.keys_packed = p.packed; enc.xkv_dense = p.x;
     enc.act = p.dec_act; enc.prec = p.prec;
+    const lamp_dec_gemm_pack* dp = p.gp && p.gp->dec ? p.gp->dec + i : nullptr;
+    const float* enc_pk[3] = {dp ? dp->enc_q : nullptr, nullptr, nullptr};
+    const float* slf_pk[3] = {dp ? dp->slf_q : nullptr, dp ? dp->slf_k : nullptr, dp ? dp->slf_v : nullptr};
+    enc.w_packs = enc_pk;
     LAMP_CK(mha_attend(enc, sc, p.s));
     LAMP_CK(mha_tail(enc, sc, &f1, pk, &ffn_ran, p.s));
     if (!ffn_ran) LAMP_CK(ffn_core(f1, p.s));
@@ -1079,7 +1106,7 @@
         LAMP_CK(int_pred(p));
         MhaCall slf{Y, Y, p.nb, L, L, d, g.dk, g.dv, &l.slf_attn, &p.label_mask, Y,
                     p.aux && p.aux->dec_self_attn ? p.aux->dec_self_attn[i] : nullptr, p.B, int(p.b0)};
-        slf.act = p.dec_act; slf.prec = p.prec;
+        slf.act = p.dec_act; slf.prec = p.prec; slf.w_packs = slf_pk;
         LAMP_CK(mha_attend(slf, w.mha, p.s));
         LAMP_CK(mha_tail(slf, w.mha, &f2, pk ? pk + 1 : nullptr, &ffn_ran, p.s));
     }
@@ -1138,7 +1165,8 @@
 
 static int forward(const lamp_model* m, const lamp_onehot_frontend* fe, const FwdDims& g, const int64_t* src_seq,
                    const int64_t* src_pos, int32_t B, int32_t T_in, float* logits, float* enc_output, const lamp_aux* aux,
-                   void* workspace, size_t workspace_bytes, hipStream_t s, const lamp_fwd_options* o = nullptr) {
+                   void* workspace, size_t workspace_bytes, hipStream_t s, const lamp_fwd_options* o = nullptr,
+                   const lamp_gemm_packs* gp = nullptr) {
     const Carver size = fwd_size(g);
     if (workspace_bytes < size.bound(1)) return LAMP_E_WORKSPACE;
     const int64_t mb = std::min<int64_t>(B, (workspace_bytes - size.fixed) / size.per);
@@ -1182,6 +1210,7 @@
         p.enc_packs = o ? o->enc_chain_packs : nullptr;
         p.dec_act = (o && (o->flags & LAMP_FWD_DEC_SIGMOID)) ? LAMP_ATTN_SIGMOID : LAMP_ATTN_SOFTMAX;
         p.prec = fwd_matmul_prec(o);
+        p.gp = gp;
         LAMP_CK(!packed ? encode_padded(p) : g.live ? encode_packed_live(p) : encode_packed(p));
         if (g.n_ahead)
             LAMP_CK(project_kv_layers(p.xk, int64_t(nb) * g.T, g.d, g.dk, g.dv, m->dec_layers, g.n_ahead, w.K_ahead,
@@ -1199,7 +1228,7 @@
 
 static int forward_tokens(const lamp_model* m, const lamp_fwd_options* o, const int64_t* src_seq, const int64_t* src_pos,
                           int32_t B, int32_t T, float* logits, float* enc_output, const lamp_aux* aux, void* workspace,
-                          size_t workspace_bytes, lamp_stream_t stream) {
+                          size_t workspace_bytes, lamp_stream_t stream, const lamp_gemm_packs* gp = nullptr) {
     FwdDims g;
     LAMP_CK(check_forward(m, nullptr, src_seq, src_pos, B, T, logits, enc_output, aux, workspace, &g, o));
     if (workspace_bytes < fwd_size(g).bound(1)) return LAMP_E_WORKSPACE;
@@ -1207,7 +1236,7 @@
         2 * m->n_layers_dec <= GEMM_MAX_SEG && m->n_layers_dec > 1 && workspace_bytes >= fwd_size(g).bound(size_t(B));
     if (!kv_ahead) g.n_ahead = 0;
     return forward(m, nullptr, g, src_seq, src_pos, B, T, logits, enc_output, aux, workspace, workspace_bytes,
-                   hipStream_t(stream), o);
+                   hipStream_t(stream), o, gp);
 }
 
 int lamp_forward(const lamp_model* m, const int64_t* src_seq, const int64_t* src_pos, int32_t B, int32_t T,
@@ -1227,6 +1256,12 @@
                       int32_t B, int32_t T, float* logits, float* enc_output, const lamp_aux* aux, void* workspace,
                       size_t workspace_bytes, lamp_stream_t stream) {
     return forward_tokens(m, opts, src_seq, src_pos, B, T, logits, enc_output, aux, workspace, workspace_bytes, stream);
+}
+
+int lamp_forward_packs(const lamp_model* m, const lamp_fwd_options* opts, const lamp_gemm_packs* packs, const int64_t* src_seq,
+                       const int64_t* src_pos, int32_t B, int32_t T, float* logits, float* enc_output, const lamp_aux* aux,
+                       void* workspace, size_t workspace_bytes, lamp_stream_t stream) {
+    return forward_tokens(m, opts, src_seq, src_pos, B, T, logits, enc_output, aux, workspace, workspace_bytes, stream, packs);
 }
 
 size_t lamp_onehot_forward_workspace_bytes(const lamp_model* m, const lamp_onehot_frontend* fe, int32_t micro_batch, int32_t T,
diff --git a/lamp_amd/csrc/gemm.hip b/lamp_amd/csrc/gemm.hip
--- a/lamp_amd/csrc/gemm.hip
+++ b/lamp_amd/csrc/gemm.hip
@@ -20,9 +20,11 @@
     return int(__umulhi(unsigned(n), mul) >> (d == 3 ? 1 : 2));
 }
 
-constexpr int gemm_min_waves(int bm, int bn, int bk, int mf) { return (mf == 16 && bm == 64 && bn == 64 && bk == 16) ? 5 : 1; }
-
-template <int BM, int BN, int BK, int WAVES_M, int WAVES_N, int MF = 32>
+constexpr int gemm_min_waves(int bm, int bn, int bk, int mf, bool wpack = false) {
+    return (wpack || (mf == 16 && bm == 64 && bn == 64 && bk == 16)) ? 5 : 1;
+}
+
+template <int BM, int BN, int BK, int WAVES_M, int WAVES_N, int MF = 32, bool WPACK = false>
 struct GemmTile {
     static constexpr int NT = WAVES_M * WAVES_N * 64;
     static constexpr int WTM = BM / WAVES_M;
@@ -35,8 +37,9 @@
     static constexpr int LDS_STRIDE = BK + (MF == 16 ? LAMP_LDS_PAD16 : 4);
     static constexpr int A_LD = BM * BK / 4 / NT;
     static constexpr int B_LD = BN * BK / 4 / NT;
-    static constexpr size_t LDS_BYTES = size_t(2) * (BM + BN) * LDS_STRIDE * sizeof(float);
-    static constexpr int MIN_WAVES = gemm_min_waves(BM, BN, BK, MF);
+    static constexpr size_t LDS_BYTES = size_t(2) * (BM + (WPACK ? 0 : BN)) * LDS_STRIDE * sizeof(float);
+    static constexpr size_t LDS_LAUNCH_BYTES = WPACK ? size_t(2) * (BM + BN) * LDS_STRIDE * sizeof(float) : LDS_BYTES;
+    static constexpr int MIN_WAVES = gemm_min_waves(BM, BN, BK, MF, WPACK);
     static_assert(MF == 32 || MF == 16, "MFMA block edge");
     static_assert(WTM % MF == 0 && WTN % MF == 0, "wave tile must be a multiple of the MFMA block");
     static_assert(BK % (MF == 32 ? 8 : 16) == 0, "BK must cover whole fragment reads");
@@ -50,10 +53,11 @@
     const unsigned lo = __builtin_amdgcn_readfirstlane(unsigned(b)), hi = __builtin_amdgcn_readfirstlane(unsigned(b >> 32));
     return reinterpret_cast<const float*>((uint64_t(hi) << 32) | lo);
 }
-template <int BM, int BN, int BK, int WAVES_M, int WAVES_N, bool KTAIL, int MF, bool RPRE, bool VEC, bool RGATHER>
+template <int BM, int BN, int BK, int WAVES_M, int WAVES_N, bool KTAIL, int MF, bool RPRE, bool VEC, bool RGATHER, bool WPACK>
 __device__ __forceinline__ void gemm_body(const GemmParams& p, int tiles_n_seg, int tiles_n, int tiles_m, int panel_split,
                                           FastDiv fd_group, FastDiv fd_seg) {
-    using T = GemmTile<BM, BN, BK, WAVES_M, WAVES_N, MF>;
+    using T = GemmTile<BM, BN, BK, WAVES_M, WAVES_N, MF, WPACK>;
+    static_assert(!WPACK || (MF == 16 && BK == 32 && WAVES_M == 1 && !KTAIL), "packed W: 16x16x4 fragments of whole 32-deep k-tiles, one wave row");
     constexpr int KQ = 64 / MF;
     constexpr int KCH = 4 * KQ;
     constexpr int NACC = MF == 32 ? 16 : 4;
@@ -130,8 +134,9 @@
     }
     const __amdgpu_buffer_rsrc_t rsA =
         make_rsrc(uniform_ptr(Abase + m0 * p.lda), __builtin_amdgcn_readfirstlane(unsigned((uint64_t(rows_m - 1) * lda + p.K) * 4u)));
-    const __amdgpu_buffer_rsrc_t rsW =
-        make_rsrc(uniform_ptr(p.W[seg] + int64_t(n0) * p.ldw), __builtin_amdgcn_readfirstlane(unsigned((uint64_t(rows_n - 1) * ldw + p.K) * 4u)));
+    const __amdgpu_buffer_rsrc_t rsW = WPACK
+        ? make_rsrc(uniform_ptr(p.Wp[seg]), __builtin_amdgcn_readfirstlane(unsigned(uint64_t(p.N) * uint64_t(p.K) * 4u)))
+        : make_rsrc(uniform_ptr(p.W[seg] + int64_t(n0) * p.ldw), __builtin_amdgcn_readfirstlane(unsigned((uint64_t(rows_n - 1) * ldw + p.K) * 4u)));
 
     acc_t acc[T::MI][T::NI];
 #pragma unroll
@@ -143,6 +148,21 @@
 
     float4 ra0[T::A_LD], rb0[T::B_LD], ra1[T::A_LD], rb1[T::B_LD];
     unsigned voa[T::A_LD], vob[T::B_LD];
+    constexpr int NWF = WPACK ? (BK / KCH) * T::NI : 1;
+    float4 wf0[NWF], wf1[NWF];
+    unsigned vow[NWF];
+    if constexpr (WPACK) {
+#pragma unroll
+        for (int c = 0; c < BK / KCH; ++c)
+#pragma unroll
+            for (int j = 0; j < T::NI; ++j)
+                vow[c * T::NI + j] = unsigned((n0 + wn * T::WTN + j * MF) >> 4) * unsigned(p.K >> 5) * 2048u + unsigned(c) * 1024u + unsigned(lane) * 16u;
+    }
+    auto wload = [&](int k0, float4 (&wf)[NWF]) {
+        const unsigned so = unsigned(k0) * 64u;
+#pragma unroll
+        for (int x = 0; x < NWF; ++x) wf[x] = bload4(rsW, vow[x], so);
+    };
 #pragma unroll
     for (int i = 0; i < T::A_LD; ++i) {
         const int idx = tid + i * T::NT;
@@ -172,8 +192,10 @@
             const unsigned so = unsigned(k0) * 4u;
 #pragma unroll
             for (int i = 0; i < T::A_LD; ++i) ra[i] = bload4(rsA, voa[i], so);
-#pragma unroll
-            for (int i = 0; i < T::B_LD; ++i) rb[i] = bload4(rsW, vob[i], so);
+            if constexpr (!WPACK) {
+#pragma unroll
+                for (int i = 0; i < T::B_LD; ++i) rb[i] = bload4(rsW, vob[i], so);
+            }
         }
     };
     auto lstore = [&](int buf, const float4 (&ra)[T::A_LD], const float4 (&rb)[T::B_LD]) {
@@ -185,11 +207,13 @@
             const int row = idx / C4, c4 = idx - row * C4;
             *reinterpret_cast<float4*>(a + row * S + c4 * 4) = ra[i];
         }
-#pragma unroll
-        for (int i = 0; i < T::B_LD; ++i) {
-            const int idx = tid + i * T::NT;
-            const int row = idx / C4, c4 = idx - row * C4;
-            *reinterpret_cast<float4*>(b + row * S + c4 * 4) = rb[i];
+        if constexpr (!WPACK) {
+#pragma unroll
+            for (int i = 0; i < T::B_LD; ++i) {
+                const int idx = tid + i * T::NT;
+                const int row = idx / C4, c4 = idx - row * C4;
+                *reinterpret_cast<float4*>(b + row * S + c4 * 4) = rb[i];
+            }
         }
     };
     auto mfma_chunk = [&](const float4 (&fa)[T::MI], const float4 (&fb)[T::NI]) {
@@ -216,7 +240,7 @@
         __builtin_amdgcn_s_setprio(0);
 #endif
     };
-    auto compute = [&](int buf) {
+    auto compute = [&](int buf, const float4 (&wf)[NWF]) {
         const float* a = As + buf * BM * S + (wm * T::WTM + l31) * S + hi * 4;
         const float* b = Bs + buf * BN * S + (wn * T::WTN + l31) * S + hi * 4;
 #pragma unroll
@@ -225,7 +249,10 @@
 #pragma unroll
             for (int i = 0; i < T::MI; ++i) fa[i] = *reinterpret_cast<const float4*>(a + i * MF * S + c * KCH);
 #pragma unroll
-            for (int j = 0; j < T::NI; ++j) fb[j] = *reinterpret_cast<const float4*>(b + j * MF * S + c * KCH);
+            for (int j = 0; j < T::NI; ++j) {
+                if constexpr (WPACK) fb[j] = wf[c * T::NI + j];
+                else fb[j] = *reinterpret_cast<const float4*>(b + j * MF * S + c * KCH);
+            }
             mfma_chunk(fa, fb);
         }
     };
@@ -293,21 +320,45 @@
     }
 
     lstore(0, ra0, rb0);
-    if (nk > 1) gload(BK, ra0, rb0);
-    if (nk > 2) gload(2 * BK, ra1, rb1);
+    [[maybe_unused]] auto ktile = [&](int t) { return (t < nk ? t : nk - 1) * BK; };
+    if constexpr (WPACK) {
+        gload(ktile(1), ra0, rb0);
+        wload(ktile(0), wf0);
+        gload(ktile(2), ra1, rb1);
+        wload(ktile(1), wf1);
+    } else {
+        if (nk > 1) gload(BK, ra0, rb0);
+        if (nk > 2) gload(2 * BK, ra1, rb1);
+    }
     __syncthreads();
 #ifdef LAMP_TUNING
     const unsigned long long t_loop = p.trace ? wall_clock64() : 0ull;
     const unsigned long long c_loop = p.trace ? __builtin_readcyclecounter() : 0ull;
 #endif
 
+    if constexpr (WPACK) {
+        int kt = 0;
+        for (; kt + 1 < nk; kt += 2) {
+            compute(0, wf0);
+            lstore(1, ra0, rb0);
+            gload(ktile(kt + 3), ra0, rb0);
+            wload(ktile(kt + 2), wf0);
+            __syncthreads();
+            compute(1, wf1);
+            lstore(0, ra1, rb1);
+            gload(ktile(kt + 4), ra1, rb1);
+            wload(ktile(kt + 3), wf1);
+            __syncthreads();
+        }
+        if (kt < nk) compute(0, wf0);
+    } else
     for (int kt = 0; kt < nk; kt += 2) {
-        compute(0);
+        compute(0, wf0);
         if (kt + 1 < nk) lstore(1, ra0, rb0);
         if (kt + 3 < nk) gload((kt + 3) * BK, ra0, rb0);
         __syncthreads();
         if (kt + 1 >= nk) break;
-        compute(1);
+        compute(1, wf1);
         if (kt + 2 < nk) lstore(0, ra1, rb1);
         if (kt + 4 < nk) gload((kt + 4) * BK, ra1, rb1);
         __syncthreads();
@@ -377,12 +428,12 @@
 #endif
 }
 
-template <int BM, int BN, int BK, int WAVES_M, int WAVES_N, bool KTAIL, int MF, bool RPRE, bool VEC, bool RGATHER = false>
-__global__ __launch_bounds__(WAVES_M* WAVES_N * 64, (gemm_min_waves(BM, BN, BK, MF))) void gemm_nt_kernel(GemmParams p, int tiles_n_seg,
+template <int BM, int BN, int BK, int WAVES_M, int WAVES_N, bool KTAIL, int MF, bool RPRE, bool VEC, bool RGATHER = false, bool WPACK = false>
+__global__ __launch_bounds__(WAVES_M* WAVES_N * 64, (gemm_min_waves(BM, BN, BK, MF, WPACK))) void gemm_nt_kernel(GemmParams p, int tiles_n_seg,
                                                                           int tiles_n, int tiles_m,
                                                                           int panel_split, FastDiv fd_group,
                                                                           FastDiv fd_seg) {
-    gemm_body<BM, BN, BK, WAVES_M, WAVES_N, KTAIL, MF, RPRE, VEC, RGATHER>(p, tiles_n_seg, tiles_n, tiles_m, panel_split, fd_group, fd_seg);
+    gemm_body<BM, BN, BK, WAVES_M, WAVES_N, KTAIL, MF, RPRE, VEC, RGATHER, WPACK>(p, tiles_n_seg, tiles_n, tiles_m, panel_split, fd_group, fd_seg);
 }
 
 #ifdef LAMP_TUNING
@@ -393,15 +444,15 @@
 extern "C" __attribute__((visibility("default"))) void lamp_debug_set_gemm_extra_lds(int bytes) { g_extra_lds = size_t(bytes); }
 #endif
 
-template <int BM, int BN, int BK, int WAVES_M, int WAVES_N, bool KTAIL, int MF, bool VEC, bool RGATHER = false>
+template <int BM, int BN, int BK, int WAVES_M, int WAVES_N, bool KTAIL, int MF, bool VEC, bool RGATHER = false, bool WPACK = false>
 static int launch_cfg2(const GemmParams& p, hipStream_t s) {
-    using T = GemmTile<BM, BN, BK, WAVES_M, WAVES_N, MF>;
+    using T = GemmTile<BM, BN, BK, WAVES_M, WAVES_N, MF, WPACK>;
     constexpr bool RPRE = T::MI * T::NI * (MF == 32 ? 16 : 4) <= 16;
-    auto kern = gemm_nt_kernel<BM, BN, BK, WAVES_M, WAVES_N, KTAIL, MF, RPRE, VEC, RGATHER>;
-    size_t LDS = T::LDS_BYTES;
+    auto kern = gemm_nt_kernel<BM, BN, BK, WAVES_M, WAVES_N, KTAIL, MF, RPRE, VEC, RGATHER, WPACK>;
+    size_t LDS = T::LDS_LAUNCH_BYTES;
     static AttrOnce once;
 #ifdef LAMP_TUNING
-    LDS += g_extra_lds;
+    if (g_extra_lds) LDS = T::LDS_BYTES + g_extra_lds;
     if (int e = once.set(reinterpret_cast<const void*>(kern), 160 * 1024)) return e;
 #else
     if (int e = once.set(reinterpret_cast<const void*>(kern), LDS)) return e;
@@ -447,6 +498,18 @@
     return launch_cfg2<BM, BN, BK, WAVES_M, WAVES_N, false, MF, false>(p, s);
 }
 
+static int launch_packed(const GemmParams& p, hipStream_t s) {
+    if (p.rg_tok) return launch_cfg2<32, 64, 32, 1, 4, false, 16, true, true, true>(p, s);
+    return launch_cfg2<32, 64, 32, 1, 4, false, 16, true, false, true>(p, s);
+}
+
+static bool gemm_packed_ok(const GemmParams& p) {
+    if (!p.vec_epilogue || (p.N & 15) || (p.K & 31) || (int64_t(p.N) + 64) * p.K * 4 >= 0x7fffffffLL) return false;
+    for (int i = 0; i < p.nseg; ++i)
+        if (!p.Wp[i] || !aligned16(p.Wp[i])) return false;
+    return true;
+}
+
 #ifdef LAMP_TUNING
 static int g_force_tile = 0;
 static unsigned long long* g_gemm_trace = nullptr;
@@ -502,7 +565,7 @@
         case 6: return launch_cfg<64, 64, 16, 2, 2>(p, s);
         case 7: return launch_cfg<128, 64, 16, 2, 2>(p, s);
         case 8: return launch_cfg<256, 128, 16, 4, 2>(p, s);
-        case 9: return launch_cfg<32, 64, 32, 1, 4, 16>(p, s);
+        case 9: return gemm_packed_ok(p) ? launch_packed(p, s) : launch_cfg<32, 64, 32, 1, 4, 16>(p, s);
         case 10: return launch_cfg<64, 32, 32, 4, 1, 16>(p, s);
         case 11: return launch_cfg<64, 64, 16, 2, 2, 16>(p, s);
         case 12: return launch_cfg<64, 64, 32, 2, 2, 16>(p, s);
@@ -519,7 +582,12 @@
     const int64_t t64 = tiles(64, 64);
     if (tiles(128, 64) >= 2048 && p.K >= 512) return launch_cfg<128, 64, 16, 2, 2, 16>(p, s);
     if (t64 >= 2048) return launch_cfg<64, 64, 32, 2, 2, 16>(p, s);
-    if (t64 >= 1200) return launch_cfg<64, 64, 16, 2, 2, 16>(p, s);
+#ifndef LAMP_PACKED_FFN_TILE
+#define LAMP_PACKED_FFN_TILE 1
+#endif
+    const bool packed = gemm_packed_ok(p);
+    if (t64 >= 1200 && !(LAMP_PACKED_FFN_TILE && packed)) return launch_cfg<64, 64, 16, 2, 2, 16>(p, s);
+    if (packed) return launch_packed(p, s);
     return launch_cfg<32, 64, 32, 1, 4, 16>(p, s);
 }
 
diff --git a/lamp_amd/csrc/lamp_kernels.h b/lamp_amd/csrc/lamp_kernels.h
--- a/lamp_amd/csrc/lamp_kernels.h
+++ b/lamp_amd/csrc/lamp_kernels.h
@@ -20,6 +20,7 @@
     int N;
     int nseg;
     const float* W[GEMM_MAX_SEG];
+    const float* Wp[GEMM_MAX_SEG];
     int64_t ldw;
     const float* bias[GEMM_MAX_SEG];
     float* C[GEMM_MAX_SEG];
```

Result: faster. 46200, median of 6 (+1.9%).
